# bcgsc/goldpolish

Hardware: NVIDIA B200
Metric: polished_mbp_per_s (higher is better)
Workload: dtype u8/u64 integer

## Files before the change

### goldpolish_b200/api.py

```python
from __future__ import annotations

import ctypes as C
import os

import numpy as np

BF_BYTES = 524288
CBF_BYTES = 10485760
DEFAULT_KS = (32, 28, 24, 20)
GP_MAX_K = 8

_HERE = os.path.dirname(os.path.abspath(__file__))


def lib_path() -> str:
    return os.environ.get("GP_LIB_PATH") or os.path.join(_HERE, "libgoldpolish_b200.so")


class GpError(RuntimeError):
    def __init__(self, code: int, msg: str):
        super().__init__(f"goldpolish_b200 error {code}: {msg}")
        self.code = code


class _Config(C.Structure):
    _fields_ = [("struct_size", C.c_uint32), ("device", C.c_int32), ("nk", C.c_uint32),
                ("k", C.c_uint32 * GP_MAX_K), ("max_insertions", C.c_uint32), ("max_deletions", C.c_uint32),
                ("mode", C.c_int32), ("mask", C.c_int32), ("missing_ratio", C.c_float),
                ("edit_ratio", C.c_float), ("jump", C.c_uint32), ("min_contig_len", C.c_uint32),
                ("max_resident_batches", C.c_uint32), ("use_ratio", C.c_int32),
                ("missing_threshold", C.c_float), ("edit_threshold", C.c_float), ("keep_counters", C.c_int32),
                ("prep_mode", C.c_int32), ("prep_k", C.c_uint32), ("to_upper", C.c_int32),
                ("max_resident_filters", C.c_uint32)]


class _Stats(C.Structure):
    _fields_ = [("kmer_ops", C.c_uint64), ("serial_kmers", C.c_uint64), ("triggers", C.c_uint64),
                ("edits", C.c_uint64), ("masked", C.c_uint64), ("rollbacks", C.c_uint64),
                ("build_ms", C.c_float), ("polish_ms", C.c_float), ("pack_ms", C.c_float),
                ("build_kernel_ms", C.c_float), ("edit_kernel_ms", C.c_float),
                ("build_launches", C.c_uint32), ("polish_launches", C.c_uint32), ("pack_launches", C.c_uint32),
                ("build_kernel", C.c_uint32), ("build_slots", C.c_uint32), ("polish_reruns", C.c_uint32),
                ("edit_sms", C.c_uint32)]


READ_ENTRY_DTYPE = np.dtype([("read_id", np.uint32), ("kmer_threshold", np.uint32)])

_lib = None

EXPORTS = ["gp_default_config", "gp_ctx_create", "gp_ctx_destroy", "gp_last_error", "gp_ctx_set_stream",
           "gp_ctx_synchronize", "gp_get_stats", "gp_reads_upload", "gp_build_filters", "gp_build_stage",
           "gp_build_run", "gp_build_fetch", "gp_build_fetch_cbf", "gp_filters_load", "gp_polish",
           "gp_polish_stage", "gp_polish_run", "gp_polish_fetch", "gp_kmer_threshold", "gp_mappings_cap",
           "gp_guard_rejects", "gp_roof_microbench", "gp_build_round_times", "gp_pipeline_run", "gp_prep", "gp_build_output_host", "gp_host_alloc", "gp_host_free",
           "gp_build_cta_times", "gp_flagged_bed", "gp_debug_nthash", "gp_reads_begin", "gp_reads_append", "gp_reads_end"]


def load_library():
    global _lib
    if _lib is not None:
        return _lib
    p = lib_path()
    if not os.path.exists(p):
        raise ImportError(f"{p} is missing: build it with `python -c 'import __graft_entry__ as g; g.build()'` "
                          "or `make -C goldpolish_b200/csrc`; goldpolish_b200 has no CPU fallback")
    l = C.CDLL(p)
    vp, u32, u64 = C.c_void_p, C.c_uint32, C.c_uint64
    l.gp_default_config.argtypes = [C.POINTER(_Config)]
    l.gp_default_config.restype = None
    l.gp_ctx_create.argtypes = [C.POINTER(_Config), C.POINTER(vp)]
    l.gp_ctx_destroy.argtypes = [vp]
    l.gp_ctx_destroy.restype = None
    l.gp_last_error.argtypes = [vp]
    l.gp_last_error.restype = C.c_char_p
    l.gp_ctx_set_stream.argtypes = [vp, vp]
    l.gp_ctx_synchronize.argtypes = [vp]
    l.gp_get_stats.argtypes = [vp, C.POINTER(_Stats)]
    l.gp_reads_upload.argtypes = [vp, vp, vp, u64]
    l.gp_build_filters.argtypes = [vp, u32, vp, vp, vp]
    l.gp_build_stage.argtypes = [vp, u32, vp, vp]
    l.gp_build_run.argtypes = [vp]
    l.gp_build_fetch.argtypes = [vp, vp]
    l.gp_build_fetch_cbf.argtypes = [vp, u32, u32, vp]
    l.gp_filters_load.argtypes = [vp, u32, vp]
    l.gp_polish.argtypes = [vp, u32, vp, vp, vp, vp, u64, vp, vp]
    l.gp_polish_stage.argtypes = [vp, u32, vp, vp, vp]
    l.gp_polish_run.argtypes = [vp]
    l.gp_polish_fetch.argtypes = [vp, vp, u64, vp, vp]
    l.gp_kmer_threshold.argtypes = [u64]
    l.gp_kmer_threshold.restype = C.c_int
    l.gp_mappings_cap.argtypes = [u64, C.c_double]
    l.gp_mappings_cap.restype = u64
    l.gp_guard_rejects.argtypes = [u64, u64]
    l.gp_guard_rejects.restype = C.c_int
    l.gp_roof_microbench.argtypes = [vp, u32, u32, u64, C.POINTER(C.c_double), C.POINTER(C.c_float)]
    l.gp_build_round_times.argtypes = [vp, C.POINTER(u64)]
    l.gp_pipeline_run.argtypes = [vp]
    l.gp_reads_begin.argtypes = [vp, u64, vp]
    l.gp_reads_append.argtypes = [vp, vp, u64]
    l.gp_reads_end.argtypes = [vp]
    l.gp_debug_nthash.argtypes = [vp, u64, u32, vp, vp, u64, C.POINTER(u64)]
    l.gp_flagged_bed.argtypes = [vp, vp, u32, vp, vp, vp, u64]
    l.gp_flagged_bed.restype = u64
    l.gp_build_cta_times.argtypes = [vp, vp, u32, C.POINTER(u32)]
    l.gp_build_output_host.argtypes = [vp, vp]
    l.gp_host_alloc.argtypes = [u64]
    l.gp_host_alloc.restype = vp
    l.gp_host_free.argtypes = [vp]
    l.gp_host_free.restype = None
    l.gp_prep.argtypes = [vp, u32, vp, vp, C.c_int32, u32, C.c_int32, vp, u64, vp]
    _lib = l
    return l


def kmer_threshold(mappings_bases: int) -> int:
    return load_library().gp_kmer_threshold(int(mappings_bases))


def mappings_cap(target_len: int, subsample_max_per_10kbp: float) -> int:
    return int(load_library().gp_mappings_cap(int(target_len), float(subsample_max_per_10kbp)))


def guard_rejects(input_bytes: int, output_bytes: int) -> bool:
    return bool(load_library().gp_guard_rejects(int(input_bytes), int(output_bytes)))


def flagged_bed(seqs, offsets, names=None):
    l = load_library()
    off = np.ascontiguousarray(offsets, dtype=np.uint64)
    n = len(off) - 1
    cap = 1024
    while True:
        rec = np.zeros(cap, dtype=np.uint32)
        st = np.zeros(cap, dtype=np.uint64)
        en = np.zeros(cap, dtype=np.uint64)
        got = int(l.gp_flagged_bed(_ptr(seqs), _ptr(off), n, _ptr(rec), _ptr(st), _ptr(en), cap))
        if got <= cap:
            break
        cap = got
    return [((names[int(rec[i])] if names is not None else int(rec[i])), int(st[i]), int(en[i])) for i in range(got)]


def _ptr(a):
    if a is None:
        return None
    if isinstance(a, np.ndarray):
        if not a.flags["C_CONTIGUOUS"]:
            raise ValueError("array must be C-contiguous")
        return a.ctypes.data
    if hasattr(a, "data_ptr"):
        if a.is_cuda or not a.is_contiguous():
            raise ValueError("tensor must be a contiguous host tensor")
        return a.data_ptr()
    raise TypeError(type(a))


class Context:

    def __init__(self, device: int = 0, ks=DEFAULT_KS, max_insertions=5, max_deletions=5, mode=1, mask=1,
                 missing_ratio=0.5, edit_ratio=0.5, jump=3, min_contig_len=100, max_resident_batches=0,
                 keep_counters=0, prep_mode=0, prep_k=0, to_upper=0, max_resident_filters=0):
        self._l = load_library()
        cfg = _Config()
        self._l.gp_default_config(C.byref(cfg))
        cfg.device = device
        cfg.nk = len(ks)
        for i, k in enumerate(ks):
            cfg.k[i] = k
        cfg.max_insertions, cfg.max_deletions, cfg.mode, cfg.mask = max_insertions, max_deletions, mode, mask
        cfg.missing_ratio, cfg.edit_ratio, cfg.jump, cfg.min_contig_len = missing_ratio, edit_ratio, jump, min_contig_len
        cfg.max_resident_batches = max_resident_batches
        cfg.keep_counters = keep_counters
        cfg.prep_mode, cfg.prep_k, cfg.to_upper = prep_mode, prep_k, to_upper
        cfg.max_resident_filters = max_resident_filters
        h = C.c_void_p()
        rc = self._l.gp_ctx_create(C.byref(cfg), C.byref(h))
        if rc != 0:
            raise GpError(rc, self._l.gp_last_error(None).decode())
        self._h = h
        self.ks = tuple(ks)
        self.nk = len(ks)
        self.n_batches = 0

    def close(self):
        if getattr(self, "_h", None):
            self._l.gp_ctx_destroy(self._h)
            self._h = None

    def __del__(self):
        try:
            self.close()
        except Exception:
            pass

    def __enter__(self):
        return self

    def __exit__(self, *a):
        self.close()

    def _ck(self, rc):
        if rc != 0:
            raise GpError(rc, self._l.gp_last_error(self._h).decode())

    def set_stream(self, cuda_stream: int | None):
        self._ck(self._l.gp_ctx_set_stream(self._h, C.c_void_p(cuda_stream or 0)))

    def synchronize(self):
        self._ck(self._l.gp_ctx_synchronize(self._h))

    def stats(self) -> dict:
        s = _Stats()
        self._ck(self._l.gp_get_stats(self._h, C.byref(s)))
        return {n: getattr(s, n) for n, _ in _Stats._fields_}

    def upload_reads(self, seqs, offsets):
        offsets = np.ascontiguousarray(offsets, dtype=np.uint64)
        self._keep = (seqs, offsets)
        self._ck(self._l.gp_reads_upload(self._h, _ptr(seqs), _ptr(offsets), len(offsets) - 1))

    def upload_reads_piecewise(self, lens, pieces):
        lens = np.ascontiguousarray(lens, dtype=np.uint32)
        self._ck(self._l.gp_reads_begin(self._h, len(lens), _ptr(lens)))
        for seqs, n in pieces:
            seqs = np.ascontiguousarray(seqs, dtype=np.uint8)
            self._ck(self._l.gp_reads_append(self._h, _ptr(seqs) if seqs.size else None, int(n)))
        self._ck(self._l.gp_reads_end(self._h))

    def build_stage(self, batch_entry_off, entries):
        off = np.ascontiguousarray(batch_entry_off, dtype=np.uint64)
        ent = np.ascontiguousarray(entries, dtype=READ_ENTRY_DTYPE)
        self.n_batches = len(off) - 1
        self._ck(self._l.gp_build_stage(self._h, self.n_batches, _ptr(off), _ptr(ent)))

    def build_run(self):
        self._ck(self._l.gp_build_run(self._h))

    def build_output(self, pinned):
        self._bf_pinned = pinned
        self._ck(self._l.gp_build_output_host(self._h, _ptr(pinned) if pinned is not None else None))

    def build_fetch(self, out=None, want=True):
        if want and out is None:
            out = np.empty((self.n_batches, self.nk, BF_BYTES), dtype=np.uint8)
        self._ck(self._l.gp_build_fetch(self._h, _ptr(out) if want else None))
        return out if want else None

    def build_filters(self, batch_entry_off, entries, fetch=True, out=None):
        self.build_stage(batch_entry_off, entries)
        self.build_run()
        return self.build_fetch(out=out, want=fetch)

    def fetch_cbf(self, batch: int, k_index: int) -> np.ndarray:
        out = np.empty(CBF_BYTES, dtype=np.uint8)
        self._ck(self._l.gp_build_fetch_cbf(self._h, batch, k_index, _ptr(out)))
        return out

    def load_filters(self, payloads):
        payloads = np.ascontiguousarray(payloads, dtype=np.uint8)
        n = payloads.size // (self.nk * BF_BYTES)
        if n * self.nk * BF_BYTES != payloads.size:
            raise ValueError("payloads must be n_batches * nk * 524288 bytes")
        self.n_batches = n
        self._ck(self._l.gp_filters_load(self._h, n, _ptr(payloads)))

    def polish_stage(self, seqs, offsets, contig_batch):
        off = np.ascontiguousarray(offsets, dtype=np.uint64)
        cb = np.ascontiguousarray(contig_batch, dtype=np.uint32)
        self._n_contigs = len(off) - 1
        self._in_bases = int(off[-1])
        self._ck(self._l.gp_polish_stage(self._h, self._n_contigs, _ptr(seqs), _ptr(off), _ptr(cb)))

    def polish_run(self):
        self._ck(self._l.gp_polish_run(self._h))

    def pipeline_run(self):
        self._ck(self._l.gp_pipeline_run(self._h))

    def polish_fetch(self, out=None):
        n = self._n_contigs
        out_off = np.zeros(n + 1, dtype=np.uint64)
        dropped = np.zeros(max(n, 1), dtype=np.uint8)
        if out is None:
            out = np.empty(self._in_bases + self._in_bases // 4 + 65536, dtype=np.uint8)
        rc = self._l.gp_polish_fetch(self._h, _ptr(out), out.nbytes if isinstance(out, np.ndarray) else out.numel(),
                                     _ptr(out_off), _ptr(dropped))
        if rc == -1 and int(out_off[n]) > (out.nbytes if isinstance(out, np.ndarray) else out.numel()):
            out = np.empty(int(out_off[n]), dtype=np.uint8)
            rc = self._l.gp_polish_fetch(self._h, _ptr(out), out.nbytes, _ptr(out_off), _ptr(dropped))
        self._ck(rc)
        return out, out_off, dropped[:n]

    def polish(self, seqs, offsets, contig_batch, out=None):
        self.polish_stage(seqs, offsets, contig_batch)
        self.polish_run()
        return self.polish_fetch(out=out)

    def prep(self, seqs, offsets, mode: int, k: int = 0, to_upper: int = 0):
        off = np.ascontiguousarray(offsets, dtype=np.uint64)
        n = len(off) - 1
        out = np.empty(int(off[-1]) + n + 16, dtype=np.uint8)
        out_off = np.zeros(n + 1, dtype=np.uint64)
        self._ck(self._l.gp_prep(self._h, n, _ptr(seqs), _ptr(off), mode, k, to_upper, _ptr(out), out.nbytes, _ptr(out_off)))
        return out, out_off

    def build_round_times(self):
        out = (C.c_uint64 * 32)()
        self._ck(self._l.gp_build_round_times(self._h, out))
        r = {n: (out[3 * i] / 1e6, out[3 * i + 1] / 1e6, int(out[3 * i + 2])) for i, n in enumerate(self.INTERVAL_KINDS)}
        r["list_entries"] = int(out[31])
        return r

    INTERVAL_KINDS = ("clear", "round0", "level1", "late", "round0+late", "level1+late")

    def debug_nthash(self, read_id: int, k: int):
        n = C.c_uint64()
        cap = 1 << 16
        while True:
            hs = np.zeros((cap, 4), dtype=np.uint64)
            valid = np.zeros(cap, dtype=np.uint8)
            rc = self._l.gp_debug_nthash(self._h, read_id, k, _ptr(hs), _ptr(valid), cap, C.byref(n))
            if rc == -1 and n.value > cap:
                cap = n.value
                continue
            self._ck(rc)
            break
        pos = np.nonzero(valid[:n.value])[0]
        return pos, hs[pos]

    def build_cta_times(self) -> np.ndarray:
        out = np.zeros((1024, 32), dtype=np.uint64)
        n = C.c_uint32()
        self._ck(self._l.gp_build_cta_times(self._h, _ptr(out), 1024, C.byref(n)))
        return out[:n.value, :18].reshape(n.value, 6, 3)

    def roof_microbench(self, warps: int, iters: int, region_bytes: int = CBF_BYTES):
        sps, ms = C.c_double(), C.c_float()
        self._ck(self._l.gp_roof_microbench(self._h, warps, iters, region_bytes, C.byref(sps), C.byref(ms)))
        return sps.value, ms.value
```

### goldpolish_b200/csrc/gp_abi.cu

```cuda
#include "gp_kernels.cuh"

#include <algorithm>
#include <cstdio>
#include <cstdlib>
#include <cstring>
#include <numeric>
#include <string>
#include <vector>

namespace {

thread_local std::string g_create_error;

struct DevBuf {
  void* p = nullptr;
  size_t cap = 0;
  cudaError_t ensure(size_t need)
  {
    if (need <= cap) return cudaSuccess;
    if (p) cudaFree(p);
    p = nullptr; cap = 0;
    size_t want = need + need / 8 + 256;
    cudaError_t e = cudaMalloc(&p, want);
    if (e != cudaSuccess) { cudaGetLastError(); e = cudaMalloc(&p, need); want = need; }
    if (e == cudaSuccess) cap = want;
    return e;
  }
  void release() { if (p) cudaFree(p); p = nullptr; cap = 0; }
  template<typename T> T* as() const { return static_cast<T*>(p); }
};

}

struct gp_ctx {
  gp_config cfg;
  int sm_count = 0;
  cudaStream_t own_stream = nullptr, stream = nullptr;
  uint8_t* bf_host_user = nullptr;
  uint32_t* bf_host_dev = nullptr;
  bool bf_streamed = false;
  std::vector<uint32_t> h_pre, h_maxthr;
  std::vector<uint64_t> h_batch_entry_off;
  std::vector<uint4> h_stream_tab;
  DevBuf d_stream_tab;
  std::vector<uint32_t> h_empty_streams;
  bool edit_ev_valid = false;
  int l2_persist_max = 0, l2_window_max = 0;
  bool l2_window_set = false, l2_roof_window = false;
  int overlap_state = 0;
  bool pipelined = false;
  cudaEvent_t ev[6] = { nullptr, nullptr, nullptr, nullptr, nullptr, nullptr };
  std::vector<cudaEvent_t> wave_ev;
  cudaEvent_t edit_ev[2] = { nullptr, nullptr };
  std::string err;
  gp_stats stats;
  bool build_timed = false, polish_timed = false, pack_timed = false;

  uint64_t n_reads = 0;
  uint64_t reads_total = 0, reads_next = 0, read_slab = 0;
  std::vector<uint32_t> h_read_len;
  std::vector<uint64_t> h_read_boff;
  DevBuf d_ascii, d_ascii_off, d_pk, d_nm, d_read_boff, d_read_len;

  uint32_t n_batches = 0;
  bool filters_ready = false;
  bool build_done = false;
  bool build_staged = false;
  uint32_t wave_batches = 0;
  bool bf_all_resident = true;
  std::vector<uint32_t> h_bf_slot;
  DevBuf d_bf_slot;
  std::vector<uint32_t> wave_first, wave_count, wave_order_off;
  DevBuf d_batch_entry_off, d_entries, d_bf_pool, d_cbf_pool, d_stream_order, d_next, d_counters;
  DevBuf d_step_pre, d_batch_max_thr, d_V, d_alive, d_anchor, d_entry_rel, d_cta_times, d_sm_table;
  uint32_t edit_sms = 0;
  uint32_t edit_ctas_per_sm = 0;
  int sm_split_state = 0;
  uint32_t level_grid = 0;
  uint64_t anchor_stride = 0;
  uint32_t alive_words = 0, n_entries = 0, surv_cap = 0, level_slots = 1, level_time_bits = 26, level_arrays = 2;
  bool levels_ok = false;
  int build_algo = 0;
  int build_algo_resolved = 1;

  uint32_t n_contigs = 0;
  bool polish_staged = false, polish_done = false;
  uint32_t grow = 0;
  std::vector<uint64_t> h_in_off, h_cap_off, h_node_off;
  std::vector<uint32_t> h_len, h_order, h_batch;
  std::vector<uint32_t> h_batch_order, h_order_pipe;
  std::vector<uint32_t> h_wave_contig_off;
  DevBuf d_batch_order, d_batch_done, d_order_pipe;
  DevBuf d_input, d_in_off, d_buf0, d_buf1, d_cap_off, d_cur_len, d_which, d_dropped, d_nodes, d_node_off,
    d_contig_batch, d_order, d_pnext, d_pcounters, d_error, d_out, d_out_off;
};

#define GP_FAIL(ctx, code, msg)                                                                              \
  do {                                                                                                       \
    (ctx)->err = (msg);                                                                                      \
    return (code);                                                                                           \
  } while (0)

#define GP_CUDA(ctx, call)                                                                                   \
  do {                                                                                                       \
    cudaError_t e_ = (call);                                                                                 \
    if (e_ != cudaSuccess) {                                                                                 \
      (ctx)->err = std::string(#call) + ": " + cudaGetErrorString(e_);                                       \
      cudaGetLastError();                                                                                    \
      return e_ == cudaErrorMemoryAllocation ? GP_ERR_OOM : GP_ERR_CUDA;                                     \
    }                                                                                                        \
  } while (0)

namespace {

__global__ void scatter_contigs_kernel(const char* __restrict__ in, const uint64_t* __restrict__ in_off,
                                       char* __restrict__ buf0, const uint64_t* __restrict__ cap_off,
                                       uint32_t* __restrict__ cur_len, uint32_t n)
{
  for (uint32_t c = blockIdx.x; c < n; c += gridDim.x) {
    const uint64_t a = in_off[c];
    const uint32_t len = uint32_t(in_off[c + 1] - a);
    char* dst = buf0 + cap_off[c];
    for (uint32_t i = threadIdx.x; i < len; i += blockDim.x) dst[i] = in[a + i];
    if (threadIdx.x == 0) cur_len[c] = len;
  }
}

__global__ void gather_contigs_kernel(const char* __restrict__ buf0, const char* __restrict__ buf1,
                                      const uint64_t* __restrict__ cap_off, const uint8_t* __restrict__ which,
                                      const uint64_t* __restrict__ out_off, char* __restrict__ out, uint32_t n)
{
  for (uint32_t c = blockIdx.x; c < n; c += gridDim.x) {
    const uint64_t o = out_off[c];
    const uint32_t len = uint32_t(out_off[c + 1] - o);
    const char* src = (which[c] ? buf1 : buf0) + cap_off[c];
    for (uint32_t i = threadIdx.x; i < len; i += blockDim.x) out[o + i] = src[i];
  }
}

int validate_config(const gp_config& c, std::string& why)
{
  if (c.nk == 0 || c.nk > GP_MAX_K_VALUES) { why = "nk must be 1..8"; return GP_ERR_ARG; }
  for (uint32_t i = 0; i < c.nk; i++)
    if (c.k[i] < 4 || c.k[i] > 32) { why = "k must be within 4..32"; return GP_ERR_ARG; }
  if (c.max_insertions > 5) { why = "max_insertions must be <= 5"; return GP_ERR_ARG; }
  if (c.max_deletions > 10) { why = "max_deletions must be <= 10"; return GP_ERR_ARG; }
  if (c.mode < 0 || c.mode > 2) { why = "mode must be 0..2"; return GP_ERR_ARG; }
  if (c.jump == 0) { why = "jump must be >= 1"; return GP_ERR_ARG; }
  if (c.prep_mode < 0 || c.prep_mode > 2) { why = "prep_mode must be 0..2"; return GP_ERR_ARG; }
  if (c.prep_mode && (c.prep_k == 0 || c.prep_k > 64)) { why = "prep_k must be within 1..64"; return GP_ERR_ARG; }
  if (!c.use_ratio && (!(c.missing_threshold > 0) || !(c.edit_threshold > 0))) { why = "x / y thresholds must be > 0"; return GP_ERR_ARG; }
  return GP_OK;
}

}

extern "C" {

void gp_default_config(gp_config* cfg)
{
  std::memset(cfg, 0, sizeof(*cfg));
  cfg->struct_size = sizeof(gp_config);
  cfg->device = 0;
  cfg->nk = 4;
  cfg->k[0] = 32; cfg->k[1] = 28; cfg->k[2] = 24; cfg->k[3] = 20;
  cfg->max_insertions = 5; cfg->max_deletions = 5; cfg->mode = 1; cfg->mask = 1;
  cfg->missing_ratio = 0.5f; cfg->edit_ratio = 0.5f;
  cfg->use_ratio = 1;
  cfg->missing_threshold = 5.0f; cfg->edit_threshold = 9.0f;
  cfg->jump = 3; cfg->min_contig_len = 100;
  cfg->max_resident_batches = 0;
}

const char* gp_last_error(const gp_ctx* ctx) { return ctx ? ctx->err.c_str() : g_create_error.c_str(); }

int gp_ctx_create(const gp_config* cfg, gp_ctx** out)
{
  if (!cfg || !out) { g_create_error = "null argument"; return GP_ERR_ARG; }
  *out = nullptr;
  gp_config c;
  gp_default_config(&c);
  std::memcpy(&c, cfg, std::min<size_t>(cfg->struct_size ? cfg->struct_size : sizeof(gp_config), sizeof(gp_config)));
  c.struct_size = sizeof(gp_config);
  std::string why;
  if (int rc = validate_config(c, why)) { g_create_error = why; return rc; }
  int ndev = 0;
  cudaError_t e = cudaGetDeviceCount(&ndev);
  if (e != cudaSuccess || ndev == 0) {
    cudaGetLastError();
    g_create_error = std::string("no CUDA device available (") + cudaGetErrorString(e) +
                     "); goldpolish_b200 has no CPU path";
    return GP_ERR_NO_DEVICE;
  }
  if (c.device < 0 || c.device >= ndev) { g_create_error = "device ordinal out of range"; return GP_ERR_ARG; }
  if ((e = cudaSetDevice(c.device)) != cudaSuccess) { g_create_error = cudaGetErrorString(e); return GP_ERR_CUDA; }
  gp_ctx* ctx = new gp_ctx();
  ctx->cfg = c;
  std::memset(&ctx->stats, 0, sizeof(ctx->stats));
  cudaDeviceGetAttribute(&ctx->sm_count, cudaDevAttrMultiProcessorCount, c.device);
  cudaDeviceGetAttribute(&ctx->l2_persist_max, cudaDevAttrMaxPersistingL2CacheSize, c.device);
  cudaDeviceGetAttribute(&ctx->l2_window_max, cudaDevAttrMaxAccessPolicyWindowSize, c.device);

  if ((e = cudaStreamCreateWithFlags(&ctx->own_stream, cudaStreamNonBlocking)) != cudaSuccess) {
    g_create_error = cudaGetErrorString(e);
    delete ctx;
    return GP_ERR_CUDA;
  }
  ctx->stream = ctx->own_stream;
  gp::preload_levels();
  gp::preload_edit();
  for (auto& ev : ctx->ev) cudaEventCreate(&ev);
  for (auto& ev : ctx->edit_ev) cudaEventCreate(&ev);
  *out = ctx;
  return GP_OK;
}

void gp_ctx_destroy(gp_ctx* ctx)
{
  if (!ctx) return;
  cudaSetDevice(ctx->cfg.device);
  cudaStreamSynchronize(ctx->stream);
  DevBuf* bufs[] = { &ctx->d_ascii, &ctx->d_ascii_off, &ctx->d_pk, &ctx->d_nm, &ctx->d_read_boff, &ctx->d_read_len,
                     &ctx->d_batch_entry_off, &ctx->d_entries, &ctx->d_bf_pool, &ctx->d_cbf_pool, &ctx->d_stream_order,
                     &ctx->d_next, &ctx->d_counters, &ctx->d_step_pre, &ctx->d_batch_max_thr, &ctx->d_V, &ctx->d_alive, &ctx->d_anchor, &ctx->d_entry_rel, &ctx->d_input, &ctx->d_in_off, &ctx->d_buf0, &ctx->d_buf1,
                     &ctx->d_cap_off, &ctx->d_cur_len, &ctx->d_which, &ctx->d_dropped, &ctx->d_nodes, &ctx->d_node_off,
                     &ctx->d_contig_batch, &ctx->d_order, &ctx->d_pnext, &ctx->d_pcounters, &ctx->d_error, &ctx->d_out,
                     &ctx->d_out_off, &ctx->d_batch_order, &ctx->d_batch_done, &ctx->d_order_pipe, &ctx->d_stream_tab, &ctx->d_cta_times, &ctx->d_bf_slot };
  for (auto* b : bufs) b->release();
  if (ctx->l2_window_set) { cudaCtxResetPersistingL2Cache(); cudaDeviceSetLimit(cudaLimitPersistingL2CacheSize, 0); }
  for (auto& ev : ctx->ev) if (ev) cudaEventDestroy(ev);
  for (auto& ev : ctx->edit_ev) if (ev) cudaEventDestroy(ev);
  for (auto& ev : ctx->wave_ev) if (ev) cudaEventDestroy(ev);
  if (ctx->own_stream) cudaStreamDestroy(ctx->own_stream);
  delete ctx;
}

int gp_ctx_set_stream(gp_ctx* ctx, void* cuda_stream)
{
  if (!ctx) return GP_ERR_ARG;
  cudaSetDevice(ctx->cfg.device);
  GP_CUDA(ctx, cudaStreamSynchronize(ctx->stream));
  ctx->stream = cuda_stream ? static_cast<cudaStream_t>(cuda_stream) : ctx->own_stream;
  return GP_OK;
}

int gp_ctx_synchronize(gp_ctx* ctx)
{
  if (!ctx) return GP_ERR_ARG;
  cudaSetDevice(ctx->cfg.device);
  GP_CUDA(ctx, cudaStreamSynchronize(ctx->stream));
  return GP_OK;
}

static uint32_t sm_split_check(gp_ctx* ctx)
{
  if (!ctx->edit_sms || !ctx->d_sm_table.p) return 0;
  std::vector<uint32_t> t(1 + 2 * 2048);
  if (cudaMemcpy(t.data(), ctx->d_sm_table.p, t.size() * 4, cudaMemcpyDeviceToHost) != cudaSuccess) { cudaGetLastError(); return 0; }
  uint32_t full = 0, other = 0, given_back = 0;
  const uint32_t keep = uint32_t(ctx->sm_count) - ctx->edit_sms;
  for (size_t i = 0; i < 2048; i++) {
    const uint32_t arrived = t[1 + 2 * i], rank_p1 = t[2 + 2 * i];
    if (arrived == ctx->edit_ctas_per_sm) { full++; if (rank_p1 > keep) given_back++; }
    else if (arrived) other++;
  }
  const bool ok = !other && full == uint32_t(ctx->sm_count) && given_back == ctx->edit_sms;
  if (ctx->sm_split_state == 0 || !ok) ctx->sm_split_state = ok ? 1 : -1;
  return ok ? given_back : 0;
}

int gp_get_stats(const gp_ctx* cctx, gp_stats* out)
{
  if (!cctx || !out) return GP_ERR_ARG;
  gp_ctx* ctx = const_cast<gp_ctx*>(cctx);
  cudaSetDevice(ctx->cfg.device);
  GP_CUDA(ctx, cudaStreamSynchronize(ctx->stream));
  if (ctx->pack_timed) cudaEventElapsedTime(&ctx->stats.pack_ms, ctx->ev[0], ctx->ev[1]);
  if (ctx->build_timed && ctx->pipelined) {
    cudaEventElapsedTime(&ctx->stats.build_ms, ctx->ev[2], ctx->ev[3]);
    unsigned long long c[gp::kBuildCounters], pc[8];
    GP_CUDA(ctx, cudaMemcpy(c, ctx->d_counters.p, sizeof c, cudaMemcpyDeviceToHost));
    GP_CUDA(ctx, cudaMemcpy(pc, ctx->d_pcounters.p, sizeof pc, cudaMemcpyDeviceToHost));
    ctx->stats.kmer_ops = c[0];
    ctx->stats.serial_kmers = c[1];
    ctx->stats.build_kernel_ms = float(double(c[21] - c[20]) * 1e-6);
    ctx->stats.edit_kernel_ms = float(double(pc[5] - pc[4]) * 1e-6);
    ctx->stats.polish_ms = ctx->stats.edit_kernel_ms;
    ctx->stats.triggers = pc[0]; ctx->stats.edits = pc[1]; ctx->stats.masked = pc[2]; ctx->stats.rollbacks = pc[3];
    ctx->stats.edit_sms = sm_split_check(ctx);
    *out = ctx->stats;
    return GP_OK;
  }
  if (ctx->build_timed) {
    cudaEventElapsedTime(&ctx->stats.build_ms, ctx->ev[2], ctx->ev[3]);
    ctx->stats.build_kernel_ms = 0;
    for (size_t wv = 0; wv < ctx->wave_first.size() && 2 * wv + 1 < ctx->wave_ev.size(); wv++) {
      float t = 0;
      if (cudaEventElapsedTime(&t, ctx->wave_ev[2 * wv], ctx->wave_ev[2 * wv + 1]) == cudaSuccess) ctx->stats.build_kernel_ms += t;
    }
    unsigned long long c[2] = { 0, 0 };
    GP_CUDA(ctx, cudaMemcpy(c, ctx->d_counters.p, sizeof c, cudaMemcpyDeviceToHost));
    ctx->stats.kmer_ops = c[0];
    ctx->stats.serial_kmers = c[1];
  }
  if (ctx->polish_timed && ctx->edit_ev_valid) {
    cudaEventElapsedTime(&ctx->stats.polish_ms, ctx->ev[4], ctx->ev[5]);
    ctx->stats.edit_kernel_ms = 0;
    if (ctx->n_contigs) cudaEventElapsedTime(&ctx->stats.edit_kernel_ms, ctx->edit_ev[0], ctx->edit_ev[1]);
    unsigned long long c[4] = { 0, 0, 0, 0 };
    GP_CUDA(ctx, cudaMemcpy(c, ctx->d_pcounters.p, sizeof c, cudaMemcpyDeviceToHost));
    ctx->stats.triggers = c[0]; ctx->stats.edits = c[1]; ctx->stats.masked = c[2]; ctx->stats.rollbacks = c[3];
  }
  *out = ctx->stats;
  return GP_OK;
}

static const uint64_t kReadSlabBytes = 256ull << 20;

int gp_reads_begin(gp_ctx* ctx, uint64_t n_reads, const uint32_t* lens)
{
  if (!ctx || (!lens && n_reads)) return GP_ERR_ARG;
  if (n_reads > 0xFFFFFFF0ull) GP_FAIL(ctx, GP_ERR_ARG, "too many reads");
  cudaSetDevice(ctx->cfg.device);
  ctx->n_reads = 0;
  ctx->reads_next = 0;
  ctx->h_read_len.assign(lens, lens + n_reads);
  ctx->h_read_boff.resize(n_reads + 1);
  uint64_t b = 0, longest = 0;
  for (uint64_t r = 0; r < n_reads; r++) {
    if (lens[r] >= (1u << 31)) GP_FAIL(ctx, GP_ERR_ARG, "read longer than 2^31 bases");
    ctx->h_read_boff[r] = b;
    b += (uint64_t(lens[r]) + 31) & ~31ull;
    longest = std::max<uint64_t>(longest, lens[r]);
  }
  ctx->h_read_boff[n_reads] = b;
  const uint64_t words = b / 32 + 2;
  ctx->read_slab = std::max(kReadSlabBytes, longest);
  if (const char* e = std::getenv("GP_READ_SLAB_BYTES")) ctx->read_slab = std::max<uint64_t>(uint64_t(std::atoll(e)), std::max<uint64_t>(longest, 1));
  GP_CUDA(ctx, ctx->d_read_boff.ensure((n_reads + 1) * 8));
  GP_CUDA(ctx, ctx->d_read_len.ensure((n_reads + 1) * 4));
  GP_CUDA(ctx, ctx->d_pk.ensure(words * 8));
  GP_CUDA(ctx, ctx->d_nm.ensure(words * 4));
  cudaStream_t s = ctx->stream;
  GP_CUDA(ctx, cudaMemcpyAsync(ctx->d_read_boff.p, ctx->h_read_boff.data(), (n_reads + 1) * 8, cudaMemcpyHostToDevice, s));
  if (n_reads) GP_CUDA(ctx, cudaMemcpyAsync(ctx->d_read_len.p, ctx->h_read_len.data(), n_reads * 4, cudaMemcpyHostToDevice, s));
  GP_CUDA(ctx, cudaMemsetAsync(ctx->d_nm.as<uint32_t>() + (words - 2), 0xFF, 8, s));
  GP_CUDA(ctx, cudaMemsetAsync(ctx->d_pk.as<uint64_t>() + (words - 2), 0, 16, s));
  GP_CUDA(ctx, cudaEventRecord(ctx->ev[0], s));
  GP_CUDA(ctx, cudaStreamSynchronize(s));
  ctx->reads_total = n_reads;
  ctx->stats.pack_launches = 0;
  return GP_OK;
}

int gp_reads_append(gp_ctx* ctx, const char* seqs, uint64_t n)
{
  if (!ctx || (!seqs && n)) return GP_ERR_ARG;
  if (ctx->reads_next + n > ctx->reads_total) GP_FAIL(ctx, GP_ERR_STATE, "gp_reads_append: more reads than gp_reads_begin announced");
  cudaSetDevice(ctx->cfg.device);
  cudaStream_t s = ctx->stream;
  uint64_t r = ctx->reads_next, done = 0;
  const uint64_t r_end = r + n;
  std::vector<uint64_t> aoff;
  while (r < r_end) {
    uint64_t r1 = r, bytes = 0;
    while (r1 < r_end && (r1 == r || bytes + ctx->h_read_len[r1] <= ctx->read_slab)) bytes += ctx->h_read_len[r1++];
    const uint64_t cnt = r1 - r;
    aoff.resize(cnt + 1);
    aoff[0] = 0;
    for (uint64_t i = 0; i < cnt; i++) aoff[i + 1] = aoff[i] + ctx->h_read_len[r + i];
    GP_CUDA(ctx, ctx->d_ascii.ensure(bytes + 16));
    GP_CUDA(ctx, ctx->d_ascii_off.ensure((cnt + 1) * 8));
    if (bytes) GP_CUDA(ctx, cudaMemcpyAsync(ctx->d_ascii.p, seqs + done, bytes, cudaMemcpyHostToDevice, s));
    GP_CUDA(ctx, cudaMemcpyAsync(ctx->d_ascii_off.p, aoff.data(), (cnt + 1) * 8, cudaMemcpyHostToDevice, s));
    gp::launch_pack_reads(ctx->d_ascii.as<char>(), ctx->d_ascii_off.as<uint64_t>(), ctx->d_read_boff.as<uint64_t>() + r,
                          ctx->d_pk.as<uint64_t>(), ctx->d_nm.as<uint32_t>(), uint32_t(cnt), s);
    GP_CUDA(ctx, cudaGetLastError());
    ctx->stats.pack_launches++;
    GP_CUDA(ctx, cudaStreamSynchronize(s));
    done += bytes;
    r = r1;
  }
  ctx->reads_next = r_end;
  return GP_OK;
}

int gp_reads_end(gp_ctx* ctx)
{
  if (!ctx) return GP_ERR_ARG;
  if (ctx->reads_next != ctx->reads_total) GP_FAIL(ctx, GP_ERR_STATE, "gp_reads_end: fewer reads appended than gp_reads_begin announced");
  cudaSetDevice(ctx->cfg.device);
  GP_CUDA(ctx, cudaEventRecord(ctx->ev[1], ctx->stream));
  GP_CUDA(ctx, cudaStreamSynchronize(ctx->stream));
  ctx->pack_timed = true;
  if (ctx->d_ascii.cap > 2 * kReadSlabBytes) ctx->d_ascii.release();
  ctx->n_reads = ctx->reads_total;
  return GP_OK;
}

int gp_reads_upload(gp_ctx* ctx, const char* seqs, const uint64_t* offsets, uint64_t n_reads)
{
  if (!ctx || (!seqs && n_reads) || !offsets) return GP_ERR_ARG;
  std::vector<uint32_t> lens(n_reads);
  for (uint64_t r = 0; r < n_reads; r++) {
    const uint64_t len = offsets[r + 1] - offsets[r];
    if (len >= (1ull << 31)) GP_FAIL(ctx, GP_ERR_ARG, "read longer than 2^31 bases");
    lens[r] = uint32_t(len);
  }
  if (int rc = gp_reads_begin(ctx, n_reads, lens.data())) return rc;
  if (n_reads)
    if (int rc = gp_reads_append(ctx, seqs + offsets[0], n_reads)) return rc;
  return gp_reads_end(ctx);
}

int gp_build_stage(gp_ctx* ctx, uint32_t n_batches, const uint64_t* batch_entry_off, const gp_read_entry* entries)
{
  if (!ctx || !batch_entry_off || (!entries && n_batches && batch_entry_off[n_batches])) return GP_ERR_ARG;
  cudaSetDevice(ctx->cfg.device);
  const gp_config& c = ctx->cfg;
  const uint64_t n_entries = batch_entry_off[n_batches];
  std::vector<uint64_t> work(n_batches, 0);
  for (uint32_t b = 0; b < n_batches; b++) {
    for (uint64_t e = batch_entry_off[b]; e < batch_entry_off[b + 1]; e++) {
      if (entries[e].read_id >= ctx->n_reads) GP_FAIL(ctx, GP_ERR_ARG, "read_id out of range (upload reads first)");
      if (entries[e].kmer_threshold < 4)
        GP_FAIL(ctx, GP_ERR_ARG, "kmer_threshold must be greater than or equal to 4");
      work[b] += ctx->h_read_len[entries[e].read_id];
    }
  }
  {
    std::vector<uint32_t> pre(size_t(c.nk) * (n_entries + 1), 0u), maxthr(std::max<uint32_t>(n_batches, 1), 0u);
    bool ok = true;
    uint64_t max_steps = 0;
    for (uint32_t ki = 0; ki < c.nk; ki++) {
      uint32_t* pk = pre.data() + size_t(ki) * (n_entries + 1);
      uint64_t acc = 0;
      for (uint64_t e = 0; e < n_entries; e++) {
        pk[e] = uint32_t(acc);
        const uint32_t len = ctx->h_read_len[entries[e].read_id];
        if (len >= c.k[ki]) acc += (uint64_t(len) - c.k[ki] + 1 + 31) / 32;
      }
      pk[n_entries] = uint32_t(acc);
      if (acc >= 0xFFFFFFFFull) ok = false;
      for (uint32_t b = 0; b < n_batches && ok; b++) {
        const uint64_t st = uint64_t(pk[batch_entry_off[b + 1]]) - pk[batch_entry_off[b]];
        max_steps = std::max(max_steps, st);
        if (st * 32 >= (1ull << 26)) ok = false;
      }
    }
    std::vector<uint16_t> entry_rel(std::max<uint64_t>(n_entries, 1), 0);
    for (uint32_t b = 0; b < n_batches; b++) {
      if (batch_entry_off[b + 1] - batch_entry_off[b] > 0xFFFFull) ok = false;
      for (uint64_t e = batch_entry_off[b]; e < batch_entry_off[b + 1]; e++) {
        maxthr[b] = std::max(maxthr[b], entries[e].kmer_threshold);
        if (entries[e].kmer_threshold > 24) ok = false;
        entry_rel[e] = uint16_t(e - batch_entry_off[b]);
      }
    }
    ctx->h_empty_streams.clear();
    for (uint32_t ki = 0; ki < c.nk; ki++) {
      const uint32_t* pk = pre.data() + size_t(ki) * (n_entries + 1);
      for (uint32_t b = 0; b < n_batches; b++)
        if (pk[batch_entry_off[b + 1]] == pk[batch_entry_off[b]]) ctx->h_empty_streams.push_back(b * c.nk + ki);
    }
    ctx->anchor_stride = 1;
    for (uint32_t ki = 0; ki < c.nk; ki++)
      ctx->anchor_stride = std::max<uint64_t>(ctx->anchor_stride, uint64_t(pre[size_t(ki) * (n_entries + 1) + n_entries]) + 1);
    ctx->levels_ok = ok;
    ctx->h_pre = pre;
    ctx->h_maxthr = maxthr;
    ctx->h_batch_entry_off.assign(batch_entry_off, batch_entry_off + n_batches + 1);
    ctx->n_entries = uint32_t(n_entries);
    ctx->alive_words = uint32_t(max_steps + 1);
    ctx->level_time_bits = 16;
    while (ctx->level_time_bits < 26 && (max_steps * 32) >> ctx->level_time_bits) ctx->level_time_bits++;
    GP_CUDA(ctx, ctx->d_step_pre.ensure(pre.size() * 4));
    GP_CUDA(ctx, ctx->d_batch_max_thr.ensure(maxthr.size() * 4));
    ctx->level_slots = 2;
    if (const char* f = std::getenv("GP_LEVEL_OVERLAP")) ctx->level_slots = f[0] == '0' ? 1u : 2u;
    ctx->level_arrays = 2;
    if (const char* f = std::getenv("GP_LEVEL_ARRAYS")) ctx->level_arrays = f[0] == '3' ? 3u : 2u;
    GP_CUDA(ctx, ctx->d_V.ensure(gp::kCbfCounters * 4 * ctx->level_arrays));
    ctx->surv_cap = uint32_t(size_t(ctx->alive_words) * 32 + size_t(8192) * 9 * 32);
    GP_CUDA(ctx, ctx->d_alive.ensure(size_t(ctx->surv_cap) * gp::kLevelSurvWords * gp::kLevelListBufs * 4 + 64 + 8192));
    GP_CUDA(ctx, cudaMemcpyAsync(ctx->d_step_pre.p, pre.data(), pre.size() * 4, cudaMemcpyHostToDevice, ctx->stream));
    GP_CUDA(ctx, cudaMemcpyAsync(ctx->d_batch_max_thr.p, maxthr.data(), maxthr.size() * 4, cudaMemcpyHostToDevice, ctx->stream));
    if (ok) {
      GP_CUDA(ctx, ctx->d_entry_rel.ensure(entry_rel.size() * 2));
      GP_CUDA(ctx, ctx->d_anchor.ensure(ctx->anchor_stride * c.nk * 2));
      GP_CUDA(ctx, cudaMemcpyAsync(ctx->d_entry_rel.p, entry_rel.data(), entry_rel.size() * 2, cudaMemcpyHostToDevice, ctx->stream));
      gp::launch_fill_anchor(ctx->d_step_pre.as<uint32_t>(), ctx->d_entry_rel.as<uint16_t>(), ctx->d_anchor.as<uint16_t>(),
                             uint32_t(n_entries), c.nk, ctx->anchor_stride, ctx->stream);
      GP_CUDA(ctx, cudaGetLastError());
    }
    GP_CUDA(ctx, cudaStreamSynchronize(ctx->stream));
  }
  {
    int algo = ctx->build_algo;
    if (const char* f = std::getenv("GP_BUILD_KERNEL")) algo = f[0] == 'l' ? 2 : (f[0] == 's' || f[0] == 'p') ? 1 : algo;
    if (algo == 0) algo = 2;
    if (!ctx->levels_ok) algo = 1;
    ctx->build_algo_resolved = algo;
  }
  const bool uses_cbf = ctx->build_algo_resolved == 1 || c.keep_counters;
  const uint64_t per_batch = uint64_t(c.nk) * gp::kCbfCounters, per_batch_bf = uint64_t(c.nk) * gp::kBfBytes;
  uint32_t wave = n_batches;
  if (c.max_resident_batches) wave = std::min(wave, c.max_resident_batches);
  {
    size_t free_b = 0, total_b = 0;
    GP_CUDA(ctx, cudaMemGetInfo(&free_b, &total_b));
    const uint64_t usable = uint64_t(free_b) + ctx->d_cbf_pool.cap + ctx->d_bf_pool.cap;
    const uint64_t headroom = 3ull << 30;
    uint64_t bf_limit = n_batches;
    if (c.max_resident_filters) bf_limit = std::min<uint64_t>(bf_limit, c.max_resident_filters);
    const uint64_t fit_bf = usable > headroom ? (usable - headroom) / 2 / per_batch_bf : 0;
    if (fit_bf == 0 && n_batches) GP_FAIL(ctx, GP_ERR_OOM, "not enough device memory for one batch of filters");
    bf_limit = std::min(bf_limit, fit_bf);
    ctx->bf_all_resident = bf_limit >= n_batches;
    if (!ctx->bf_all_resident) wave = uint32_t(std::min<uint64_t>(wave, bf_limit));
    if (uses_cbf) {
      const uint64_t left = usable > headroom ? usable - headroom - (ctx->bf_all_resident ? uint64_t(n_batches) * per_batch_bf : 0) : 0;
      const uint64_t fit = left / (per_batch + (ctx->bf_all_resident ? 0 : per_batch_bf));
      if (fit == 0 && n_batches) GP_FAIL(ctx, GP_ERR_OOM, "not enough device memory for one batch of counting filters");
      wave = uint32_t(std::min<uint64_t>(wave, fit));
    }
  }
  GP_CUDA(ctx, ctx->d_bf_pool.ensure(std::max<uint64_t>(uint64_t(ctx->bf_all_resident ? n_batches : wave) * per_batch_bf, 4)));
  if (n_batches && uses_cbf) {
    cudaError_t e = ctx->d_cbf_pool.ensure(uint64_t(wave) * per_batch);
    while (e != cudaSuccess && wave > 1) { cudaGetLastError(); wave = (wave + 1) / 2; e = ctx->d_cbf_pool.ensure(uint64_t(wave) * per_batch); }
    GP_CUDA(ctx, e);
  }
  ctx->wave_batches = wave;
  ctx->wave_first.clear(); ctx->wave_count.clear(); ctx->wave_order_off.clear();
  std::vector<uint32_t> order_all;
  order_all.reserve(size_t(n_batches) * c.nk);
  for (uint32_t first = 0; first < n_batches; first += wave) {
    const uint32_t cnt = std::min(wave, n_batches - first);
    ctx->wave_first.push_back(first);
    ctx->wave_count.push_back(cnt);
    ctx->wave_order_off.push_back(uint32_t(order_all.size()));
    std::vector<uint32_t> idx(size_t(cnt) * c.nk);
    std::iota(idx.begin(), idx.end(), 0u);
    std::stable_sort(idx.begin(), idx.end(), [&](uint32_t a, uint32_t b2) {
      return work[first + a / c.nk] > work[first + b2 / c.nk];
    });
    order_all.insert(order_all.end(), idx.begin(), idx.end());
  }
  const size_t n_waves = ctx->wave_first.size();
  GP_CUDA(ctx, ctx->d_batch_entry_off.ensure((size_t(n_batches) + 1) * 8));
  GP_CUDA(ctx, ctx->d_entries.ensure(std::max<size_t>(n_entries, 1) * sizeof(gp_read_entry)));
  GP_CUDA(ctx, ctx->d_stream_order.ensure(std::max<size_t>(order_all.size(), 1) * 4));
  GP_CUDA(ctx, ctx->d_next.ensure(std::max<size_t>(n_waves, 1) * 4));
  GP_CUDA(ctx, ctx->d_counters.ensure(gp::kBuildCounters * 8));
  cudaStream_t s = ctx->stream;
  GP_CUDA(ctx, cudaMemcpyAsync(ctx->d_batch_entry_off.p, batch_entry_off, (size_t(n_batches) + 1) * 8, cudaMemcpyHostToDevice, s));
  if (n_entries)
    GP_CUDA(ctx, cudaMemcpyAsync(ctx->d_entries.p, entries, n_entries * sizeof(gp_read_entry), cudaMemcpyHostToDevice, s));
  if (!order_all.empty())
    GP_CUDA(ctx, cudaMemcpyAsync(ctx->d_stream_order.p, order_all.data(), order_all.size() * 4, cudaMemcpyHostToDevice, s));
  GP_CUDA(ctx, cudaStreamSynchronize(s));
  ctx->n_batches = n_batches;
  ctx->build_staged = true;
  ctx->filters_ready = false;
  ctx->build_done = false;
  return GP_OK;
}

static int build_stream_tab(gp_ctx* ctx, cudaStream_t s, bool build_order)
{
  const gp_config& c = ctx->cfg;
  const size_t total = size_t(ctx->n_batches) * c.nk;
  ctx->h_stream_tab.resize(std::max<size_t>(total, 1));
  const size_t ne1 = size_t(ctx->n_entries) + 1;
  size_t w = 0;
  for (size_t wv = 0; wv < ctx->wave_first.size(); wv++)
    for (uint32_t st = 0; st < ctx->wave_count[wv] * c.nk; st++, w++) {
      const uint32_t lb = st / c.nk, ki = st - lb * c.nk;
      const uint32_t b = build_order ? ctx->h_batch_order[ctx->wave_first[wv] + lb] : ctx->wave_first[wv] + lb;
      const uint32_t* pk = ctx->h_pre.data() + size_t(ki) * ne1;
      const uint32_t steps = pk[ctx->h_batch_entry_off[b + 1]] - pk[ctx->h_batch_entry_off[b]];
      ctx->h_stream_tab[w] = make_uint4(steps, ctx->h_maxthr[b] - 2u + ki, b, 0u);
    }
  GP_CUDA(ctx, ctx->d_stream_tab.ensure(ctx->h_stream_tab.size() * sizeof(uint4)));
  GP_CUDA(ctx, cudaMemcpyAsync(ctx->d_stream_tab.p, ctx->h_stream_tab.data(), ctx->h_stream_tab.size() * sizeof(uint4), cudaMemcpyHostToDevice, s));
  return GP_OK;
}

static int upload_bf_slots(gp_ctx* ctx, cudaStream_t s, bool build_order)
{
  if (ctx->bf_all_resident) return GP_OK;
  const uint32_t nb = ctx->n_batches, wave = std::max(ctx->wave_batches, 1u);
  ctx->h_bf_slot.resize(nb);
  for (uint32_t pos = 0; pos < nb; pos++) ctx->h_bf_slot[build_order ? ctx->h_batch_order[pos] : pos] = pos % wave;
  GP_CUDA(ctx, ctx->d_bf_slot.ensure(std::max<size_t>(nb, 1) * 4));
  GP_CUDA(ctx, cudaMemcpyAsync(ctx->d_bf_slot.p, ctx->h_bf_slot.data(), size_t(nb) * 4, cudaMemcpyHostToDevice, s));
  return GP_OK;
}

static int build_launch_levels_wave(gp_ctx* ctx, cudaStream_t s, size_t wv, uint32_t* batch_done, int ctas_per_sm, uint32_t reserve_sms = 0)
{
  const gp_config& c = ctx->cfg;
  {
    size_t tab_off = 0;
    for (size_t i = 0; i < wv; i++) tab_off += size_t(ctx->wave_count[i]) * c.nk;
    gp::LevelParams p;
    std::memset(&p, 0, sizeof p);
    p.pk = ctx->d_pk.as<uint64_t>();
    p.nm = ctx->d_nm.as<uint32_t>();
    p.read_boff = ctx->d_read_boff.as<uint64_t>();
    p.read_len = ctx->d_read_len.as<uint32_t>();
    p.batch_entry_off = ctx->d_batch_entry_off.as<uint64_t>();
    p.entries = ctx->d_entries.as<gp_read_entry>();
    p.step_pre = ctx->d_step_pre.as<uint32_t>();
    p.batch_max_thr = ctx->d_batch_max_thr.as<uint32_t>();
    p.anchor = ctx->d_anchor.as<uint16_t>();
    p.anchor_stride = ctx->anchor_stride;
    p.V = ctx->d_V.as<uint32_t>();
    p.surv = ctx->d_alive.as<uint32_t>();
    p.bars = reinterpret_cast<unsigned long long*>(ctx->d_alive.as<uint32_t>() + size_t(gp::kLevelSurvWords) * gp::kLevelListBufs * ctx->surv_cap);
    p.overlap = ctx->level_slots > 1 ? 1u : 0u;
    p.arrays = ctx->level_arrays;
    p.time_bits = ctx->level_time_bits;
    if (const char* f = std::getenv("GP_LEVEL_REPORT_CTA")) p.report_cta = uint32_t(std::atoi(f));
    p.cbf_pool = c.keep_counters ? ctx->d_cbf_pool.as<uint8_t>() : nullptr;
    p.bf_pool = ctx->d_bf_pool.as<uint32_t>();
    p.bf_slot = ctx->bf_all_resident ? nullptr : ctx->d_bf_slot.as<uint32_t>();
    p.counters = ctx->d_counters.as<unsigned long long>();
    p.surv_cap = ctx->surv_cap;
    p.n_entries = ctx->n_entries;
    p.n_streams = ctx->wave_count[wv] * c.nk;
    p.first_batch = ctx->wave_first[wv];
    p.stream_tab = ctx->d_stream_tab.as<uint4>() + tab_off;
    p.nk = c.nk;
    for (uint32_t i = 0; i < gp::kMaxK; i++) p.k[i] = i < c.nk ? c.k[i] : 0;
    if (c.keep_counters) GP_CUDA(ctx, cudaMemsetAsync(ctx->d_cbf_pool.p, 0, uint64_t(p.n_streams) * gp::kCbfCounters, s));
    GP_CUDA(ctx, cudaMemsetAsync(ctx->d_V.p, 0xFF, gp::kCbfCounters * 4 * ctx->level_arrays, s));
    GP_CUDA(ctx, cudaMemsetAsync(p.bars, 0, 64 + 8192, s));
    p.speed = reinterpret_cast<uint32_t*>(p.bars + 8);
    {
      const char* e = std::getenv("GP_LEVEL_WEIGHTED");
      p.weighted = !(e && e[0] == '0') ? 1u : 0u;
    }
    while (ctx->wave_ev.size() < 2 * (wv + 1)) { cudaEvent_t e2 = nullptr; cudaEventCreate(&e2); ctx->wave_ev.push_back(e2); }
    if (!batch_done) GP_CUDA(ctx, cudaEventRecord(ctx->wave_ev[2 * wv], s));
    p.batch_done = batch_done;
    p.n_batches_total = ctx->n_batches;
    p.bf_host = ctx->bf_host_dev;
    {
      const size_t vbytes = gp::kCbfCounters * 4 * p.arrays;
      const char* e = std::getenv("GP_L2_PERSIST");
      const bool want = !(e && e[0] == '0') && ctx->l2_persist_max > 0 && vbytes <= size_t(ctx->l2_window_max);
      cudaStreamAttrValue av;
      std::memset(&av, 0, sizeof av);
      if (want) {
        const char* wsel = std::getenv("GP_L2_WINDOW");
        const bool only_c = wsel && wsel[0] == 'c' && p.arrays == 3u;
        const size_t wbytes = only_c ? gp::kCbfCounters * 4 : vbytes;
        av.accessPolicyWindow.base_ptr = only_c ? static_cast<void*>(ctx->d_V.as<uint32_t>() + 2 * gp::kCbfCounters) : ctx->d_V.p;
        av.accessPolicyWindow.num_bytes = wbytes;
        av.accessPolicyWindow.hitRatio = std::min(1.0f, float(ctx->l2_persist_max) / float(wbytes));
        av.accessPolicyWindow.hitProp = cudaAccessPropertyPersisting;
        av.accessPolicyWindow.missProp = cudaAccessPropertyStreaming;
      }
      if (want != ctx->l2_window_set) {
        if (cudaDeviceSetLimit(cudaLimitPersistingL2CacheSize, want ? size_t(ctx->l2_persist_max) : 0) != cudaSuccess) cudaGetLastError();
        if (!want) cudaCtxResetPersistingL2Cache();
      }
      if (want || ctx->l2_window_set) {
        GP_CUDA(ctx, cudaStreamSetAttribute(s, cudaStreamAttributeAccessPolicyWindow, &av));
        ctx->l2_window_set = want;
      }
    }
    if (std::getenv("GP_LEVEL_CTA_TIMES")) {
      GP_CUDA(ctx, ctx->d_cta_times.ensure(size_t(ctx->sm_count) * 4 * 32 * 8));
      GP_CUDA(ctx, cudaMemsetAsync(ctx->d_cta_times.p, 0, size_t(ctx->sm_count) * 4 * 32 * 8, s));
      p.cta_times = ctx->d_cta_times.as<unsigned long long>();
    }
    if (reserve_sms) {
      const size_t bytes = (1 + 2 * 2048) * 4;
      GP_CUDA(ctx, ctx->d_sm_table.ensure(bytes));
      GP_CUDA(ctx, cudaMemsetAsync(ctx->d_sm_table.p, 0, bytes, s));
      p.keep_sms = uint32_t(ctx->sm_count) - reserve_sms;
      p.sm_table = ctx->d_sm_table.as<uint32_t>();
    }
    ctx->level_grid = uint32_t((ctx->sm_count - int(reserve_sms)) * gp::levels_ctas_per_sm(ctas_per_sm));
    GP_CUDA(ctx, gp::launch_build_filters_levels(p, ctx->sm_count, s, ctas_per_sm));
    if (!batch_done) GP_CUDA(ctx, cudaEventRecord(ctx->wave_ev[2 * wv + 1], s));
  }
  return GP_OK;
}

static int build_launch_inorder_wave(gp_ctx* ctx, cudaStream_t s, size_t wv)
{
  const gp_config& c = ctx->cfg;
  gp::BuildParams p;
  std::memset(&p, 0, sizeof p);
  p.pk = ctx->d_pk.as<uint64_t>();
  p.nm = ctx->d_nm.as<uint32_t>();
  p.read_boff = ctx->d_read_boff.as<uint64_t>();
  p.read_len = ctx->d_read_len.as<uint32_t>();
  p.batch_entry_off = ctx->d_batch_entry_off.as<uint64_t>();
  p.entries = ctx->d_entries.as<gp_read_entry>();
  p.cbf_pool = ctx->d_cbf_pool.as<uint8_t>();
  p.bf_pool = ctx->d_bf_pool.as<uint32_t>();
  p.bf_slot = ctx->bf_all_resident ? nullptr : ctx->d_bf_slot.as<uint32_t>();
  p.stream_order = ctx->d_stream_order.as<uint32_t>() + ctx->wave_order_off[wv];
  p.next_stream = ctx->d_next.as<uint32_t>() + wv;
  p.counters = ctx->d_counters.as<unsigned long long>();
  p.n_streams = ctx->wave_count[wv] * c.nk;
  p.first_batch = ctx->wave_first[wv];
  p.nk = c.nk;
  for (uint32_t i = 0; i < gp::kMaxK; i++) p.k[i] = i < c.nk ? c.k[i] : 0;
  GP_CUDA(ctx, cudaMemsetAsync(ctx->d_cbf_pool.p, 0, uint64_t(p.n_streams) * gp::kCbfCounters, s));
  while (ctx->wave_ev.size() < 2 * (wv + 1)) { cudaEvent_t e2 = nullptr; cudaEventCreate(&e2); ctx->wave_ev.push_back(e2); }
  GP_CUDA(ctx, cudaEventRecord(ctx->wave_ev[2 * wv], s));
  gp::launch_build_filters(p, ctx->sm_count, s);
  GP_CUDA(ctx, cudaGetLastError());
  GP_CUDA(ctx, cudaEventRecord(ctx->wave_ev[2 * wv + 1], s));
  return GP_OK;
}

static int wave_payloads_out(gp_ctx* ctx, cudaStream_t s, size_t wv, bool kernel_streams)
{
  if (ctx->bf_all_resident || kernel_streams || !ctx->bf_host_user) return GP_OK;
  const uint64_t per = uint64_t(ctx->cfg.nk) * gp::kBfBytes;
  GP_CUDA(ctx, cudaMemcpyAsync(ctx->bf_host_user + uint64_t(ctx->wave_first[wv]) * per, ctx->d_bf_pool.p,
                               uint64_t(ctx->wave_count[wv]) * per, cudaMemcpyDeviceToHost, s));
  return GP_OK;
}

int gp_build_run(gp_ctx* ctx)
{
  if (!ctx) return GP_ERR_ARG;
  if (!ctx->build_staged) GP_FAIL(ctx, GP_ERR_STATE, "gp_build_run before gp_build_stage");
  cudaSetDevice(ctx->cfg.device);
  const gp_config& c = ctx->cfg;
  cudaStream_t s = ctx->stream;
  if (!ctx->bf_all_resident && !ctx->bf_host_user)
    GP_FAIL(ctx, GP_ERR_STATE, "the filters of this call are not all resident at once (max_resident_filters / device memory): "
                               "name a page-locked destination with gp_build_output_host, or use gp_pipeline_run");
  GP_CUDA(ctx, cudaEventRecord(ctx->ev[2], s));
  ctx->pipelined = false;
  uint32_t launches = 0;
  GP_CUDA(ctx, cudaMemsetAsync(ctx->d_counters.p, 0, gp::kBuildCounters * 8, s));
  GP_CUDA(ctx, cudaMemsetAsync(ctx->d_counters.as<unsigned long long>() + 20, 0xFF, 8, s));
  const uint64_t per_bf = uint64_t(c.nk) * gp::kBfBytes;
  if (ctx->n_batches) {
    GP_CUDA(ctx, cudaMemsetAsync(ctx->d_next.p, 0, ctx->wave_first.size() * 4, s));
    if (ctx->bf_all_resident) GP_CUDA(ctx, cudaMemsetAsync(ctx->d_bf_pool.p, 0, uint64_t(ctx->n_batches) * per_bf, s));
  }
  const int algo = ctx->build_algo_resolved;
  if (int rc = upload_bf_slots(ctx, s, false)) return rc;
  if (algo == 2)
    if (int rc = build_stream_tab(ctx, s, false)) return rc;
  for (size_t wv = 0; wv < ctx->wave_first.size(); wv++) {
    if (!ctx->bf_all_resident) GP_CUDA(ctx, cudaMemsetAsync(ctx->d_bf_pool.p, 0, uint64_t(ctx->wave_count[wv]) * per_bf, s));
    if (algo == 2) { if (int rc = build_launch_levels_wave(ctx, s, wv, nullptr, 0)) return rc; }
    else if (int rc = build_launch_inorder_wave(ctx, s, wv)) return rc;
    if (int rc = wave_payloads_out(ctx, s, wv, algo == 2 && ctx->bf_host_dev)) return rc;
    launches += 1;
  }
  ctx->bf_streamed = ctx->bf_host_user && ((algo == 2 && ctx->bf_host_dev) || !ctx->bf_all_resident);
  GP_CUDA(ctx, cudaEventRecord(ctx->ev[3], s));
  ctx->build_timed = true;
  ctx->stats.build_launches = launches;
  ctx->stats.build_kernel = uint32_t(algo);
  ctx->stats.build_slots = algo == 2 ? ctx->level_slots : 0;
  ctx->filters_ready = ctx->bf_all_resident;
  ctx->build_done = true;
  return GP_OK;
}

int gp_build_round_times(gp_ctx* ctx, uint64_t out[32])
{
  if (!ctx || !out) return GP_ERR_ARG;
  if (!ctx->build_done) GP_FAIL(ctx, GP_ERR_STATE, "no filters have been built");
  cudaSetDevice(ctx->cfg.device);
  GP_CUDA(ctx, cudaStreamSynchronize(ctx->stream));
  unsigned long long c[gp::kBuildCounters];
  GP_CUDA(ctx, cudaMemcpy(c, ctx->d_counters.p, sizeof c, cudaMemcpyDeviceToHost));
  std::memset(out, 0, 32 * 8);
  for (uint32_t i = 0; i < gp::kLevelDiag; i++) out[i] = c[gp::kLevelDiagAt + i];
  out[31] = c[17];
  return GP_OK;
}

int gp_debug_nthash(gp_ctx* ctx, uint64_t read_id, uint32_t k, uint64_t* hashes, uint8_t* valid, uint64_t cap_positions,
                    uint64_t* n_positions)
{
  if (!ctx || !hashes || !valid || !n_positions) return GP_ERR_ARG;
  if (read_id >= ctx->n_reads) GP_FAIL(ctx, GP_ERR_ARG, "read_id out of range (upload reads first)");
  if (k < 4 || k > 32) GP_FAIL(ctx, GP_ERR_ARG, "k must be within 4..32");
  cudaSetDevice(ctx->cfg.device);
  const uint32_t len = ctx->h_read_len[read_id];
  const uint64_t npos = len >= k ? uint64_t(len) - k + 1 : 0;
  *n_positions = npos;
  if (npos == 0) return GP_OK;
  if (npos > cap_positions) GP_FAIL(ctx, GP_ERR_ARG, "gp_debug_nthash: output too small (needed positions are in n_positions)");
  uint64_t boff = 0;
  GP_CUDA(ctx, cudaMemcpy(&boff, ctx->d_read_boff.as<uint64_t>() + read_id, 8, cudaMemcpyDeviceToHost));
  DevBuf dh, dv;
  GP_CUDA(ctx, dh.ensure(npos * 32));
  cudaError_t e = dv.ensure(npos);
  if (e != cudaSuccess) { dh.release(); GP_CUDA(ctx, e); }
  gp::launch_debug_nthash(ctx->d_pk.as<uint64_t>(), ctx->d_nm.as<uint32_t>(), boff >> 5, len, k, dh.as<uint64_t>(), dv.as<uint8_t>(), ctx->stream);
  e = cudaGetLastError();
  if (e == cudaSuccess) e = cudaMemcpyAsync(hashes, dh.p, npos * 32, cudaMemcpyDeviceToHost, ctx->stream);
  if (e == cudaSuccess) e = cudaMemcpyAsync(valid, dv.p, npos, cudaMemcpyDeviceToHost, ctx->stream);
  if (e == cudaSuccess) e = cudaStreamSynchronize(ctx->stream);
  dh.release(); dv.release();
  GP_CUDA(ctx, e);
  return GP_OK;
}

int gp_build_cta_times(gp_ctx* ctx, uint64_t* out, uint32_t cap_ctas, uint32_t* n_ctas)
{
  if (!ctx || !out || !n_ctas) return GP_ERR_ARG;
  if (!ctx->build_done || !ctx->d_cta_times.p) GP_FAIL(ctx, GP_ERR_STATE, "no per-CTA times were recorded (set GP_LEVEL_CTA_TIMES=1 before the build)");
  cudaSetDevice(ctx->cfg.device);
  GP_CUDA(ctx, cudaStreamSynchronize(ctx->stream));
  *n_ctas = std::min(cap_ctas, ctx->level_grid);
  GP_CUDA(ctx, cudaMemcpy(out, ctx->d_cta_times.p, size_t(*n_ctas) * 32 * 8, cudaMemcpyDeviceToHost));
  return GP_OK;
}

void* gp_host_alloc(uint64_t bytes)
{
  void* p = nullptr;
  if (cudaHostAlloc(&p, size_t(bytes), cudaHostAllocDefault) != cudaSuccess) { cudaGetLastError(); return nullptr; }
  return p;
}

void gp_host_free(void* p)
{
  if (p) cudaFreeHost(p);
}

int gp_build_output_host(gp_ctx* ctx, uint8_t* bf_out_pinned)
{
  if (!ctx) return GP_ERR_ARG;
  cudaSetDevice(ctx->cfg.device);
  ctx->bf_host_user = nullptr;
  ctx->bf_host_dev = nullptr;
  ctx->bf_streamed = false;
  if (!bf_out_pinned) return GP_OK;
  cudaPointerAttributes at;
  if (cudaPointerGetAttributes(&at, bf_out_pinned) != cudaSuccess || at.type != cudaMemoryTypeHost || !at.devicePointer) {
    cudaGetLastError();
    GP_FAIL(ctx, GP_ERR_ARG, "gp_build_output_host needs page-locked host memory (cudaHostAlloc / cudaHostRegister)");
  }
  ctx->bf_host_user = bf_out_pinned;
  ctx->bf_host_dev = static_cast<uint32_t*>(at.devicePointer);
  return GP_OK;
}

int gp_build_fetch(gp_ctx* ctx, uint8_t* bf_out)
{
  if (!ctx) return GP_ERR_ARG;
  if (!ctx->build_done && !ctx->filters_ready) GP_FAIL(ctx, GP_ERR_STATE, "no filters have been built");
  cudaSetDevice(ctx->cfg.device);
  if (bf_out && bf_out == ctx->bf_host_user && ctx->bf_streamed) {
    GP_CUDA(ctx, cudaStreamSynchronize(ctx->stream));
    for (uint32_t sidx : ctx->h_empty_streams) std::memset(bf_out + uint64_t(sidx) * gp::kBfBytes, 0, gp::kBfBytes);
    return GP_OK;
  }
  if (bf_out && !ctx->bf_all_resident)
    GP_FAIL(ctx, GP_ERR_STATE, "the filters of earlier waves are no longer resident: their payloads went to the buffer named with "
                               "gp_build_output_host (pass that pointer)");
  if (bf_out && ctx->n_batches)
    GP_CUDA(ctx, cudaMemcpyAsync(bf_out, ctx->d_bf_pool.p, uint64_t(ctx->n_batches) * ctx->cfg.nk * gp::kBfBytes,
                                 cudaMemcpyDeviceToHost, ctx->stream));
  GP_CUDA(ctx, cudaStreamSynchronize(ctx->stream));
  return GP_OK;
}

int gp_build_fetch_cbf(gp_ctx* ctx, uint32_t batch, uint32_t k_index, uint8_t* cbf_out)
{
  if (!ctx || !cbf_out) return GP_ERR_ARG;
  if (!ctx->build_done) GP_FAIL(ctx, GP_ERR_STATE, "no filters have been built");
  if (batch >= ctx->n_batches || k_index >= ctx->cfg.nk) GP_FAIL(ctx, GP_ERR_ARG, "batch / k index out of range");
  if (ctx->build_algo_resolved == 2 && !ctx->cfg.keep_counters)
    GP_FAIL(ctx, GP_ERR_STATE, "counting-filter bytes were not materialised: create the context with keep_counters = 1");
  const size_t last = ctx->wave_first.size() - 1;
  if (batch < ctx->wave_first[last]) GP_FAIL(ctx, GP_ERR_STATE, "counting filter of an earlier wave is no longer resident");
  cudaSetDevice(ctx->cfg.device);
  const uint64_t sid = uint64_t(batch - ctx->wave_first[last]) * ctx->cfg.nk + k_index;
  GP_CUDA(ctx, cudaMemcpyAsync(cbf_out, ctx->d_cbf_pool.as<uint8_t>() + sid * gp::kCbfCounters, gp::kCbfCounters,
                               cudaMemcpyDeviceToHost, ctx->stream));
  GP_CUDA(ctx, cudaStreamSynchronize(ctx->stream));
  return GP_OK;
}

int gp_build_filters(gp_ctx* ctx, uint32_t n_batches, const uint64_t* batch_entry_off, const gp_read_entry* entries,
                     uint8_t* bf_out)
{
  int rc = gp_build_stage(ctx, n_batches, batch_entry_off, entries);
  if (rc) return rc;
  if ((rc = gp_build_run(ctx))) return rc;
  return gp_build_fetch(ctx, bf_out);
}

int gp_filters_load(gp_ctx* ctx, uint32_t n_batches, const uint8_t* bf_payloads)
{
  if (!ctx || (!bf_payloads && n_batches)) return GP_ERR_ARG;
  cudaSetDevice(ctx->cfg.device);
  const uint64_t bytes = uint64_t(n_batches) * ctx->cfg.nk * gp::kBfBytes;
  GP_CUDA(ctx, ctx->d_bf_pool.ensure(std::max<uint64_t>(bytes, 4)));
  if (bytes) GP_CUDA(ctx, cudaMemcpyAsync(ctx->d_bf_pool.p, bf_payloads, bytes, cudaMemcpyHostToDevice, ctx->stream));
  GP_CUDA(ctx, cudaStreamSynchronize(ctx->stream));
  ctx->n_batches = n_batches;
  ctx->filters_ready = true;
  ctx->bf_all_resident = true;
  ctx->build_staged = false;
  ctx->build_done = false;
  return GP_OK;
}

static int polish_layout(gp_ctx* ctx)
{
  const uint32_t n = ctx->n_contigs;
  const uint32_t g = ctx->grow;
  ctx->h_cap_off.assign(n + 1, 0);
  ctx->h_node_off.assign(n + 1, 0);
  for (uint32_t i = 0; i < n; i++) {
    const uint64_t len = ctx->h_len[i];
    uint64_t cap = len + (len >> 1) + 4096;
    uint64_t nodes = (len >> 2) + 2048;
    cap <<= g; nodes <<= g;
    cap = (cap + 15) & ~15ull;
    if (cap >= (1ull << 32)) { ctx->err = "contig too long for 32-bit positions"; return GP_ERR_ARG; }
    ctx->h_cap_off[i + 1] = ctx->h_cap_off[i] + cap;
    ctx->h_node_off[i + 1] = ctx->h_node_off[i] + nodes;
  }
  GP_CUDA(ctx, ctx->d_buf0.ensure(std::max<uint64_t>(ctx->h_cap_off[n], 16)));
  GP_CUDA(ctx, ctx->d_buf1.ensure(std::max<uint64_t>(ctx->h_cap_off[n], 16)));
  GP_CUDA(ctx, ctx->d_nodes.ensure(std::max<uint64_t>(ctx->h_node_off[n], 1) * sizeof(gp::EdNode)));
  GP_CUDA(ctx, ctx->d_cap_off.ensure((size_t(n) + 1) * 8));
  GP_CUDA(ctx, ctx->d_node_off.ensure((size_t(n) + 1) * 8));
  GP_CUDA(ctx, cudaMemcpyAsync(ctx->d_cap_off.p, ctx->h_cap_off.data(), (size_t(n) + 1) * 8, cudaMemcpyHostToDevice, ctx->stream));
  GP_CUDA(ctx, cudaMemcpyAsync(ctx->d_node_off.p, ctx->h_node_off.data(), (size_t(n) + 1) * 8, cudaMemcpyHostToDevice, ctx->stream));
  GP_CUDA(ctx, cudaStreamSynchronize(ctx->stream));
  return GP_OK;
}

int gp_polish_stage(gp_ctx* ctx, uint32_t n_contigs, const char* seqs, const uint64_t* offsets, const uint32_t* contig_batch)
{
  if (!ctx || !offsets || (!seqs && n_contigs && offsets[n_contigs]) || (!contig_batch && n_contigs)) return GP_ERR_ARG;
  if (!ctx->filters_ready && !ctx->build_staged)
    GP_FAIL(ctx, GP_ERR_STATE, "gp_polish needs filters (gp_build_filters, gp_build_stage or gp_filters_load)");
  cudaSetDevice(ctx->cfg.device);
  const uint32_t n = n_contigs;
  ctx->n_contigs = n;
  ctx->h_len.resize(n);
  ctx->h_in_off.assign(offsets, offsets + n + 1);
  ctx->h_batch.assign(contig_batch, contig_batch + n);
  for (uint32_t i = 0; i < n; i++) {
    const uint64_t len = offsets[i + 1] - offsets[i];
    if (len >= (1ull << 31)) GP_FAIL(ctx, GP_ERR_ARG, "contig longer than 2^31 bases");
    if (contig_batch[i] >= ctx->n_batches) GP_FAIL(ctx, GP_ERR_ARG, "contig_batch out of range of the current filter set");
    ctx->h_len[i] = uint32_t(len);
  }
  ctx->h_order.resize(n);
  std::iota(ctx->h_order.begin(), ctx->h_order.end(), 0u);
  std::stable_sort(ctx->h_order.begin(), ctx->h_order.end(), [&](uint32_t a, uint32_t b) { return ctx->h_len[a] > ctx->h_len[b]; });
  const uint64_t total = offsets[n];
  GP_CUDA(ctx, ctx->d_input.ensure(std::max<uint64_t>(total, 16)));
  GP_CUDA(ctx, ctx->d_in_off.ensure((size_t(n) + 1) * 8));
  GP_CUDA(ctx, ctx->d_cur_len.ensure(std::max<size_t>(n, 1) * 4));
  GP_CUDA(ctx, ctx->d_which.ensure(std::max<size_t>(n, 1)));
  GP_CUDA(ctx, ctx->d_dropped.ensure(std::max<size_t>(n, 1)));
  GP_CUDA(ctx, ctx->d_contig_batch.ensure(std::max<size_t>(n, 1) * 4));
  GP_CUDA(ctx, ctx->d_order.ensure(std::max<size_t>(n, 1) * 4));
  GP_CUDA(ctx, ctx->d_pnext.ensure(4));
  GP_CUDA(ctx, ctx->d_pcounters.ensure(64));
  GP_CUDA(ctx, ctx->d_error.ensure(4));
  cudaStream_t s = ctx->stream;
  if (total) GP_CUDA(ctx, cudaMemcpyAsync(ctx->d_input.p, seqs, total, cudaMemcpyHostToDevice, s));
  GP_CUDA(ctx, cudaMemcpyAsync(ctx->d_in_off.p, offsets, (size_t(n) + 1) * 8, cudaMemcpyHostToDevice, s));
  if (n) {
    GP_CUDA(ctx, cudaMemcpyAsync(ctx->d_contig_batch.p, contig_batch, size_t(n) * 4, cudaMemcpyHostToDevice, s));
    GP_CUDA(ctx, cudaMemcpyAsync(ctx->d_order.p, ctx->h_order.data(), size_t(n) * 4, cudaMemcpyHostToDevice, s));
  }
  ctx->grow = 0;
  if (int rc = polish_layout(ctx)) return rc;
  ctx->polish_staged = true;
  ctx->polish_done = false;
  return GP_OK;
}

static int polish_prepare(gp_ctx* ctx)
{
  cudaStream_t s = ctx->stream;
  const uint32_t n = ctx->n_contigs;
  GP_CUDA(ctx, cudaMemsetAsync(ctx->d_pnext.p, 0, 4, s));
  GP_CUDA(ctx, cudaMemsetAsync(ctx->d_pcounters.p, 0, 64, s));
  GP_CUDA(ctx, cudaMemsetAsync(ctx->d_pcounters.as<unsigned long long>() + 4, 0xFF, 8, s));
  GP_CUDA(ctx, cudaMemsetAsync(ctx->d_error.p, 0, 4, s));
  if (n == 0) return GP_OK;
  const uint32_t grid = std::min<uint32_t>(n, uint32_t(ctx->sm_count) * 8u);
  scatter_contigs_kernel<<<grid, 256, 0, s>>>(ctx->d_input.as<char>(), ctx->d_in_off.as<uint64_t>(), ctx->d_buf0.as<char>(),
                                              ctx->d_cap_off.as<uint64_t>(), ctx->d_cur_len.as<uint32_t>(), n);
  GP_CUDA(ctx, cudaGetLastError());
  return GP_OK;
}

static int polish_edit(gp_ctx* ctx, cudaStream_t es, const uint32_t* order, uint32_t n_order, const uint32_t* batch_done, int alongside)
{
  const gp_config& c = ctx->cfg;
  const uint32_t n = order ? n_order : ctx->n_contigs;
  if (n == 0) return GP_OK;
  gp::EditParams p;
  std::memset(&p, 0, sizeof p);
  p.n_contigs = n;
  p.buf[0] = ctx->d_buf0.as<char>();
  p.buf[1] = ctx->d_buf1.as<char>();
  p.cap_off = ctx->d_cap_off.as<uint64_t>();
  p.cur_len = ctx->d_cur_len.as<uint32_t>();
  p.which = ctx->d_which.as<uint8_t>();
  p.dropped = ctx->d_dropped.as<uint8_t>();
  p.nodes = ctx->d_nodes.as<gp::EdNode>();
  p.node_off = ctx->d_node_off.as<uint64_t>();
  p.contig_batch = ctx->d_contig_batch.as<uint32_t>();
  p.bf_pool = ctx->d_bf_pool.as<uint32_t>();
  p.bf_slot = ctx->bf_all_resident ? nullptr : ctx->d_bf_slot.as<uint32_t>();
  p.order = order ? order : ctx->d_order.as<uint32_t>();
  p.batch_done = batch_done;
  p.n_batches = ctx->n_batches;
  p.next_contig = ctx->d_pnext.as<uint32_t>();
  p.counters = ctx->d_pcounters.as<unsigned long long>();
  p.error = ctx->d_error.as<int>();
  p.nk = c.nk;
  for (uint32_t i = 0; i < c.nk; i++) {
    p.k[i] = c.k[i];
    const float kf = static_cast<float>(c.k[i]);
    const float jf = static_cast<float>(c.jump);
    if (c.use_ratio) {
      p.thr_missing[i] = (kf / jf) * c.missing_ratio;
      p.thr_edit[i] = (kf / jf) * c.edit_ratio;
      p.thr_del[i] = (1 + (kf / jf)) * c.edit_ratio;
    } else {
      p.thr_missing[i] = kf / c.missing_threshold;
      p.thr_edit[i] = kf / c.edit_threshold;
      p.thr_del[i] = kf / c.edit_threshold;
    }
    p.insertion_cap[i] = static_cast<unsigned>(kf * 1.5f);
  }
  p.max_insertions = c.max_insertions; p.max_deletions = c.max_deletions; p.jump = c.jump;
  p.min_contig_len = c.min_contig_len; p.mode = c.mode; p.mask = c.mask;
  if (!alongside) GP_CUDA(ctx, cudaEventRecord(ctx->edit_ev[0], es));
  GP_CUDA(ctx, gp::launch_edit(p, ctx->sm_count, es, alongside));
  if (!alongside) GP_CUDA(ctx, cudaEventRecord(ctx->edit_ev[1], es));
  ctx->edit_ev_valid = !alongside;
  return GP_OK;
}

static int prep_launch(gp_ctx* ctx, int32_t mode, uint32_t k, int32_t to_upper)
{
  if (ctx->n_contigs == 0 || (!mode && !to_upper)) return GP_OK;
  gp::PrepParams q;
  std::memset(&q, 0, sizeof q);
  q.n_contigs = ctx->n_contigs;
  q.buf[0] = ctx->d_buf0.as<char>();
  q.buf[1] = ctx->d_buf1.as<char>();
  q.cap_off = ctx->d_cap_off.as<uint64_t>();
  q.cur_len = ctx->d_cur_len.as<uint32_t>();
  q.which = ctx->d_which.as<uint8_t>();
  q.dropped = ctx->d_dropped.as<uint8_t>();
  q.k = k; q.mode = mode; q.to_upper = to_upper;
  GP_CUDA(ctx, gp::launch_prep(q, ctx->sm_count, ctx->stream));
  return GP_OK;
}

static int polish_launch(gp_ctx* ctx)
{
  if (int rc = polish_prepare(ctx)) return rc;
  if (int rc = polish_edit(ctx, ctx->stream, nullptr, 0, nullptr, false)) return rc;
  return prep_launch(ctx, ctx->cfg.prep_mode, ctx->cfg.prep_k, ctx->cfg.to_upper);
}

int gp_polish_run(gp_ctx* ctx)
{
  if (!ctx) return GP_ERR_ARG;
  if (!ctx->polish_staged) GP_FAIL(ctx, GP_ERR_STATE, "gp_polish_run before gp_polish_stage");
  if (!ctx->filters_ready)
    GP_FAIL(ctx, GP_ERR_STATE, "gp_polish_run needs the whole filter set resident (build it first; when the filters do not all fit, "
                               "gp_pipeline_run polishes wave by wave)");
  cudaSetDevice(ctx->cfg.device);
  GP_CUDA(ctx, cudaEventRecord(ctx->ev[4], ctx->stream));
  if (int rc = polish_launch(ctx)) return rc;
  GP_CUDA(ctx, cudaEventRecord(ctx->ev[5], ctx->stream));
  ctx->polish_timed = true;
  ctx->stats.polish_launches = ctx->n_contigs ? 2 + ((ctx->cfg.prep_mode || ctx->cfg.to_upper) ? 1 : 0) : 0;
  ctx->polish_done = true;
  return GP_OK;
}

int gp_prep(gp_ctx* ctx, uint32_t n_records, const char* seqs, const uint64_t* offsets, int32_t mode, uint32_t k,
            int32_t to_upper, char* out_seqs, uint64_t out_cap, uint64_t* out_offsets)
{
  if (!ctx || !offsets || !out_offsets || (!seqs && n_records && offsets[n_records])) return GP_ERR_ARG;
  if (mode < 0 || mode > 2 || (mode && (k == 0 || k > 64))) GP_FAIL(ctx, GP_ERR_ARG, "gp_prep: mode 0..2, k 1..64");
  cudaSetDevice(ctx->cfg.device);
  const uint32_t n = n_records;
  ctx->n_contigs = n;
  ctx->h_len.resize(n);
  ctx->h_in_off.assign(offsets, offsets + n + 1);
  ctx->h_batch.assign(n, 0u);
  for (uint32_t i = 0; i < n; i++) {
    const uint64_t len = offsets[i + 1] - offsets[i];
    if (len >= (1ull << 31)) GP_FAIL(ctx, GP_ERR_ARG, "record longer than 2^31 bases");
    ctx->h_len[i] = uint32_t(len);
  }
  const uint64_t total = offsets[n];
  GP_CUDA(ctx, ctx->d_input.ensure(std::max<uint64_t>(total, 16)));
  GP_CUDA(ctx, ctx->d_in_off.ensure((size_t(n) + 1) * 8));
  GP_CUDA(ctx, ctx->d_cur_len.ensure(std::max<size_t>(n, 1) * 4));
  GP_CUDA(ctx, ctx->d_which.ensure(std::max<size_t>(n, 1)));
  GP_CUDA(ctx, ctx->d_dropped.ensure(std::max<size_t>(n, 1)));
  GP_CUDA(ctx, ctx->d_pnext.ensure(4));
  GP_CUDA(ctx, ctx->d_pcounters.ensure(64));
  GP_CUDA(ctx, ctx->d_error.ensure(4));
  cudaStream_t s = ctx->stream;
  if (total) GP_CUDA(ctx, cudaMemcpyAsync(ctx->d_input.p, seqs, total, cudaMemcpyHostToDevice, s));
  GP_CUDA(ctx, cudaMemcpyAsync(ctx->d_in_off.p, offsets, (size_t(n) + 1) * 8, cudaMemcpyHostToDevice, s));
  ctx->grow = 0;
  if (int rc = polish_layout(ctx)) return rc;
  if (int rc = polish_prepare(ctx)) return rc;
  GP_CUDA(ctx, cudaMemsetAsync(ctx->d_which.p, 0, std::max<size_t>(n, 1), s));
  GP_CUDA(ctx, cudaMemsetAsync(ctx->d_dropped.p, 0, std::max<size_t>(n, 1), s));
  if (int rc = prep_launch(ctx, mode, k, to_upper)) return rc;
  ctx->polish_staged = false;
  ctx->polish_done = true;
  return gp_polish_fetch(ctx, out_seqs, out_cap, out_offsets, nullptr);
}

int gp_pipeline_run(gp_ctx* ctx)
{
  if (!ctx) return GP_ERR_ARG;
  if (!ctx->build_staged) GP_FAIL(ctx, GP_ERR_STATE, "gp_pipeline_run before gp_build_stage");
  if (!ctx->polish_staged) GP_FAIL(ctx, GP_ERR_STATE, "gp_pipeline_run before gp_polish_stage");
  cudaSetDevice(ctx->cfg.device);
  const gp_config& c = ctx->cfg;
  const uint32_t n = ctx->n_contigs, nb = ctx->n_batches;
  if (ctx->overlap_state == 0 && ctx->pipelined) {
    int err = 0;
    GP_CUDA(ctx, cudaMemcpyAsync(&err, ctx->d_error.p, 4, cudaMemcpyDeviceToHost, ctx->stream));
    GP_CUDA(ctx, cudaStreamSynchronize(ctx->stream));
    if (ctx->overlap_state == 0) ctx->overlap_state = err == 2 ? -1 : 1;
    if (ctx->sm_split_state == 0) sm_split_check(ctx);
  }
  const int algo = ctx->build_algo_resolved;
  const bool overlap = algo == 2 && n && nb && !c.keep_counters && ctx->overlap_state >= 0 && !std::getenv("GP_NO_OVERLAP");
  if (!overlap && ctx->bf_all_resident) {
    if (int rc = gp_build_run(ctx)) return rc;
    return gp_polish_run(ctx);
  }
  {
    std::vector<uint32_t> maxlen(nb, 0), pos(nb, 0);
    for (uint32_t i = 0; i < n; i++) maxlen[ctx->h_batch[i]] = std::max(maxlen[ctx->h_batch[i]], ctx->h_len[i]);
    ctx->h_batch_order.resize(nb);
    std::iota(ctx->h_batch_order.begin(), ctx->h_batch_order.end(), 0u);
    if (overlap)
      std::stable_sort(ctx->h_batch_order.begin(), ctx->h_batch_order.end(), [&](uint32_t a, uint32_t b) { return maxlen[a] > maxlen[b]; });
    for (uint32_t i = 0; i < nb; i++) pos[ctx->h_batch_order[i]] = i;
    ctx->h_order_pipe.resize(n);
    std::iota(ctx->h_order_pipe.begin(), ctx->h_order_pipe.end(), 0u);
    std::stable_sort(ctx->h_order_pipe.begin(), ctx->h_order_pipe.end(), [&](uint32_t a, uint32_t b) {
      const uint32_t pa = pos[ctx->h_batch[a]], pb = pos[ctx->h_batch[b]];
      return pa != pb ? pa < pb : ctx->h_len[a] > ctx->h_len[b];
    });
    ctx->h_wave_contig_off.assign(ctx->wave_first.size() + 1, 0);
    for (uint32_t i = 0; i < n; i++) {
      const uint32_t p = pos[ctx->h_batch[i]];
      size_t wv = ctx->wave_batches ? p / ctx->wave_batches : 0;
      if (wv >= ctx->wave_first.size()) wv = ctx->wave_first.size() - 1;
      ctx->h_wave_contig_off[wv + 1]++;
    }
    for (size_t wv = 0; wv < ctx->wave_first.size(); wv++) ctx->h_wave_contig_off[wv + 1] += ctx->h_wave_contig_off[wv];
  }
  cudaStream_t s = ctx->stream;
  GP_CUDA(ctx, ctx->d_batch_order.ensure(std::max<size_t>(nb, 1) * 4));
  GP_CUDA(ctx, ctx->d_batch_done.ensure((size_t(nb) + 1) * 4));
  GP_CUDA(ctx, ctx->d_order_pipe.ensure(std::max<size_t>(n, 1) * 4));
  GP_CUDA(ctx, cudaEventRecord(ctx->ev[2], s));
  GP_CUDA(ctx, cudaMemcpyAsync(ctx->d_batch_order.p, ctx->h_batch_order.data(), size_t(nb) * 4, cudaMemcpyHostToDevice, s));
  GP_CUDA(ctx, cudaMemcpyAsync(ctx->d_order_pipe.p, ctx->h_order_pipe.data(), size_t(n) * 4, cudaMemcpyHostToDevice, s));
  GP_CUDA(ctx, cudaMemsetAsync(ctx->d_batch_done.p, 0, (size_t(nb) + 1) * 4, s));
  GP_CUDA(ctx, cudaMemsetAsync(ctx->d_counters.p, 0, gp::kBuildCounters * 8, s));
  GP_CUDA(ctx, cudaMemsetAsync(ctx->d_counters.as<unsigned long long>() + 20, 0xFF, 8, s));
  GP_CUDA(ctx, cudaMemsetAsync(ctx->d_next.p, 0, ctx->wave_first.size() * 4, s));
  const uint64_t per_bf = uint64_t(c.nk) * gp::kBfBytes;
  if (ctx->bf_all_resident) GP_CUDA(ctx, cudaMemsetAsync(ctx->d_bf_pool.p, 0, uint64_t(nb) * per_bf, s));
  if (int rc = upload_bf_slots(ctx, s, true)) return rc;
  if (algo == 2)
    if (int rc = build_stream_tab(ctx, s, true)) return rc;
  if (int rc = polish_prepare(ctx)) return rc;
  uint32_t edit_sms = 0;
  if (overlap) {
    uint64_t draft = 0, steps = 0;
    for (uint32_t i = 0; i < n; i++) draft += ctx->h_len[i];
    for (uint32_t ki = 0; ki < c.nk; ki++) steps += ctx->h_pre[size_t(ki) * (ctx->n_entries + 1) + ctx->n_entries];
    const double edit_s = double(draft) * 0.8e-6, build_s = std::max(1e-6, double(steps) * 32.0 / 9.6e9);
    edit_sms = uint32_t(std::ceil(4.5 * edit_s / build_s / 12.0));
    edit_sms = std::min(std::max(edit_sms, 2u), 24u);
    if (const char* e = std::getenv("GP_EDIT_SMS")) edit_sms = uint32_t(std::max(0, std::atoi(e)));
    if (std::getenv("GP_LEVEL_CTAS") || int(edit_sms) * 2 > ctx->sm_count) edit_sms = 0;
    if (ctx->sm_split_state < 0) edit_sms = 0;
  }
  ctx->edit_sms = edit_sms;
  ctx->edit_ctas_per_sm = uint32_t(gp::levels_ctas_per_sm(0));
  ctx->stats.edit_sms = edit_sms;
  int shared_ctas = 2;
  if (const char* e = std::getenv("GP_EXP_PIPE_CTAS")) shared_ctas = std::max(1, std::atoi(e));
  uint32_t launches = 0, edit_launches = 0;
  uint32_t* bd = overlap ? ctx->d_batch_done.as<uint32_t>() : nullptr;
  for (size_t wv = 0; wv < ctx->wave_first.size(); wv++) {
    if (!ctx->bf_all_resident) GP_CUDA(ctx, cudaMemsetAsync(ctx->d_bf_pool.p, 0, uint64_t(ctx->wave_count[wv]) * per_bf, s));
    if (algo == 2) { if (int rc = build_launch_levels_wave(ctx, s, wv, bd, overlap && !edit_sms ? shared_ctas : 0, edit_sms)) return rc; }
    else if (int rc = build_launch_inorder_wave(ctx, s, wv)) return rc;
    launches++;
    const uint32_t c0 = ctx->h_wave_contig_off[wv], c1 = ctx->h_wave_contig_off[wv + 1];
    if (c1 > c0) {
      if (wv) GP_CUDA(ctx, cudaMemsetAsync(ctx->d_pnext.p, 0, 4, s));
      if (int rc = polish_edit(ctx, s, ctx->d_order_pipe.as<uint32_t>() + c0, c1 - c0, bd, overlap ? (edit_sms ? 2 : 1) : 0)) return rc;
      edit_launches++;
    }
    if (int rc = wave_payloads_out(ctx, s, wv, algo == 2 && ctx->bf_host_dev)) return rc;
  }
  ctx->bf_streamed = ctx->bf_host_user && ((algo == 2 && ctx->bf_host_dev) || !ctx->bf_all_resident);
  if (int rc = prep_launch(ctx, c.prep_mode, c.prep_k, c.to_upper)) return rc;
  GP_CUDA(ctx, cudaEventRecord(ctx->ev[3], s));
  ctx->pipelined = true;
  ctx->build_timed = true;
  ctx->polish_timed = true;
  ctx->stats.build_launches = launches;
  ctx->stats.build_kernel = uint32_t(algo);
  ctx->stats.build_slots = algo == 2 ? ctx->level_slots : 0;
  ctx->stats.polish_launches = 1 + edit_launches + ((c.prep_mode || c.to_upper) ? 1 : 0);
  ctx->filters_ready = ctx->bf_all_resident;
  ctx->build_done = true;
  ctx->polish_done = true;
  return GP_OK;
}

int gp_polish_fetch(gp_ctx* ctx, char* out_seqs, uint64_t out_cap, uint64_t* out_offsets, uint8_t* out_dropped)
{
  if (!ctx || !out_offsets) return GP_ERR_ARG;
  if (!ctx->polish_done) GP_FAIL(ctx, GP_ERR_STATE, "gp_polish_fetch before gp_polish_run");
  cudaSetDevice(ctx->cfg.device);
  cudaStream_t s = ctx->stream;
  const uint32_t n = ctx->n_contigs;
  std::vector<uint32_t> len(n);
  std::vector<uint8_t> dropped(n);
  for (;;) {
    int err = 0;
    GP_CUDA(ctx, cudaMemcpyAsync(&err, ctx->d_error.p, 4, cudaMemcpyDeviceToHost, s));
    if (n) {
      GP_CUDA(ctx, cudaMemcpyAsync(len.data(), ctx->d_cur_len.p, size_t(n) * 4, cudaMemcpyDeviceToHost, s));
      GP_CUDA(ctx, cudaMemcpyAsync(dropped.data(), ctx->d_dropped.p, n, cudaMemcpyDeviceToHost, s));
    }
    GP_CUDA(ctx, cudaStreamSynchronize(s));
    if (!err) break;
    ctx->stats.polish_reruns++;
    auto rerun = [&]() { return ctx->filters_ready ? polish_launch(ctx) : gp_pipeline_run(ctx); };
    if (err == 2) {
      ctx->overlap_state = -1;
      if (int rc = rerun()) return rc;
      continue;
    }
    if (ctx->grow >= 4) GP_FAIL(ctx, GP_ERR_OVERFLOW, "edited contig outgrew its device buffers");
    ctx->grow++;
    if (int rc = polish_layout(ctx)) return rc;
    if (int rc = rerun()) return rc;
  }
  uint64_t o = 0;
  for (uint32_t i = 0; i < n; i++) {
    out_offsets[i] = o;
    if (!dropped[i]) o += len[i];
    if (out_dropped) out_dropped[i] = dropped[i];
  }
  out_offsets[n] = o;
  if (o > out_cap || (o && !out_seqs)) GP_FAIL(ctx, GP_ERR_ARG, "output buffer too small (needed size is in out_offsets[n])");
  if (o) {
    GP_CUDA(ctx, ctx->d_out.ensure(o));
    GP_CUDA(ctx, ctx->d_out_off.ensure((size_t(n) + 1) * 8));
    GP_CUDA(ctx, cudaMemcpyAsync(ctx->d_out_off.p, out_offsets, (size_t(n) + 1) * 8, cudaMemcpyHostToDevice, s));
    const uint32_t grid = std::min<uint32_t>(n, uint32_t(ctx->sm_count) * 8u);
    gather_contigs_kernel<<<grid, 256, 0, s>>>(ctx->d_buf0.as<char>(), ctx->d_buf1.as<char>(), ctx->d_cap_off.as<uint64_t>(),
                                               ctx->d_which.as<uint8_t>(), ctx->d_out_off.as<uint64_t>(), ctx->d_out.as<char>(), n);
    GP_CUDA(ctx, cudaGetLastError());
    GP_CUDA(ctx, cudaMemcpyAsync(out_seqs, ctx->d_out.p, o, cudaMemcpyDeviceToHost, s));
    GP_CUDA(ctx, cudaStreamSynchronize(s));
  }
  return GP_OK;
}

int gp_polish(gp_ctx* ctx, uint32_t n_contigs, const char* seqs, const uint64_t* offsets, const uint32_t* contig_batch,
              char* out_seqs, uint64_t out_cap, uint64_t* out_offsets, uint8_t* out_dropped)
{
  int rc = gp_polish_stage(ctx, n_contigs, seqs, offsets, contig_batch);
  if (rc) return rc;
  if ((rc = gp_polish_run(ctx))) return rc;
  return gp_polish_fetch(ctx, out_seqs, out_cap, out_offsets, out_dropped);
}

uint64_t gp_flagged_bed(const char* seqs, const uint64_t* offsets, uint32_t n_records, uint32_t* run_record,
                        uint64_t* run_start, uint64_t* run_end, uint64_t cap)
{
  if (!offsets || (!seqs && n_records && offsets[n_records])) return 0;
  uint64_t n = 0;
  for (uint32_t r = 0; r < n_records; r++) {
    const char* s = seqs + offsets[r];
    const uint64_t len = offsets[r + 1] - offsets[r];
    for (uint64_t i = 0; i < len;) {
      if (s[i] < 'a' || s[i] > 'z') { i++; continue; }
      uint64_t j = i + 1;
      while (j < len && s[j] >= 'a' && s[j] <= 'z') j++;
      if (n < cap) {
        if (run_record) run_record[n] = r;
        if (run_start) run_start[n] = i;
        if (run_end) run_end[n] = j;
      }
      n++;
      i = j;
    }
  }
  return n;
}

int gp_kmer_threshold(uint64_t mappings_bases)
{
  const double a = 4.66943, b = 2.11391e-07;
  const int t = int(std::round(a + double(mappings_bases) * b));
  return std::min(t, 13);
}

uint64_t gp_mappings_cap(uint64_t target_len, double subsample_max_per_10kbp)
{
  return uint64_t(double(target_len) * subsample_max_per_10kbp / 10000.0);
}

int gp_guard_rejects(uint64_t input_bytes, uint64_t output_bytes)
{
  if (input_bytes == 0) return 0;
  return (output_bytes * 10000ull) / input_bytes < 7500ull ? 1 : 0;
}

int gp_roof_microbench(gp_ctx* ctx, uint32_t warps, uint32_t iters, uint64_t region_bytes, double* sectors_per_s, float* ms)
{
  if (!ctx || !sectors_per_s || warps == 0 || iters == 0 || region_bytes < 4096) return GP_ERR_ARG;
  cudaSetDevice(ctx->cfg.device);
  DevBuf cbf, bf;
  GP_CUDA(ctx, cbf.ensure(std::max<uint64_t>(uint64_t(warps) * region_bytes, gp::kCbfCounters * 4)));
  cudaError_t e = bf.ensure(uint64_t(warps) * gp::kBfBytes);
  if (e != cudaSuccess) { cbf.release(); GP_CUDA(ctx, e); }
  cudaStream_t s = ctx->stream;
  int mode = 0;
  if (const char* m = std::getenv("GP_ROOF_MODE")) mode = std::atoi(m);
  {
    cudaStreamSynchronize(s);
    const bool want = mode >= 3 && ctx->l2_persist_max > 0 && !(std::getenv("GP_L2_PERSIST") && std::getenv("GP_L2_PERSIST")[0] == '0');
    cudaStreamAttrValue av;
    std::memset(&av, 0, sizeof av);
    if (want) {
      av.accessPolicyWindow.base_ptr = cbf.p;
      av.accessPolicyWindow.num_bytes = gp::kCbfCounters * 4;
      av.accessPolicyWindow.hitRatio = 1.0f;
      av.accessPolicyWindow.hitProp = cudaAccessPropertyPersisting;
      av.accessPolicyWindow.missProp = cudaAccessPropertyStreaming;
    }
    if (cudaDeviceSetLimit(cudaLimitPersistingL2CacheSize, want ? size_t(ctx->l2_persist_max) : 0) != cudaSuccess) cudaGetLastError();
    cudaCtxResetPersistingL2Cache();
    cudaStreamSetAttribute(s, cudaStreamAttributeAccessPolicyWindow, &av);
    ctx->l2_window_set = false;
    ctx->l2_roof_window = want;
  }
  cudaMemsetAsync(cbf.p, 0, uint64_t(warps) * region_bytes, s);
  cudaMemsetAsync(bf.p, 0, uint64_t(warps) * gp::kBfBytes, s);
  cudaEvent_t a, b;
  cudaEventCreate(&a); cudaEventCreate(&b);
  gp::launch_roof(cbf.as<uint8_t>(), bf.as<uint32_t>(), region_bytes, std::min(iters, 64u), warps, s);
  cudaEventRecord(a, s);
  gp::launch_roof(cbf.as<uint8_t>(), bf.as<uint32_t>(), region_bytes, iters, warps, s);
  cudaEventRecord(b, s);
  e = cudaStreamSynchronize(s);
  float t = 0;
  cudaEventElapsedTime(&t, a, b);
  cudaEventDestroy(a); cudaEventDestroy(b);
  if (ctx->l2_roof_window) {
    cudaStreamAttrValue av;
    std::memset(&av, 0, sizeof av);
    cudaStreamSetAttribute(s, cudaStreamAttributeAccessPolicyWindow, &av);
    cudaCtxResetPersistingL2Cache();
    cudaDeviceSetLimit(cudaLimitPersistingL2CacheSize, 0);
    ctx->l2_roof_window = false;
  }
  cbf.release(); bf.release();
  GP_CUDA(ctx, e);
  if (ms) *ms = t;
  const int touches = mode >= 3 ? 4 : 8;
  *sectors_per_s = double(warps) * iters * 32.0 * touches / (double(t) * 1e-3);
  return GP_OK;
}

}
```

### goldpolish_b200/csrc/gp_build_levels.cu

```cuda
#include "gp_hashing.cuh"

#include <algorithm>
#include <cstdlib>

namespace gp {

constexpr uint32_t kTimeBits = 26;
constexpr uint32_t kTimeMask = (1u << kTimeBits) - 1u;
constexpr int kLevelWarps = 8;

constexpr uint32_t kRuns = 8;

struct LevelCtx {
  const uint64_t* tf;
  const uint64_t* tr;
  uint32_t lane, gwarp;
};

__device__ __forceinline__ uint64_t warp_list_base(uint32_t n_steps, const uint64_t* cum, uint32_t gwarp)
{
  return ((uint64_t(n_steps) * cum[0]) >> 32) + uint64_t(gwarp) * (kRuns + 1u);
}
__device__ __forceinline__ void run_of_row(uint32_t r, uint32_t n_steps, const uint64_t* cum, uint32_t& s0, uint32_t& len)
{
  const uint32_t r0 = uint32_t(uint64_t(n_steps) * r / kRuns), r1 = uint32_t(uint64_t(n_steps) * (r + 1u) / kRuns);
  const uint64_t rowlen = r1 - r0, phase = (uint64_t(r) << 32) / kRuns;
  const uint32_t a = uint32_t((rowlen * cum[0] + phase) >> 32), b = uint32_t((rowlen * cum[1] + phase) >> 32);
  s0 = r0 + a;
  len = r < kRuns ? b - a : 0u;
}

__device__ __forceinline__ uint32_t pack_index(uint64_t h) { return cbf_index(h) | ((uint32_t(h >> 21) & 1u) << 24); }
__device__ __forceinline__ void unpack_index(uint32_t w, uint32_t& ci, uint32_t& bi)
{
  ci = w & 0xFFFFFFu;
  bi = (w & 0x1FFFFFu) | ((w >> 24) << 21);
}
__device__ __forceinline__ void derive_rest(uint64_t h0, const StreamConsts& sc, uint32_t (&pw)[4])
{
  uint64_t h1 = h0 * sc.mul1, h2 = h0 * sc.mul2, h3 = h0 * sc.mul3;
  h1 ^= h1 >> kMultiShift; h2 ^= h2 >> kMultiShift; h3 ^= h3 >> kMultiShift;
  pw[1] = pack_index(h1); pw[2] = pack_index(h2); pw[3] = pack_index(h3);
}

template<bool PARTIAL, typename F>
__device__ __forceinline__ void for_runs(const LevelParams& p, const LevelCtx& c, const uint64_t* cum, uint32_t batch, uint32_t ki,
                                         const StreamConsts& sc, uint32_t n_steps, uint32_t row0, uint32_t row1, F&& f)
{
  const uint32_t* pre = p.step_pre + uint64_t(ki) * (p.n_entries + 1);
  const uint64_t e0 = p.batch_entry_off[batch], e1 = p.batch_entry_off[batch + 1];
  const uint32_t base = __ldg(pre + e0);
  const uint16_t* anchor = p.anchor + uint64_t(ki) * p.anchor_stride + base;
  uint32_t h_e = 0, h_first = 0, h_last = 0, h_thr = 0, h_len = 0, h_wlo = 0, h_whi = 0;
  {
    uint32_t s0 = 0, len = 0;
    if (c.lane >= row0 && c.lane < row1) run_of_row(c.lane, n_steps, cum, s0, len);
    if (len) {
      h_e = __ldg(anchor + s0);
      const uint64_t e = e0 + h_e;
      h_first = __ldg(pre + e) - base; h_last = __ldg(pre + e + 1) - base;
      const gp_read_entry ent = p.entries[e];
      h_thr = ent.kmer_threshold;
      h_len = p.read_len[ent.read_id];
      const uint64_t wb = p.read_boff[ent.read_id] >> 5;
      h_wlo = uint32_t(wb); h_whi = uint32_t(wb >> 32);
    }
  }
#pragma unroll 1
  for (uint32_t r = row0; r < row1; r++) {
    uint32_t s0, len;
    run_of_row(r, n_steps, cum, s0, len);
    if (len == 0) continue;
    const uint32_t s_end = s0 + len;
    const uint64_t e_head = e0 + __shfl_sync(0xffffffffu, h_e, r);
    uint32_t first = __shfl_sync(0xffffffffu, h_first, r), last = __shfl_sync(0xffffffffu, h_last, r);
    uint32_t kthr = __shfl_sync(0xffffffffu, h_thr, r), len_r = __shfl_sync(0xffffffffu, h_len, r);
    uint64_t wbase = uint64_t(__shfl_sync(0xffffffffu, h_wlo, r)) | (uint64_t(__shfl_sync(0xffffffffu, h_whi, r)) << 32);
    uint32_t s = s0;
    for (uint64_t e = e_head; e < e1 && s < s_end; e++) {
      if (e != e_head) {
        first = __ldg(pre + e) - base; last = __ldg(pre + e + 1) - base;
        if (last <= s) continue;
        const gp_read_entry ent = p.entries[e];
        kthr = ent.kmer_threshold;
        len_r = p.read_len[ent.read_id];
        wbase = p.read_boff[ent.read_id] >> 5;
      }
      const uint32_t thr = kthr - 2u + ki;
      const uint32_t npos = len_r - sc.k + 1;
      uint32_t rs = s - first;
      uint64_t w0 = __ldg(p.pk + wbase + rs), w1 = __ldg(p.pk + wbase + rs + 1);
      uint32_t m0 = __ldg(p.nm + wbase + rs), m1 = __ldg(p.nm + wbase + rs + 1);
      for (; s < last && s < s_end; s++) {
        rs = s - first;
        const uint64_t cw0 = w0, cw1 = w1;
        const uint32_t cm0 = m0, cm1 = m1;
        if (s + 1 < last && s + 1 < s_end) {
          w0 = cw1; m0 = cm1;
          w1 = __ldg(p.pk + wbase + rs + 2);
          m1 = __ldg(p.nm + wbase + rs + 2);
        }
        uint64_t h0 = 0;
        const bool valid = hash_h0<PARTIAL>(c.tf, c.tr, cw0, cw1, cm0, cm1, rs * 32u, npos, c.lane, sc, h0);
        uint32_t pw[4] = { 0xFFFFF0u, 0xFFFFF1u, 0xFFFFF2u, 0xFFFFF3u };
        if (valid) { pw[0] = pack_index(h0); derive_rest(h0, sc, pw); }
        f(s, thr, valid, h0, pw);
      }
    }
  }
}

__global__ void fill_anchor_kernel(const uint32_t* __restrict__ step_pre, const uint16_t* __restrict__ entry_rel,
                                   uint16_t* __restrict__ anchor, uint32_t n_entries, uint32_t nk, uint64_t anchor_stride)
{
  const uint64_t w = (uint64_t(blockIdx.x) * blockDim.x + threadIdx.x) >> 5;
  const uint32_t lane = threadIdx.x & 31u;
  if (w >= uint64_t(n_entries) * nk) return;
  const uint32_t ki = uint32_t(w / n_entries), e = uint32_t(w - uint64_t(ki) * n_entries);
  const uint32_t* pre = step_pre + uint64_t(ki) * (n_entries + 1);
  const uint32_t a = pre[e], b = pre[e + 1];
  const uint16_t v = entry_rel[e];
  for (uint32_t s = a + lane; s < b; s += 32) anchor[uint64_t(ki) * anchor_stride + s] = v;
}

void launch_fill_anchor(const uint32_t* step_pre, const uint16_t* entry_rel, uint16_t* anchor, uint32_t n_entries,
                        uint32_t nk, uint64_t anchor_stride, cudaStream_t s)
{
  const uint64_t warps = uint64_t(n_entries) * nk;
  if (warps == 0) return;
  fill_anchor_kernel<<<uint32_t((warps + 7) / 8), 256, 0, s>>>(step_pre, entry_rel, anchor, n_entries, nk, anchor_stride);
}

struct SurvList {
  uint32_t *lo, *hi, *meta;
};
__device__ __forceinline__ SurvList list_of(const LevelParams& p, uint32_t buf, uint32_t n_steps, const uint64_t* cum, uint32_t gwarp)
{
  SurvList l;
  l.lo = p.surv + uint64_t(buf) * kLevelSurvWords * p.surv_cap + warp_list_base(n_steps, cum, gwarp) * 32u;
  l.hi = l.lo + p.surv_cap;
  l.meta = l.hi + p.surv_cap;
  return l;
}
__device__ __forceinline__ void surv_append(const SurvList& l, uint32_t& cnt, bool q, uint64_t h0, uint32_t meta, uint32_t lane)
{
  const uint32_t m = __ballot_sync(0xffffffffu, q);
  if (q) {
    const uint32_t i = cnt + __popc(m & ((1u << lane) - 1u));
    l.lo[i] = uint32_t(h0);
    l.hi[i] = uint32_t(h0 >> 32);
    l.meta[i] = meta;
  }
  cnt += __popc(m);
}
template<int E>
__device__ __forceinline__ void fetch_entries(const SurvList& l, uint32_t cnt, uint32_t r, uint32_t lane, uint32_t (&lo)[E],
                                              uint32_t (&hi)[E], uint32_t (&meta)[E])
{
#pragma unroll
  for (int e = 0; e < E; e++) {
    const uint32_t i = r + 32u * e + lane;
    lo[e] = 0; hi[e] = 0; meta[e] = 0;
    if (i < cnt) {
      lo[e] = __ldcg(l.lo + i);
      hi[e] = __ldcg(l.hi + i);
      meta[e] = __ldcg(l.meta + i);
    }
  }
}
__device__ __forceinline__ void red_min(uint32_t* p, uint32_t v)
{
  asm volatile("red.relaxed.gpu.global.min.u32 [%0], %1;" ::"l"(p), "r"(v) : "memory");
}
__device__ __forceinline__ void red_or(uint32_t* p, uint32_t v)
{
  asm volatile("red.relaxed.gpu.global.or.b32 [%0], %1;" ::"l"(p), "r"(v) : "memory");
}

__device__ __forceinline__ void bf_load(const uint32_t* __restrict__ bf, const uint32_t (&pw)[4], uint32_t (&w)[4])
{
#pragma unroll
  for (int j = 0; j < 4; j++) { uint32_t ci, bi; unpack_index(pw[j], ci, bi); w[j] = __ldcg(bf + (bi >> 5)); }
}
__device__ __forceinline__ void bf_set(uint32_t* __restrict__ bf, const uint32_t (&pw)[4], const uint32_t (&w)[4])
{
#pragma unroll
  for (int j = 0; j < 4; j++) {
    uint32_t ci, bi;
    unpack_index(pw[j], ci, bi);
    if (!(w[j] & (1u << (bi & 31u)))) red_or(bf + (bi >> 5), 1u << (bi & 31u));
  }
}
__device__ __forceinline__ void bf_insert(uint32_t* __restrict__ bf, const uint32_t (&pw)[4])
{
  uint32_t w[4];
  bf_load(bf, pw, w);
  bf_set(bf, pw, w);
}

struct ListJob {
  SurvList lst;
  uint32_t cnt;
  const uint32_t* V;
  uint32_t* Vn;
  uint32_t* bf;
  uint8_t* cbf;
  uint32_t L, lread, tag, tag_next, vmask;
};

__device__ __forceinline__ uint32_t list_round_all(const ListJob& J, const StreamConsts& sc, uint32_t lane, uint32_t (&nlo)[2],
                                                   uint32_t (&nhi)[2], uint32_t (&nmeta)[2])
{
  uint32_t kept = 0;
  for (uint32_t r = 0; r < J.cnt; r += 64u) {
    uint64_t h0[2];
    uint32_t pw[2][4], meta[2], v[2][4], fw[2][4];
    bool live[2], q[2], ins[2];
#pragma unroll
    for (int e = 0; e < 2; e++) {
      live[e] = r + 32u * e + lane < J.cnt;
      meta[e] = nmeta[e];
      h0[e] = uint64_t(nlo[e]) | (uint64_t(nhi[e]) << 32);
      ins[e] = live[e] && (meta[e] >> kTimeBits) == J.L + 1u;
      pw[e][0] = pack_index(h0[e]);
      derive_rest(h0[e], sc, pw[e]);
#pragma unroll
      for (int j = 0; j < 4; j++) v[e][j] = live[e] ? __ldcg(J.V + (pw[e][j] & 0xFFFFFFu)) : 0u;
#pragma unroll
      for (int j = 0; j < 4; j++) fw[e][j] = 0u;
      if (ins[e]) bf_load(J.bf, pw[e], fw[e]);
    }
    if (r + 64u < J.cnt) fetch_entries<2>(J.lst, J.cnt, r + 64u, lane, nlo, nhi, nmeta);
#pragma unroll
    for (int e = 0; e < 2; e++) {
      const uint32_t t = meta[e] & kTimeMask, thr = meta[e] >> kTimeBits;
      bool reached = live[e];
      uint32_t mx = 0;
#pragma unroll
      for (int j = 0; j < 4; j++) {
        reached &= (v[e][j] & ~J.vmask) == J.tag;
        mx = max(mx, v[e][j] & J.vmask);
        if (J.cbf && live[e] && v[e][j] == (J.tag | t)) J.cbf[pw[e][j] & 0xFFFFFFu] = (uint8_t)J.L;
      }
      q[e] = reached && t > mx && thr > J.L;
      if (q[e] && ins[e]) bf_set(J.bf, pw[e], fw[e]);
      if (q[e] && J.L < J.lread) {
#pragma unroll
        for (int j = 0; j < 4; j++) red_min(J.Vn + (pw[e][j] & 0xFFFFFFu), J.tag_next | t);
      }
    }
    surv_append(J.lst, kept, q[0], h0[0], meta[0], lane);
    surv_append(J.lst, kept, q[1], h0[1], meta[1], lane);
  }
  return kept;
}

__device__ __forceinline__ uint32_t list_round_first(const ListJob& J, const StreamConsts& sc, uint32_t lane, uint32_t (&nlo)[2],
                                                     uint32_t (&nhi)[2], uint32_t (&nmeta)[2])
{
  uint32_t kept = 0;
  for (uint32_t r = 0; r < J.cnt; r += 64u) {
    uint64_t h0[2];
    uint32_t pw[2][4], meta[2], v0[2], v[2][3];
    bool live[2], q[2];
#pragma unroll
    for (int e = 0; e < 2; e++) {
      live[e] = r + 32u * e + lane < J.cnt;
      meta[e] = nmeta[e];
      h0[e] = uint64_t(nlo[e]) | (uint64_t(nhi[e]) << 32);
      pw[e][0] = pack_index(h0[e]);
      v0[e] = live[e] ? __ldcg(J.V + (pw[e][0] & 0xFFFFFFu)) : 0u;
    }
    if (r + 64u < J.cnt) fetch_entries<2>(J.lst, J.cnt, r + 64u, lane, nlo, nhi, nmeta);
#pragma unroll
    for (int e = 0; e < 2; e++) {
      const uint32_t t = meta[e] & kTimeMask;
      q[e] = live[e] && (v0[e] & ~J.vmask) == J.tag && (v0[e] & J.vmask) < t;
      if (q[e]) derive_rest(h0[e], sc, pw[e]);
#pragma unroll
      for (int j = 0; j < 3; j++) v[e][j] = q[e] ? __ldcg(J.V + (pw[e][j + 1] & 0xFFFFFFu)) : 0u;
    }
#pragma unroll
    for (int e = 0; e < 2; e++) {
      const uint32_t t = meta[e] & kTimeMask, thr = meta[e] >> kTimeBits;
#pragma unroll
      for (int j = 0; j < 3; j++) q[e] = q[e] && (v[e][j] & ~J.vmask) == J.tag && (v[e][j] & J.vmask) < t;
      q[e] = q[e] && thr > J.L;
      if (q[e] && thr == J.L + 1u) bf_insert(J.bf, pw[e]);
      if (q[e] && J.L < J.lread) {
#pragma unroll
        for (int j = 0; j < 4; j++) red_min(J.Vn + (pw[e][j] & 0xFFFFFFu), J.tag_next | t);
      }
    }
    surv_append(J.lst, kept, q[0], h0[0], meta[0], lane);
    surv_append(J.lst, kept, q[1], h0[1], meta[1], lane);
  }
  return kept;
}

__device__ __forceinline__ unsigned long long ld_relaxed_u64(const unsigned long long* p)
{
  unsigned long long v;
  asm volatile("ld.relaxed.gpu.global.u64 %0, [%1];" : "=l"(v) : "l"(p) : "memory");
  return v;
}

__device__ __forceinline__ unsigned long long globaltimer_ns()
{
  unsigned long long t;
  asm volatile("mov.u64 %0, %%globaltimer;" : "=l"(t));
  return t;
}

__device__ __forceinline__ void filter_final(const LevelParams& p, uint32_t batch, uint32_t ki, uint32_t slot, uint32_t gtid, uint32_t gthreads)
{
  if (p.bf_host) {
    const uint4* __restrict__ src = reinterpret_cast<const uint4*>(p.bf_pool + (uint64_t(slot) * p.nk + ki) * kBfWords);
    uint4* __restrict__ dst = reinterpret_cast<uint4*>(p.bf_host + (uint64_t(batch) * p.nk + ki) * kBfWords);
    for (uint32_t i = gtid; i < kBfWords / 4u; i += gthreads) dst[i] = __ldcg(src + i);
  }
  if (p.batch_done && gtid == 0) {
    atomicAdd(p.batch_done + batch, 1u);
    atomicAdd(p.batch_done + p.n_batches_total, 1u);
  }
}

__device__ __forceinline__ unsigned long long block_sum(unsigned long long v, unsigned long long* scratch)
{
#pragma unroll
  for (int o = 16; o > 0; o >>= 1) v += __shfl_xor_sync(0xffffffffu, v, o);
  __syncthreads();
  if ((threadIdx.x & 31u) == 0u) scratch[threadIdx.x >> 5] = v;
  __syncthreads();
  unsigned long long t = 0;
  for (uint32_t w = 0; w < (blockDim.x >> 5); w++) t += scratch[w];
  return t;
}

enum : uint32_t { MK_NONE = 0, MK_CLEAR = 1, MK_R0 = 2, MK_R1 = 3 };

struct StreamSt {
  uint32_t valid;
  uint32_t sid, batch, ki, n_steps, lread;
  uint32_t slot;
  uint32_t buf;
  uint32_t cum;
  uint32_t pb;
  uint32_t L;
  uint32_t tag;
  uint32_t tag_next;
};

struct Sched {
  StreamSt cur;
  StreamSt tail;
  uint32_t next_sid, epoch, ord;
  uint32_t need_clear, parts, part, r0_done, publish, recal;
  uint4 nx_info;
};

struct Plan {
  uint32_t finished, main_kind, tail_on;
  uint32_t row0, row1, part, last_part, publish, recal;
  StreamSt cur, tail;
  uint32_t done_n, done_b[2], done_ki[2], done_slot[2];
};

__global__ void __launch_bounds__(kLevelWarps * 32, 3) build_filters_levels_kernel(LevelParams p)
{
  __shared__ uint64_t tf[8 * 256];
  __shared__ uint64_t tr[8 * 256];
  __shared__ Sched sch;
  __shared__ Plan plans[2];
  __shared__ uint32_t warp_cnt[2][kLevelWarps];
  __shared__ uint64_t cum_sh[2][kLevelWarps + 1];
  __shared__ unsigned long long cal_ns, cal_steps;
  __shared__ unsigned long long red_sh[3][kLevelWarps];
  __shared__ unsigned long long diag[kLevelDiag];
  __shared__ uint32_t dense_sh;
  if (p.batch_done) asm volatile("griddepcontrol.launch_dependents;" ::: "memory");
  if (threadIdx.x == 0) {
    uint32_t dense = blockIdx.x;
    if (p.keep_sms < p.sms) {
      const uint32_t per_sm = gridDim.x / p.sms;
      uint32_t smid;
      asm volatile("mov.u32 %0, %%smid;" : "=r"(smid));
      uint32_t* arrivals = p.sm_table + 1u + 2u * (smid & 2047u);
      uint32_t* rank_p1 = arrivals + 1;
      const uint32_t slot = atomicAdd(arrivals, 1u);
      uint32_t rank;
      if (slot == 0u) {
        rank = atomicAdd(p.sm_table, 1u);
        atomicExch(rank_p1, rank + 1u);
      } else {
        while ((rank = *reinterpret_cast<volatile uint32_t*>(rank_p1)) == 0u) { }
        rank -= 1u;
      }
      dense = rank < p.keep_sms && slot < per_sm ? slot * p.keep_sms + rank : 0xFFFFFFFFu;
    }
    dense_sh = dense;
  }
  __syncthreads();
  if (dense_sh == 0xFFFFFFFFu) return;
#define nb (p.n_ctas)
#define bid dense_sh
#define gtid (dense_sh * blockDim.x + threadIdx.x)
#define gthreads (nb * blockDim.x)
  LevelCtx c;
  c.lane = threadIdx.x & 31u;
  c.gwarp = 0;
  if (bid == 0 && threadIdx.x == 0) atomicMin(p.counters + 20, globaltimer_ns());
  fill_hash_tables(tf, tr);
  c.tf = tf; c.tr = tr;
#define gwarp_now (dense_sh * uint32_t(kLevelWarps) + wib)
  const uint32_t nwarps = (nb * blockDim.x) >> 5;
  const uint32_t wib = threadIdx.x >> 5;
  const uint32_t tb = p.time_bits, vmask = (1u << tb) - 1u, maxtag = (1u << (32u - tb)) - 1u;
  const bool planner = threadIdx.x == 32u;
  unsigned long long ops = 0, list_seen = 0;
  if (threadIdx.x == 0) { cal_ns = 0; cal_steps = 0; }
  if (threadIdx.x < kLevelDiag) diag[threadIdx.x] = 0;
  if (threadIdx.x <= uint32_t(kLevelWarps))
    cum_sh[0][threadIdx.x] = cum_sh[1][threadIdx.x] = (uint64_t(bid * kLevelWarps + threadIdx.x) << 32) / nwarps;

  auto new_tag = [&]() { sch.epoch++; return (maxtag - sch.epoch) << tb; };
  auto begin_stream = [&]() {
    StreamSt& S = sch.cur;
    const uint32_t prev_cum = S.cum;
    S.valid = 0;
    for (;;) {
      const uint32_t sid = sch.next_sid;
      if (sid >= p.n_streams) return;
      sch.next_sid = sid + 1u;
      const uint4 info = sch.nx_info;
      if (sid + 1u < p.n_streams) sch.nx_info = __ldg(p.stream_tab + sid + 1u);
      const uint32_t ki = sid % p.nk, batch = info.z;
      if (info.x == 0) {
        if (p.batch_done && bid == 0) { atomicAdd(p.batch_done + batch, 1u); atomicAdd(p.batch_done + p.n_batches_total, 1u); }
        continue;
      }
      const uint32_t lmax = info.y;
      S.valid = 1; S.sid = sid; S.batch = batch; S.ki = ki; S.n_steps = info.x;
      S.slot = p.bf_slot ? __ldg(p.bf_slot + batch) : batch;
      S.lread = p.cbf_pool ? lmax : lmax - 1u;
      S.buf = sch.ord & 1u;
      sch.ord++;
      sch.publish = p.weighted && (sch.ord & 63u) == 4u;
      sch.recal = p.weighted && (sch.ord & 63u) == 5u;
      S.cum = sch.recal ? prev_cum ^ 1u : prev_cum;
      sch.part = 0; sch.r0_done = 0;
      const uint32_t pending = sch.tail.valid ? sch.tail.lread + 2u - sch.tail.L : 0u;
      sch.need_clear = sch.epoch + lmax + 2u + pending > maxtag - 1u;
      const uint32_t z = (sch.tail.lread + sch.tail.pb) & 1u;
      S.pb = sch.tail.valid ? (p.arrays == 3u ? z ^ 1u : z) : 0u;
      sch.parts = 1;
      if (p.overlap && p.arrays == 3u && sch.tail.valid && !sch.need_clear) {
        const uint32_t left = sch.tail.lread + 1u - sch.tail.L;
        sch.parts = left > 2u ? min(left - 1u, kRuns) : 1u;
      }
      return;
    }
  };
  auto make_plan = [&](const Plan* prev, Plan& P) {
    P.done_n = 0;
    auto push_done = [&](const StreamSt& S) { P.done_b[P.done_n] = S.batch; P.done_ki[P.done_n] = S.ki; P.done_slot[P.done_n] = S.slot; P.done_n++; };
    if (prev) {
      if (prev->tail_on) {
        if (sch.tail.L >= sch.tail.lread) { push_done(sch.tail); sch.tail.valid = 0; }
        else { sch.tail.L++; sch.tail.tag = sch.tail.tag_next; }
      }
      switch (prev->main_kind) {
      case MK_CLEAR:
        sch.epoch = 0; sch.need_clear = 0;
        break;
      case MK_R0:
        if (++sch.part == sch.parts) {
          sch.r0_done = 1;
          if (sch.cur.lread == 0u) { push_done(sch.cur); sch.cur.valid = 0; }
        }
        break;
      case MK_R1:
        if (sch.cur.lread <= 1u) push_done(sch.cur);
        else { sch.tail = sch.cur; sch.tail.L = 2; sch.tail.tag = sch.cur.tag_next; }
        sch.cur.valid = 0;
        break;
      default: break;
      }
    }
    if (!sch.cur.valid) begin_stream();
    P.tail_on = sch.tail.valid;
    P.main_kind = MK_NONE;
    if (sch.cur.valid) {
      if (sch.need_clear) {
        if (!sch.tail.valid) P.main_kind = MK_CLEAR;
      } else if (!sch.r0_done) {
        if (!sch.tail.valid || (p.overlap && (p.arrays == 3u || sch.tail.L == sch.tail.lread))) {
          P.main_kind = MK_R0;
          if (sch.part == 0u) sch.cur.tag = new_tag();
          P.part = sch.part;
          P.last_part = sch.part + 1u == sch.parts;
          P.row0 = kRuns * sch.part / sch.parts;
          P.row1 = kRuns * (sch.part + 1u) / sch.parts;
          P.publish = sch.publish; P.recal = sch.recal;
        }
      } else {
        if (!sch.tail.valid || (p.overlap && p.arrays == 3u && sch.tail.L == sch.tail.lread)) {
          P.main_kind = MK_R1;
          sch.cur.L = 1;
          sch.cur.tag_next = new_tag();
        }
      }
    }
    if (P.tail_on) sch.tail.tag_next = new_tag();
    P.cur = sch.cur; P.tail = sch.tail;
    P.finished = P.main_kind == MK_NONE && !P.tail_on;
  };
  if (planner) {
    sch.next_sid = 0; sch.epoch = 0; sch.ord = 0;
    sch.cur.valid = 0; sch.cur.cum = 0; sch.tail.valid = 0;
    sch.need_clear = 0; sch.parts = 1; sch.part = 0; sch.r0_done = 0; sch.publish = 0; sch.recal = 0;
    sch.nx_info = p.n_streams ? __ldg(p.stream_tab) : make_uint4(0u, 0u, 0u, 0u);
    make_plan(nullptr, plans[0]);
  }
  __syncthreads();

  auto t1_array = [&](const StreamSt& S) { return p.V + (p.arrays == 3u ? 2u : ((1u + S.pb) & 1u)) * kCbfCounters; };
  unsigned long long target = 0;
  for (uint32_t it = 0;; it++) {
    const Plan& P = plans[it & 1u];
    const uint32_t main_kind = P.main_kind, tail_on = P.tail_on;
    const bool tail_first = tail_on && ((wib & 1u) == 0u || main_kind == MK_NONE);
    uint32_t nx_lo[2], nx_hi[2], nx_meta[2];
    uint32_t pre_for = 0;
    if (!P.finished && (tail_first || main_kind == MK_R1)) {
      const StreamSt* S = tail_first ? &P.tail : &P.cur;
      const SurvList l = list_of(p, S->buf, S->n_steps, cum_sh[S->cum] + wib, gwarp_now);
      fetch_entries<2>(l, warp_cnt[S->buf][wib], 0, c.lane, nx_lo, nx_hi, nx_meta);
      pre_for = tail_first ? 1u : 2u;
    }
    unsigned long long t_a = 0, t_b = 0;
    if (threadIdx.x == 0) {
      t_a = globaltimer_ns();
      while (ld_relaxed_u64(p.bars) < target) {
        if (globaltimer_ns() - t_a > 10000000000ull) asm volatile("trap;");
      }
      __threadfence();
      t_b = globaltimer_ns();
      target += nb;
    }
    __syncthreads();
    for (uint32_t i = 0; i < P.done_n; i++) filter_final(p, P.done_b[i], P.done_ki[i], P.done_slot[i], gtid, gthreads);
    if (P.finished) break;
    if (planner) make_plan(&P, plans[(it + 1u) & 1u]);
    if (main_kind == MK_R0 && P.part == 0u && P.recal) {
      unsigned long long tot = 0;
      for (uint32_t i = threadIdx.x; i < gridDim.x; i += blockDim.x) tot += __ldcg(p.speed + i);
      tot = block_sum(tot, red_sh[0]);
      const unsigned long long mean = max(1ull, tot / nb), lo = max(1ull, mean * 7ull / 10ull), hi = mean * 14ull / 10ull + 1ull;
      unsigned long long all = 0, before = 0, mine = 0;
      for (uint32_t i = threadIdx.x; i < nb; i += blockDim.x) {
        const unsigned long long v = min(max((unsigned long long)__ldcg(p.speed + i), lo), hi);
        all += v;
        if (i < bid) before += v;
        if (i == bid) mine = v;
      }
      all = block_sum(all, red_sh[0]); before = block_sum(before, red_sh[1]); mine = block_sum(mine, red_sh[2]);
      if (threadIdx.x <= uint32_t(kLevelWarps))
        cum_sh[P.cur.cum][threadIdx.x] = ((before * kLevelWarps + mine * threadIdx.x) << 32) / (all * kLevelWarps);
      __syncthreads();
    }

    for (uint32_t ph = 0; ph < 2u; ph++) {
      const bool tail_now = tail_on ? (tail_first ? ph == 0u : ph == 1u) : false;
      const bool main_now = tail_on ? !tail_now : ph == 0u;
      if (!tail_now && !(main_now && main_kind != MK_NONE)) continue;
      if (main_now && main_kind == MK_CLEAR) {
        for (uint64_t i = gtid; i < kCbfCounters * p.arrays; i += gthreads) p.V[i] = 0xFFFFFFFFu;
        continue;
      }
      if (main_now && main_kind == MK_R0) {
        const uint32_t ki = P.cur.ki, batch = P.cur.batch, cb = P.cur.buf, n_steps = P.cur.n_steps;
        const uint64_t* cum = cum_sh[P.cur.cum] + wib;
        const StreamConsts sc = stream_consts(p.k[ki]);
        uint32_t* __restrict__ bf = p.bf_pool + (uint64_t(P.cur.slot) * p.nk + ki) * kBfWords;
        const SurvList lst = list_of(p, cb, n_steps, cum, gwarp_now);
        uint32_t cnt = P.part ? warp_cnt[cb][wib] : 0u;
        const uint32_t tag = P.cur.tag;
        uint32_t* __restrict__ VC = t1_array(P.cur);
        unsigned long long w_t0 = 0;
        uint32_t w_steps = 0;
        if (threadIdx.x == 0) w_t0 = globaltimer_ns();
        with_kmer_shape(sc, [&](auto shape) {
          for_runs<decltype(shape)::value>(p, c, cum, batch, ki, sc, n_steps, P.row0, P.row1,
                   [&](uint32_t s, uint32_t thr, bool valid, uint64_t h0, const uint32_t (&pw)[4]) {
                     const uint32_t t = s * 32u + c.lane;
                     const bool q = valid && thr > 0u;
                     if (q) {
#pragma unroll
                       for (int j = 0; j < 4; j++) red_min(VC + (pw[j] & 0xFFFFFFu), tag | t);
                       if (thr == 1u) bf_insert(bf, pw);
                     }
                     if (valid) ops++;
                     w_steps++;
                     surv_append(lst, cnt, q && thr > 1u, h0, t | (thr << kTimeBits), c.lane);
                   });
        });
        if (c.lane == 0) warp_cnt[cb][wib] = cnt;
        if (threadIdx.x == 0 && p.weighted) { cal_ns += globaltimer_ns() - w_t0; cal_steps += w_steps; }
        continue;
      }
      const StreamSt* S = tail_now ? &P.tail : &P.cur;
      const uint32_t sbuf = S->buf;
      const StreamConsts sc = stream_consts(p.k[S->ki]);
      ListJob J;
      J.L = S->L; J.lread = S->lread; J.tag = S->tag; J.tag_next = S->tag_next; J.vmask = vmask;
      J.lst = list_of(p, sbuf, S->n_steps, cum_sh[S->cum] + wib, gwarp_now);
      J.V = J.L == 1u ? t1_array(*S) : p.V + ((J.L + S->pb) & 1u) * kCbfCounters;
      J.Vn = p.V + ((J.L + 1u + S->pb) & 1u) * kCbfCounters;
      J.bf = p.bf_pool + (uint64_t(S->slot) * p.nk + S->ki) * kBfWords;
      J.cbf = p.cbf_pool ? p.cbf_pool + uint64_t(S->sid) * kCbfCounters : nullptr;
      J.cnt = warp_cnt[sbuf][wib];
      if (c.lane == 0) list_seen += J.cnt;
      if (pre_for != (tail_now ? 1u : 2u)) fetch_entries<2>(J.lst, J.cnt, 0, c.lane, nx_lo, nx_hi, nx_meta);
      pre_for = 0;
      const uint32_t kept = (J.cbf || J.L > 1u) ? list_round_all(J, sc, c.lane, nx_lo, nx_hi, nx_meta)
                                                 : list_round_first(J, sc, c.lane, nx_lo, nx_hi, nx_meta);
      __syncwarp();
      if (c.lane == 0) warp_cnt[sbuf][wib] = kept;
    }

    __syncthreads();
    if (threadIdx.x == 0) {
      const unsigned long long t_c = globaltimer_ns();
      if (main_kind == MK_R0 && P.publish && P.last_part && p.weighted) {
        p.speed[bid] = uint32_t(min(max(cal_steps * 4000000ull / max(cal_ns, 1ull), 1ull), 262143ull));
        cal_ns = 0; cal_steps = 0;
      }
      __threadfence();
      atomicAdd(p.bars, 1ull);
      const uint32_t kind = main_kind == MK_CLEAR ? 0u : main_kind == MK_R0 ? (tail_on ? 4u : 1u) : main_kind == MK_R1 ? (tail_on ? 5u : 2u) : 3u;
      diag[kind * 3 + 0] += t_b - t_a;
      diag[kind * 3 + 1] += t_c - t_b;
      diag[kind * 3 + 2] += 1;
    }
  }
#pragma unroll
  for (int o = 16; o > 0; o >>= 1) ops += __shfl_xor_sync(0xffffffffu, ops, o);
  if (c.lane == 0 && ops) atomicAdd(p.counters + 0, ops);
  if (c.lane == 0 && list_seen) atomicAdd(p.counters + 17, list_seen);
  if (bid == 0 && threadIdx.x == 0) atomicMax(p.counters + 21, globaltimer_ns());
  if (bid == p.report_cta && threadIdx.x == 0)
    for (uint32_t i = 0; i < kLevelDiag; i++) p.counters[kLevelDiagAt + i] += diag[i];
  if (p.cta_times && threadIdx.x < kLevelDiag) p.cta_times[bid * 32u + threadIdx.x] = diag[threadIdx.x];
#undef bid
#undef nb
#undef gtid
#undef gthreads
#undef gwarp_now
}

__global__ void __launch_bounds__(kLevelWarps * 32) debug_nthash_kernel(const uint64_t* __restrict__ pk, const uint32_t* __restrict__ nm,
                                                                        uint64_t wbase, uint32_t len, uint32_t k,
                                                                        uint64_t* __restrict__ h, uint8_t* __restrict__ valid)
{
  __shared__ uint64_t tf[8 * 256];
  __shared__ uint64_t tr[8 * 256];
  fill_hash_tables(tf, tr);
  __syncthreads();
  if (len < k) return;
  const StreamConsts sc = stream_consts(k);
  const uint32_t npos = len - k + 1, lane = threadIdx.x & 31u;
  const uint32_t warp = (blockIdx.x * blockDim.x + threadIdx.x) >> 5, nwarps = (gridDim.x * blockDim.x) >> 5;
  with_kmer_shape(sc, [&](auto shape) {
    for (uint32_t s = warp; s * 32u < npos; s += nwarps) {
      const uint64_t w0 = __ldg(pk + wbase + s), w1 = __ldg(pk + wbase + s + 1);
      const uint32_t m0 = __ldg(nm + wbase + s), m1 = __ldg(nm + wbase + s + 1);
      uint64_t h0 = 0;
      const bool ok = hash_h0<decltype(shape)::value>(tf, tr, w0, w1, m0, m1, s * 32u, npos, lane, sc, h0);
      const uint32_t pos = s * 32u + lane;
      if (pos < npos) {
        valid[pos] = ok ? 1 : 0;
        uint64_t h1 = h0 * sc.mul1, h2 = h0 * sc.mul2, h3 = h0 * sc.mul3;
        h1 ^= h1 >> kMultiShift; h2 ^= h2 >> kMultiShift; h3 ^= h3 >> kMultiShift;
        h[4 * uint64_t(pos) + 0] = ok ? h0 : 0; h[4 * uint64_t(pos) + 1] = ok ? h1 : 0;
        h[4 * uint64_t(pos) + 2] = ok ? h2 : 0; h[4 * uint64_t(pos) + 3] = ok ? h3 : 0;
      }
    }
  });
}

void launch_debug_nthash(const uint64_t* pk, const uint32_t* nm, uint64_t wbase, uint32_t len, uint32_t k, uint64_t* h,
                         uint8_t* valid, cudaStream_t s)
{
  debug_nthash_kernel<<<8, kLevelWarps * 32, 0, s>>>(pk, nm, wbase, len, k, h, valid);
}

int levels_ctas_per_sm(int ctas_per_sm)
{
  int per_sm = 0;
  cudaOccupancyMaxActiveBlocksPerMultiprocessor(&per_sm, build_filters_levels_kernel, kLevelWarps * 32, 0);
  if (per_sm < 1) per_sm = 1;
  if (per_sm > 4) per_sm = 4;
  if (ctas_per_sm > 0) per_sm = std::min(per_sm, ctas_per_sm);
  if (const char* e = std::getenv("GP_LEVEL_CTAS")) per_sm = std::max(1, std::min(per_sm, std::atoi(e)));
  return per_sm;
}

int levels_max_grid(int sm_count, int ctas_per_sm) { return sm_count * levels_ctas_per_sm(ctas_per_sm); }

void preload_levels()
{
  cudaFuncAttributes a;
  if (cudaFuncGetAttributes(&a, (const void*)build_filters_levels_kernel) != cudaSuccess) cudaGetLastError();
  if (cudaFuncGetAttributes(&a, (const void*)fill_anchor_kernel) != cudaSuccess) cudaGetLastError();
}

cudaError_t launch_build_filters_levels(const LevelParams& p, int sm_count, cudaStream_t s, int ctas_per_sm)
{
  if (p.n_streams == 0) return cudaSuccess;
  cudaFuncSetAttribute((const void*)build_filters_levels_kernel, cudaFuncAttributePreferredSharedMemoryCarveout, 58);
  LevelParams lp = p;
  lp.sms = uint32_t(sm_count);
  if (lp.keep_sms == 0 || lp.keep_sms > lp.sms || !lp.sm_table) lp.keep_sms = lp.sms;
  lp.n_ctas = lp.keep_sms * uint32_t(levels_ctas_per_sm(ctas_per_sm));
  void* args[] = { &lp };
  return cudaLaunchCooperativeKernel((const void*)build_filters_levels_kernel, dim3(sm_count * levels_ctas_per_sm(ctas_per_sm)),
                                     dim3(kLevelWarps * 32), args, 0, s);
}

}
```

### goldpolish_b200/csrc/gp_kernels.cuh

```cuda
#pragma once

#include "../../include/goldpolish_b200.h"
#include "gp_common.cuh"

namespace gp {

constexpr int kBuildCounters = 64;
constexpr uint32_t kLevelDiag = 18, kLevelDiagAt = 32;

struct BuildParams {
  const uint64_t* pk;
  const uint32_t* nm;
  const uint64_t* read_boff;
  const uint32_t* read_len;
  const uint64_t* batch_entry_off;
  const gp_read_entry* entries;
  uint8_t* cbf_pool;
  uint32_t* bf_pool;
  const uint32_t* bf_slot;
  const uint32_t* stream_order;
  uint32_t* next_stream;
  unsigned long long* counters;
  uint32_t n_streams;
  uint32_t first_batch;
  uint32_t nk;
  uint32_t k[kMaxK];
};

constexpr uint32_t kLevelSurvWords = 3;
constexpr uint32_t kLevelListBufs = 2;

struct LevelParams {
  const uint64_t* pk;
  const uint32_t* nm;
  const uint64_t* read_boff;
  const uint32_t* read_len;
  const uint64_t* batch_entry_off;
  const gp_read_entry* entries;
  const uint32_t* step_pre;
  const uint32_t* batch_max_thr;
  const uint4* stream_tab;
  uint32_t* batch_done;
  uint32_t n_batches_total;
  const uint16_t* anchor;
  uint64_t anchor_stride;
  uint32_t* V;
  uint32_t* surv;
  unsigned long long* bars;
  uint32_t* speed;
  uint32_t weighted;
  uint32_t sms;
  uint32_t n_ctas;
  uint32_t keep_sms;
  uint32_t* sm_table;
  uint32_t overlap;
  uint32_t arrays;
  uint8_t* cbf_pool;
  uint32_t* bf_pool;
  const uint32_t* bf_slot;
  uint32_t* bf_host;
  unsigned long long* counters;
  unsigned long long* cta_times;
  uint32_t surv_cap;
  uint32_t time_bits;
  uint32_t report_cta;
  uint32_t n_entries;
  uint32_t n_streams;
  uint32_t first_batch;
  uint32_t nk;
  uint32_t k[kMaxK];
};

struct EdNode {
  int32_t type;
  uint32_t s, e, c;
};

struct EditParams {
  uint32_t n_contigs;
  char* buf[2];
  const uint64_t* cap_off;
  uint32_t* cur_len;
  uint8_t* which;
  uint8_t* dropped;
  EdNode* nodes;
  const uint64_t* node_off;
  const uint32_t* contig_batch;
  const uint32_t* bf_pool;
  const uint32_t* bf_slot;
  const uint32_t* batch_done;
  uint32_t n_batches;
  const uint32_t* order;
  uint32_t* next_contig;
  unsigned long long* counters;
  int* error;
  uint32_t nk;
  uint32_t k[kMaxK];
  float thr_missing[kMaxK], thr_edit[kMaxK], thr_del[kMaxK];
  uint32_t insertion_cap[kMaxK];
  uint32_t max_insertions, max_deletions, jump, min_contig_len;
  int32_t mode, mask;
};

struct PrepParams {
  uint32_t n_contigs;
  char* buf[2];
  const uint64_t* cap_off;
  uint32_t* cur_len;
  uint8_t* which;
  const uint8_t* dropped;
  uint32_t k;
  int32_t mode;
  int32_t to_upper;
};

void launch_pack_reads(const char* ascii, const uint64_t* ascii_off, const uint64_t* base_off, uint64_t* pk,
                       uint32_t* nm, uint32_t n_reads, cudaStream_t s);
void launch_build_filters(const BuildParams& p, int sm_count, cudaStream_t s);
cudaError_t launch_build_filters_levels(const LevelParams& p, int sm_count, cudaStream_t s, int ctas_per_sm = 0);
int levels_ctas_per_sm(int ctas_per_sm);
void preload_levels();
void launch_debug_nthash(const uint64_t* pk, const uint32_t* nm, uint64_t wbase, uint32_t len, uint32_t k, uint64_t* h,
                         uint8_t* valid, cudaStream_t s);
int levels_max_grid(int sm_count, int ctas_per_sm);
void preload_edit();
void launch_fill_anchor(const uint32_t* step_pre, const uint16_t* entry_rel, uint16_t* anchor, uint32_t n_entries,
                        uint32_t nk, uint64_t anchor_stride, cudaStream_t s);
void launch_roof(uint8_t* cbf_pool, uint32_t* bf_pool, uint64_t region, uint32_t iters, uint32_t warps, cudaStream_t s);
cudaError_t launch_prep(const PrepParams& p, int sm_count, cudaStream_t s);
cudaError_t launch_edit(const EditParams& p, int sm_count, cudaStream_t s, int alongside_build = 0);

}
```

Baseline: 31.71.

## Group level-build survivors into hash buckets and dedupe warp peers before atomics

Restructures the level-based filter build so survivor entries are binned into per-CTA hash buckets, with an overflow list, and regrouped through a shared-memory counting sort before each round. Within a warp, lanes holding identical k-mer hashes are matched so that only one leader issues the Bloom-filter insert and the red.min updates, carrying the minimum time. The goal is fewer redundant global atomics and better locality on the counter array. In exchange it adds a grouping phase, extra bucket memory, match and ballot overhead per element, and it drops the three-array split-round mode.

```diff
diff --git a/goldpolish_b200/api.py b/goldpolish_b200/api.py
--- a/goldpolish_b200/api.py
+++ b/goldpolish_b200/api.py
@@ -311,7 +311,13 @@
         r["list_entries"] = int(out[31])
         return r
 
-    INTERVAL_KINDS = ("clear", "round0", "level1", "late", "round0+late", "level1+late")
+    INTERVAL_KINDS = ("clear", "hash", "level1", "late", "hash+late", "group")
+
+    def build_touch_counts(self):
+        out = (C.c_uint64 * 32)()
+        self._ck(self._l.gp_build_round_times(self._h, out))
+        n = len(self.INTERVAL_KINDS) * 3
+        return {"group_visits": int(out[n]), "red_min": int(out[n + 1]), "overflow_entries": int(out[n + 2])}
 
     def debug_nthash(self, read_id: int, k: int):
         n = C.c_uint64()
diff --git a/goldpolish_b200/csrc/gp_abi.cu b/goldpolish_b200/csrc/gp_abi.cu
--- a/goldpolish_b200/csrc/gp_abi.cu
+++ b/goldpolish_b200/csrc/gp_abi.cu
@@ -72,13 +72,13 @@
   DevBuf d_bf_slot;
   std::vector<uint32_t> wave_first, wave_count, wave_order_off;
   DevBuf d_batch_entry_off, d_entries, d_bf_pool, d_cbf_pool, d_stream_order, d_next, d_counters;
-  DevBuf d_step_pre, d_batch_max_thr, d_V, d_alive, d_anchor, d_entry_rel, d_cta_times, d_sm_table;
+  DevBuf d_step_pre, d_batch_max_thr, d_V, d_alive, d_groups, d_anchor, d_entry_rel, d_cta_times, d_sm_table;
   uint32_t edit_sms = 0;
   uint32_t edit_ctas_per_sm = 0;
   int sm_split_state = 0;
   uint32_t level_grid = 0;
   uint64_t anchor_stride = 0;
-  uint32_t alive_words = 0, n_entries = 0, surv_cap = 0, level_slots = 1, level_time_bits = 26, level_arrays = 2;
+  uint32_t alive_words = 0, n_entries = 0, surv_cap = 0, level_slots = 1, level_time_bits = 26;
   bool levels_ok = false;
   int build_algo = 0;
   int build_algo_resolved = 1;
@@ -222,7 +222,7 @@
   cudaStreamSynchronize(ctx->stream);
   DevBuf* bufs[] = { &ctx->d_ascii, &ctx->d_ascii_off, &ctx->d_pk, &ctx->d_nm, &ctx->d_read_boff, &ctx->d_read_len,
                      &ctx->d_batch_entry_off, &ctx->d_entries, &ctx->d_bf_pool, &ctx->d_cbf_pool, &ctx->d_stream_order,
-                     &ctx->d_next, &ctx->d_counters, &ctx->d_step_pre, &ctx->d_batch_max_thr, &ctx->d_V, &ctx->d_alive, &ctx->d_anchor, &ctx->d_entry_rel, &ctx->d_input, &ctx->d_in_off, &ctx->d_buf0, &ctx->d_buf1,
+                     &ctx->d_next, &ctx->d_counters, &ctx->d_step_pre, &ctx->d_batch_max_thr, &ctx->d_V, &ctx->d_alive, &ctx->d_groups, &ctx->d_anchor, &ctx->d_entry_rel, &ctx->d_input, &ctx->d_in_off, &ctx->d_buf0, &ctx->d_buf1,
                      &ctx->d_cap_off, &ctx->d_cur_len, &ctx->d_which, &ctx->d_dropped, &ctx->d_nodes, &ctx->d_node_off,
                      &ctx->d_contig_batch, &ctx->d_order, &ctx->d_pnext, &ctx->d_pcounters, &ctx->d_error, &ctx->d_out,
                      &ctx->d_out_off, &ctx->d_batch_order, &ctx->d_batch_done, &ctx->d_order_pipe, &ctx->d_stream_tab, &ctx->d_cta_times, &ctx->d_bf_slot };
@@ -478,11 +478,7 @@
     GP_CUDA(ctx, ctx->d_batch_max_thr.ensure(maxthr.size() * 4));
     ctx->level_slots = 2;
     if (const char* f = std::getenv("GP_LEVEL_OVERLAP")) ctx->level_slots = f[0] == '0' ? 1u : 2u;
-    ctx->level_arrays = 2;
-    if (const char* f = std::getenv("GP_LEVEL_ARRAYS")) ctx->level_arrays = f[0] == '3' ? 3u : 2u;
-    GP_CUDA(ctx, ctx->d_V.ensure(gp::kCbfCounters * 4 * ctx->level_arrays));
-    ctx->surv_cap = uint32_t(size_t(ctx->alive_words) * 32 + size_t(8192) * 9 * 32);
-    GP_CUDA(ctx, ctx->d_alive.ensure(size_t(ctx->surv_cap) * gp::kLevelSurvWords * gp::kLevelListBufs * 4 + 64 + 8192));
+    GP_CUDA(ctx, ctx->d_V.ensure(gp::kCbfCounters * 4 * 2));
     GP_CUDA(ctx, cudaMemcpyAsync(ctx->d_step_pre.p, pre.data(), pre.size() * 4, cudaMemcpyHostToDevice, ctx->stream));
     GP_CUDA(ctx, cudaMemcpyAsync(ctx->d_batch_max_thr.p, maxthr.data(), maxthr.size() * 4, cudaMemcpyHostToDevice, ctx->stream));
     if (ok) {
@@ -617,17 +613,13 @@
     p.anchor = ctx->d_anchor.as<uint16_t>();
     p.anchor_stride = ctx->anchor_stride;
     p.V = ctx->d_V.as<uint32_t>();
-    p.surv = ctx->d_alive.as<uint32_t>();
-    p.bars = reinterpret_cast<unsigned long long*>(ctx->d_alive.as<uint32_t>() + size_t(gp::kLevelSurvWords) * gp::kLevelListBufs * ctx->surv_cap);
     p.overlap = ctx->level_slots > 1 ? 1u : 0u;
-    p.arrays = ctx->level_arrays;
     p.time_bits = ctx->level_time_bits;
     if (const char* f = std::getenv("GP_LEVEL_REPORT_CTA")) p.report_cta = uint32_t(std::atoi(f));
     p.cbf_pool = c.keep_counters ? ctx->d_cbf_pool.as<uint8_t>() : nullptr;
     p.bf_pool = ctx->d_bf_pool.as<uint32_t>();
     p.bf_slot = ctx->bf_all_resident ? nullptr : ctx->d_bf_slot.as<uint32_t>();
     p.counters = ctx->d_counters.as<unsigned long long>();
-    p.surv_cap = ctx->surv_cap;
     p.n_entries = ctx->n_entries;
     p.n_streams = ctx->wave_count[wv] * c.nk;
     p.first_batch = ctx->wave_first[wv];
@@ -635,7 +627,30 @@
     p.nk = c.nk;
     for (uint32_t i = 0; i < gp::kMaxK; i++) p.k[i] = i < c.nk ? c.k[i] : 0;
     if (c.keep_counters) GP_CUDA(ctx, cudaMemsetAsync(ctx->d_cbf_pool.p, 0, uint64_t(p.n_streams) * gp::kCbfCounters, s));
-    GP_CUDA(ctx, cudaMemsetAsync(ctx->d_V.p, 0xFF, gp::kCbfCounters * 4 * ctx->level_arrays, s));
+    {
+      const uint32_t ctas = uint32_t((ctx->sm_count - int(reserve_sms)) * gp::levels_ctas_per_sm(ctas_per_sm));
+      const uint32_t warps = ctas * gp::kLevelWarpsPerCta;
+      const uint64_t occ = uint64_t(ctx->alive_words) * 32;
+      const uint32_t per_cta = gp::buckets_per_cta(occ, ctas);
+      p.n_buckets = per_cta * ctas;
+      p.ovf_cap = uint32_t(occ);
+      p.list_stride = uint32_t(uint64_t(per_cta) * (gp::kBucketCap / gp::kLevelWarpsPerCta) + (occ + warps - 1) / warps + 32);
+      ctx->surv_cap = uint32_t(uint64_t(warps) * p.list_stride);
+      p.surv_cap = ctx->surv_cap;
+      const size_t list_b = size_t(ctx->surv_cap) * gp::kLevelSurvWords * gp::kLevelListBufs * 4;
+      GP_CUDA(ctx, ctx->d_alive.ensure(list_b + 64 + 8192));
+      p.surv = ctx->d_alive.as<uint32_t>();
+      p.bars = reinterpret_cast<unsigned long long*>(ctx->d_alive.as<char>() + list_b);
+      const size_t bkt_b = size_t(gp::kLevelListBufs) * p.n_buckets * gp::kBucketCap * 16, ovf_b = size_t(gp::kLevelListBufs) * p.ovf_cap * 16;
+      const size_t cnt_words = size_t(gp::kLevelListBufs) * p.n_buckets + p.n_streams;
+      GP_CUDA(ctx, ctx->d_groups.ensure(bkt_b + ovf_b + cnt_words * 4));
+      p.bkt = ctx->d_groups.as<uint4>();
+      p.ovf = reinterpret_cast<uint4*>(ctx->d_groups.as<char>() + bkt_b);
+      p.bkt_cnt = reinterpret_cast<uint32_t*>(ctx->d_groups.as<char>() + bkt_b + ovf_b);
+      p.ovf_cnt = p.bkt_cnt + size_t(gp::kLevelListBufs) * p.n_buckets;
+      GP_CUDA(ctx, cudaMemsetAsync(p.bkt_cnt, 0, cnt_words * 4, s));
+    }
+    GP_CUDA(ctx, cudaMemsetAsync(ctx->d_V.p, 0xFF, gp::kCbfCounters * 4 * 2, s));
     GP_CUDA(ctx, cudaMemsetAsync(p.bars, 0, 64 + 8192, s));
     p.speed = reinterpret_cast<uint32_t*>(p.bars + 8);
     {
@@ -648,18 +663,15 @@
     p.n_batches_total = ctx->n_batches;
     p.bf_host = ctx->bf_host_dev;
     {
-      const size_t vbytes = gp::kCbfCounters * 4 * p.arrays;
+      const size_t vbytes = gp::kCbfCounters * 4 * 2;
       const char* e = std::getenv("GP_L2_PERSIST");
       const bool want = !(e && e[0] == '0') && ctx->l2_persist_max > 0 && vbytes <= size_t(ctx->l2_window_max);
       cudaStreamAttrValue av;
       std::memset(&av, 0, sizeof av);
       if (want) {
-        const char* wsel = std::getenv("GP_L2_WINDOW");
-        const bool only_c = wsel && wsel[0] == 'c' && p.arrays == 3u;
-        const size_t wbytes = only_c ? gp::kCbfCounters * 4 : vbytes;
-        av.accessPolicyWindow.base_ptr = only_c ? static_cast<void*>(ctx->d_V.as<uint32_t>() + 2 * gp::kCbfCounters) : ctx->d_V.p;
-        av.accessPolicyWindow.num_bytes = wbytes;
-        av.accessPolicyWindow.hitRatio = std::min(1.0f, float(ctx->l2_persist_max) / float(wbytes));
+        av.accessPolicyWindow.base_ptr = ctx->d_V.p;
+        av.accessPolicyWindow.num_bytes = vbytes;
+        av.accessPolicyWindow.hitRatio = std::min(1.0f, float(ctx->l2_persist_max) / float(vbytes));
         av.accessPolicyWindow.hitProp = cudaAccessPropertyPersisting;
         av.accessPolicyWindow.missProp = cudaAccessPropertyStreaming;
       }
@@ -782,6 +794,7 @@
   GP_CUDA(ctx, cudaMemcpy(c, ctx->d_counters.p, sizeof c, cudaMemcpyDeviceToHost));
   std::memset(out, 0, 32 * 8);
   for (uint32_t i = 0; i < gp::kLevelDiag; i++) out[i] = c[gp::kLevelDiagAt + i];
+  for (uint32_t i = 0; i < gp::kLevelTouch; i++) out[gp::kLevelDiag + i] = c[gp::kLevelTouchAt + i];
   out[31] = c[17];
   return GP_OK;
 }
diff --git a/goldpolish_b200/csrc/gp_build_levels.cu b/goldpolish_b200/csrc/gp_build_levels.cu
--- a/goldpolish_b200/csrc/gp_build_levels.cu
+++ b/goldpolish_b200/csrc/gp_build_levels.cu
@@ -7,7 +7,9 @@
 
 constexpr uint32_t kTimeBits = 26;
 constexpr uint32_t kTimeMask = (1u << kTimeBits) - 1u;
-constexpr int kLevelWarps = 8;
+__device__ __forceinline__ uint32_t thr_of(uint32_t meta) { return meta >> kTimeBits; }
+constexpr int kLevelWarps = int(kLevelWarpsPerCta);
+constexpr uint32_t kGroupBins = 2048;
 
 constexpr uint32_t kRuns = 8;
 
@@ -17,10 +19,6 @@
   uint32_t lane, gwarp;
 };
 
-__device__ __forceinline__ uint64_t warp_list_base(uint32_t n_steps, const uint64_t* cum, uint32_t gwarp)
-{
-  return ((uint64_t(n_steps) * cum[0]) >> 32) + uint64_t(gwarp) * (kRuns + 1u);
-}
 __device__ __forceinline__ void run_of_row(uint32_t r, uint32_t n_steps, const uint64_t* cum, uint32_t& s0, uint32_t& len)
 {
   const uint32_t r0 = uint32_t(uint64_t(n_steps) * r / kRuns), r1 = uint32_t(uint64_t(n_steps) * (r + 1u) / kRuns);
@@ -134,10 +132,10 @@
 struct SurvList {
   uint32_t *lo, *hi, *meta;
 };
-__device__ __forceinline__ SurvList list_of(const LevelParams& p, uint32_t buf, uint32_t n_steps, const uint64_t* cum, uint32_t gwarp)
+__device__ __forceinline__ SurvList list_of(const LevelParams& p, uint32_t buf, uint32_t gwarp)
 {
   SurvList l;
-  l.lo = p.surv + uint64_t(buf) * kLevelSurvWords * p.surv_cap + warp_list_base(n_steps, cum, gwarp) * 32u;
+  l.lo = p.surv + uint64_t(buf) * kLevelSurvWords * p.surv_cap + uint64_t(gwarp) * p.list_stride;
   l.hi = l.lo + p.surv_cap;
   l.meta = l.hi + p.surv_cap;
   return l;
@@ -168,6 +166,10 @@
     }
   }
 }
+
+__device__ __forceinline__ bool leads(uint32_t sub, uint32_t lane) { return sub != 0u && uint32_t(__ffs(sub)) - 1u == lane; }
+__device__ __forceinline__ uint32_t earliest(uint32_t peers, bool race, uint32_t t) { return __reduce_min_sync(peers, race ? t : 0xFFFFFFFFu); }
+
 __device__ __forceinline__ void red_min(uint32_t* p, uint32_t v)
 {
   asm volatile("red.relaxed.gpu.global.min.u32 [%0], %1;" ::"l"(p), "r"(v) : "memory");
@@ -207,9 +209,10 @@
   uint8_t* cbf;
   uint32_t L, lread, tag, tag_next, vmask;
 };
+struct Touch { unsigned long long visits, reds; };
 
 __device__ __forceinline__ uint32_t list_round_all(const ListJob& J, const StreamConsts& sc, uint32_t lane, uint32_t (&nlo)[2],
-                                                   uint32_t (&nhi)[2], uint32_t (&nmeta)[2])
+                                                   uint32_t (&nhi)[2], uint32_t (&nmeta)[2], Touch& tc)
 {
   uint32_t kept = 0;
   for (uint32_t r = 0; r < J.cnt; r += 64u) {
@@ -221,7 +224,7 @@
       live[e] = r + 32u * e + lane < J.cnt;
       meta[e] = nmeta[e];
       h0[e] = uint64_t(nlo[e]) | (uint64_t(nhi[e]) << 32);
-      ins[e] = live[e] && (meta[e] >> kTimeBits) == J.L + 1u;
+      ins[e] = live[e] && thr_of(meta[e]) == J.L + 1u;
       pw[e][0] = pack_index(h0[e]);
       derive_rest(h0[e], sc, pw[e]);
 #pragma unroll
@@ -233,7 +236,7 @@
     if (r + 64u < J.cnt) fetch_entries<2>(J.lst, J.cnt, r + 64u, lane, nlo, nhi, nmeta);
 #pragma unroll
     for (int e = 0; e < 2; e++) {
-      const uint32_t t = meta[e] & kTimeMask, thr = meta[e] >> kTimeBits;
+      const uint32_t t = meta[e] & kTimeMask, thr = thr_of(meta[e]);
       bool reached = live[e];
       uint32_t mx = 0;
 #pragma unroll
@@ -243,11 +246,16 @@
         if (J.cbf && live[e] && v[e][j] == (J.tag | t)) J.cbf[pw[e][j] & 0xFFFFFFu] = (uint8_t)J.L;
       }
       q[e] = reached && t > mx && thr > J.L;
-      if (q[e] && ins[e]) bf_set(J.bf, pw[e], fw[e]);
-      if (q[e] && J.L < J.lread) {
-#pragma unroll
-        for (int j = 0; j < 4; j++) red_min(J.Vn + (pw[e][j] & 0xFFFFFFu), J.tag_next | t);
-      }
+      const bool race = q[e] && J.L < J.lread;
+      const uint32_t peers = __match_any_sync(0xffffffffu, h0[e]);
+      const uint32_t rm = __ballot_sync(0xffffffffu, race) & peers, tmin = earliest(peers, race, t);
+      if (leads(__ballot_sync(0xffffffffu, q[e] && ins[e]) & peers, lane)) bf_set(J.bf, pw[e], fw[e]);
+      if (leads(rm, lane)) {
+#pragma unroll
+        for (int j = 0; j < 4; j++) red_min(J.Vn + (pw[e][j] & 0xFFFFFFu), J.tag_next | tmin);
+      }
+      const bool vis = leads(__ballot_sync(0xffffffffu, live[e]) & peers, lane);
+      tc.visits += __popc(__ballot_sync(0xffffffffu, vis)); tc.reds += 4u * __popc(__ballot_sync(0xffffffffu, leads(rm, lane)));
     }
     surv_append(J.lst, kept, q[0], h0[0], meta[0], lane);
     surv_append(J.lst, kept, q[1], h0[1], meta[1], lane);
@@ -256,7 +264,7 @@
 }
 
 __device__ __forceinline__ uint32_t list_round_first(const ListJob& J, const StreamConsts& sc, uint32_t lane, uint32_t (&nlo)[2],
-                                                     uint32_t (&nhi)[2], uint32_t (&nmeta)[2])
+                                                     uint32_t (&nhi)[2], uint32_t (&nmeta)[2], Touch& tc)
 {
   uint32_t kept = 0;
   for (uint32_t r = 0; r < J.cnt; r += 64u) {
@@ -282,15 +290,20 @@
     }
 #pragma unroll
     for (int e = 0; e < 2; e++) {
-      const uint32_t t = meta[e] & kTimeMask, thr = meta[e] >> kTimeBits;
+      const uint32_t t = meta[e] & kTimeMask, thr = thr_of(meta[e]);
 #pragma unroll
       for (int j = 0; j < 3; j++) q[e] = q[e] && (v[e][j] & ~J.vmask) == J.tag && (v[e][j] & J.vmask) < t;
       q[e] = q[e] && thr > J.L;
-      if (q[e] && thr == J.L + 1u) bf_insert(J.bf, pw[e]);
-      if (q[e] && J.L < J.lread) {
-#pragma unroll
-        for (int j = 0; j < 4; j++) red_min(J.Vn + (pw[e][j] & 0xFFFFFFu), J.tag_next | t);
-      }
+      const bool ins = q[e] && thr == J.L + 1u, race = q[e] && J.L < J.lread;
+      const uint32_t peers = __match_any_sync(0xffffffffu, h0[e]);
+      const uint32_t rm = __ballot_sync(0xffffffffu, race) & peers, tmin = earliest(peers, race, t);
+      if (leads(__ballot_sync(0xffffffffu, ins) & peers, lane)) bf_insert(J.bf, pw[e]);
+      if (leads(rm, lane)) {
+#pragma unroll
+        for (int j = 0; j < 4; j++) red_min(J.Vn + (pw[e][j] & 0xFFFFFFu), J.tag_next | tmin);
+      }
+      const bool vis = leads(__ballot_sync(0xffffffffu, live[e]) & peers, lane);
+      tc.visits += __popc(__ballot_sync(0xffffffffu, vis)); tc.reds += 4u * __popc(__ballot_sync(0xffffffffu, leads(rm, lane)));
     }
     surv_append(J.lst, kept, q[0], h0[0], meta[0], lane);
     surv_append(J.lst, kept, q[1], h0[1], meta[1], lane);
@@ -337,7 +350,7 @@
   return t;
 }
 
-enum : uint32_t { MK_NONE = 0, MK_CLEAR = 1, MK_R0 = 2, MK_R1 = 3 };
+enum : uint32_t { MK_NONE = 0, MK_CLEAR = 1, MK_HASH = 2, MK_GROUP = 3, MK_R1 = 4 };
 
 struct StreamSt {
   uint32_t valid;
@@ -355,21 +368,22 @@
   StreamSt cur;
   StreamSt tail;
   uint32_t next_sid, epoch, ord;
-  uint32_t need_clear, parts, part, r0_done, publish, recal;
+  uint32_t need_clear, hashed, grouped, publish, recal;
   uint4 nx_info;
 };
 
 struct Plan {
   uint32_t finished, main_kind, tail_on;
-  uint32_t row0, row1, part, last_part, publish, recal;
+  uint32_t publish, recal;
   StreamSt cur, tail;
   uint32_t done_n, done_b[2], done_ki[2], done_slot[2];
 };
 
 __global__ void __launch_bounds__(kLevelWarps * 32, 3) build_filters_levels_kernel(LevelParams p)
 {
-  __shared__ uint64_t tf[8 * 256];
-  __shared__ uint64_t tr[8 * 256];
+  __shared__ uint64_t tabs[2][8 * 256];
+  uint64_t* const tf = tabs[0];
+  uint64_t* const tr = tabs[1];
   __shared__ Sched sch;
   __shared__ Plan plans[2];
   __shared__ uint32_t warp_cnt[2][kLevelWarps];
@@ -417,7 +431,8 @@
   const uint32_t wib = threadIdx.x >> 5;
   const uint32_t tb = p.time_bits, vmask = (1u << tb) - 1u, maxtag = (1u << (32u - tb)) - 1u;
   const bool planner = threadIdx.x == 32u;
-  unsigned long long ops = 0, list_seen = 0;
+  unsigned long long ops = 0, list_seen = 0, n_ovf = 0;
+  Touch tc = { 0ull, 0ull };
   if (threadIdx.x == 0) { cal_ns = 0; cal_steps = 0; }
   if (threadIdx.x < kLevelDiag) diag[threadIdx.x] = 0;
   if (threadIdx.x <= uint32_t(kLevelWarps))
@@ -448,16 +463,10 @@
       sch.publish = p.weighted && (sch.ord & 63u) == 4u;
       sch.recal = p.weighted && (sch.ord & 63u) == 5u;
       S.cum = sch.recal ? prev_cum ^ 1u : prev_cum;
-      sch.part = 0; sch.r0_done = 0;
+      sch.hashed = 0; sch.grouped = 0;
       const uint32_t pending = sch.tail.valid ? sch.tail.lread + 2u - sch.tail.L : 0u;
       sch.need_clear = sch.epoch + lmax + 2u + pending > maxtag - 1u;
-      const uint32_t z = (sch.tail.lread + sch.tail.pb) & 1u;
-      S.pb = sch.tail.valid ? (p.arrays == 3u ? z ^ 1u : z) : 0u;
-      sch.parts = 1;
-      if (p.overlap && p.arrays == 3u && sch.tail.valid && !sch.need_clear) {
-        const uint32_t left = sch.tail.lread + 1u - sch.tail.L;
-        sch.parts = left > 2u ? min(left - 1u, kRuns) : 1u;
-      }
+      S.pb = sch.tail.valid ? (sch.tail.lread + sch.tail.pb) & 1u : 0u;
       return;
     }
   };
@@ -473,11 +482,12 @@
       case MK_CLEAR:
         sch.epoch = 0; sch.need_clear = 0;
         break;
-      case MK_R0:
-        if (++sch.part == sch.parts) {
-          sch.r0_done = 1;
-          if (sch.cur.lread == 0u) { push_done(sch.cur); sch.cur.valid = 0; }
-        }
+      case MK_HASH:
+        sch.hashed = 1;
+        break;
+      case MK_GROUP:
+        sch.grouped = 1;
+        if (sch.cur.lread == 0u) { push_done(sch.cur); sch.cur.valid = 0; }
         break;
       case MK_R1:
         if (sch.cur.lread <= 1u) push_done(sch.cur);
@@ -491,24 +501,22 @@
     P.tail_on = sch.tail.valid;
     P.main_kind = MK_NONE;
     if (sch.cur.valid) {
-      if (sch.need_clear) {
-        if (!sch.tail.valid) P.main_kind = MK_CLEAR;
-      } else if (!sch.r0_done) {
-        if (!sch.tail.valid || (p.overlap && (p.arrays == 3u || sch.tail.L == sch.tail.lread))) {
-          P.main_kind = MK_R0;
-          if (sch.part == 0u) sch.cur.tag = new_tag();
-          P.part = sch.part;
-          P.last_part = sch.part + 1u == sch.parts;
-          P.row0 = kRuns * sch.part / sch.parts;
-          P.row1 = kRuns * (sch.part + 1u) / sch.parts;
+      if (!sch.hashed) {
+        if (!sch.tail.valid || p.overlap) {
+          P.main_kind = MK_HASH;
           P.publish = sch.publish; P.recal = sch.recal;
         }
-      } else {
-        if (!sch.tail.valid || (p.overlap && p.arrays == 3u && sch.tail.L == sch.tail.lread)) {
-          P.main_kind = MK_R1;
-          sch.cur.L = 1;
-          sch.cur.tag_next = new_tag();
+      } else if (sch.need_clear) {
+        if (!sch.tail.valid) P.main_kind = MK_CLEAR;
+      } else if (!sch.grouped) {
+        if (!sch.tail.valid || (p.overlap && sch.tail.L == sch.tail.lread)) {
+          P.main_kind = MK_GROUP;
+          sch.cur.tag = new_tag();
         }
+      } else if (!sch.tail.valid) {
+        P.main_kind = MK_R1;
+        sch.cur.L = 1;
+        sch.cur.tag_next = new_tag();
       }
     }
     if (P.tail_on) sch.tail.tag_next = new_tag();
@@ -518,23 +526,23 @@
   if (planner) {
     sch.next_sid = 0; sch.epoch = 0; sch.ord = 0;
     sch.cur.valid = 0; sch.cur.cum = 0; sch.tail.valid = 0;
-    sch.need_clear = 0; sch.parts = 1; sch.part = 0; sch.r0_done = 0; sch.publish = 0; sch.recal = 0;
+    sch.need_clear = 0; sch.hashed = 0; sch.grouped = 0; sch.publish = 0; sch.recal = 0;
     sch.nx_info = p.n_streams ? __ldg(p.stream_tab) : make_uint4(0u, 0u, 0u, 0u);
     make_plan(nullptr, plans[0]);
   }
   __syncthreads();
 
-  auto t1_array = [&](const StreamSt& S) { return p.V + (p.arrays == 3u ? 2u : ((1u + S.pb) & 1u)) * kCbfCounters; };
+  auto t1_array = [&](const StreamSt& S) { return p.V + ((1u + S.pb) & 1u) * kCbfCounters; };
   unsigned long long target = 0;
   for (uint32_t it = 0;; it++) {
     const Plan& P = plans[it & 1u];
     const uint32_t main_kind = P.main_kind, tail_on = P.tail_on;
-    const bool tail_first = tail_on && ((wib & 1u) == 0u || main_kind == MK_NONE);
+    const bool tail_first = tail_on && ((wib & 1u) == 0u || main_kind == MK_NONE || main_kind == MK_GROUP);
     uint32_t nx_lo[2], nx_hi[2], nx_meta[2];
     uint32_t pre_for = 0;
     if (!P.finished && (tail_first || main_kind == MK_R1)) {
       const StreamSt* S = tail_first ? &P.tail : &P.cur;
-      const SurvList l = list_of(p, S->buf, S->n_steps, cum_sh[S->cum] + wib, gwarp_now);
+      const SurvList l = list_of(p, S->buf, gwarp_now);
       fetch_entries<2>(l, warp_cnt[S->buf][wib], 0, c.lane, nx_lo, nx_hi, nx_meta);
       pre_for = tail_first ? 1u : 2u;
     }
@@ -552,7 +560,7 @@
     for (uint32_t i = 0; i < P.done_n; i++) filter_final(p, P.done_b[i], P.done_ki[i], P.done_slot[i], gtid, gthreads);
     if (P.finished) break;
     if (planner) make_plan(&P, plans[(it + 1u) & 1u]);
-    if (main_kind == MK_R0 && P.part == 0u && P.recal) {
+    if (main_kind == MK_HASH && P.recal) {
       unsigned long long tot = 0;
       for (uint32_t i = threadIdx.x; i < gridDim.x; i += blockDim.x) tot += __ldcg(p.speed + i);
       tot = block_sum(tot, red_sh[0]);
@@ -573,39 +581,38 @@
     for (uint32_t ph = 0; ph < 2u; ph++) {
       const bool tail_now = tail_on ? (tail_first ? ph == 0u : ph == 1u) : false;
       const bool main_now = tail_on ? !tail_now : ph == 0u;
-      if (!tail_now && !(main_now && main_kind != MK_NONE)) continue;
+      if (!tail_now && !(main_now && main_kind != MK_NONE && main_kind != MK_GROUP)) continue;
       if (main_now && main_kind == MK_CLEAR) {
-        for (uint64_t i = gtid; i < kCbfCounters * p.arrays; i += gthreads) p.V[i] = 0xFFFFFFFFu;
+        for (uint64_t i = gtid; i < kCbfCounters * 2u; i += gthreads) p.V[i] = 0xFFFFFFFFu;
         continue;
       }
-      if (main_now && main_kind == MK_R0) {
-        const uint32_t ki = P.cur.ki, batch = P.cur.batch, cb = P.cur.buf, n_steps = P.cur.n_steps;
+      if (main_now && main_kind == MK_HASH) {
+        const uint32_t ki = P.cur.ki, batch = P.cur.batch, n_steps = P.cur.n_steps;
         const uint64_t* cum = cum_sh[P.cur.cum] + wib;
         const StreamConsts sc = stream_consts(p.k[ki]);
-        uint32_t* __restrict__ bf = p.bf_pool + (uint64_t(P.cur.slot) * p.nk + ki) * kBfWords;
-        const SurvList lst = list_of(p, cb, n_steps, cum, gwarp_now);
-        uint32_t cnt = P.part ? warp_cnt[cb][wib] : 0u;
-        const uint32_t tag = P.cur.tag;
-        uint32_t* __restrict__ VC = t1_array(P.cur);
+        const uint32_t n_bkt = nb * buckets_per_cta(uint64_t(n_steps) * 32u, nb);
+        uint4* __restrict__ bkt = p.bkt + uint64_t(P.cur.buf) * p.n_buckets * kBucketCap;
+        uint32_t* __restrict__ bcnt = p.bkt_cnt + P.cur.buf * p.n_buckets;
+        uint4* __restrict__ ovf = p.ovf + uint64_t(P.cur.buf) * p.ovf_cap;
+        uint32_t* __restrict__ ocnt = p.ovf_cnt + P.cur.sid;
         unsigned long long w_t0 = 0;
         uint32_t w_steps = 0;
         if (threadIdx.x == 0) w_t0 = globaltimer_ns();
         with_kmer_shape(sc, [&](auto shape) {
-          for_runs<decltype(shape)::value>(p, c, cum, batch, ki, sc, n_steps, P.row0, P.row1,
+          for_runs<decltype(shape)::value>(p, c, cum, batch, ki, sc, n_steps, 0u, kRuns,
                    [&](uint32_t s, uint32_t thr, bool valid, uint64_t h0, const uint32_t (&pw)[4]) {
                      const uint32_t t = s * 32u + c.lane;
-                     const bool q = valid && thr > 0u;
-                     if (q) {
-#pragma unroll
-                       for (int j = 0; j < 4; j++) red_min(VC + (pw[j] & 0xFFFFFFu), tag | t);
-                       if (thr == 1u) bf_insert(bf, pw);
+                     if (valid && thr > 0u) {
+                       const uint32_t b = uint32_t(((h0 >> 32) * n_bkt) >> 32);
+                       const uint4 ent = make_uint4(uint32_t(h0), uint32_t(h0 >> 32), t | (thr << kTimeBits), 0u);
+                       const uint32_t i = atomicAdd(bcnt + b, 1u);
+                       if (i < kBucketCap) bkt[uint64_t(b) * kBucketCap + i] = ent;
+                       else { ovf[atomicAdd(ocnt, 1u)] = ent; n_ovf++; }
                      }
                      if (valid) ops++;
                      w_steps++;
-                     surv_append(lst, cnt, q && thr > 1u, h0, t | (thr << kTimeBits), c.lane);
                    });
         });
-        if (c.lane == 0) warp_cnt[cb][wib] = cnt;
         if (threadIdx.x == 0 && p.weighted) { cal_ns += globaltimer_ns() - w_t0; cal_steps += w_steps; }
         continue;
       }
@@ -614,8 +621,8 @@
       const StreamConsts sc = stream_consts(p.k[S->ki]);
       ListJob J;
       J.L = S->L; J.lread = S->lread; J.tag = S->tag; J.tag_next = S->tag_next; J.vmask = vmask;
-      J.lst = list_of(p, sbuf, S->n_steps, cum_sh[S->cum] + wib, gwarp_now);
-      J.V = J.L == 1u ? t1_array(*S) : p.V + ((J.L + S->pb) & 1u) * kCbfCounters;
+      J.lst = list_of(p, sbuf, gwarp_now);
+      J.V = p.V + ((J.L + S->pb) & 1u) * kCbfCounters;
       J.Vn = p.V + ((J.L + 1u + S->pb) & 1u) * kCbfCounters;
       J.bf = p.bf_pool + (uint64_t(S->slot) * p.nk + S->ki) * kBfWords;
       J.cbf = p.cbf_pool ? p.cbf_pool + uint64_t(S->sid) * kCbfCounters : nullptr;
@@ -623,22 +630,110 @@
       if (c.lane == 0) list_seen += J.cnt;
       if (pre_for != (tail_now ? 1u : 2u)) fetch_entries<2>(J.lst, J.cnt, 0, c.lane, nx_lo, nx_hi, nx_meta);
       pre_for = 0;
-      const uint32_t kept = (J.cbf || J.L > 1u) ? list_round_all(J, sc, c.lane, nx_lo, nx_hi, nx_meta)
-                                                 : list_round_first(J, sc, c.lane, nx_lo, nx_hi, nx_meta);
+      const uint32_t kept = (J.cbf || J.L > 1u) ? list_round_all(J, sc, c.lane, nx_lo, nx_hi, nx_meta, tc)
+                                                 : list_round_first(J, sc, c.lane, nx_lo, nx_hi, nx_meta, tc);
       __syncwarp();
       if (c.lane == 0) warp_cnt[sbuf][wib] = kept;
+    }
+
+    if (main_kind == MK_GROUP) {
+      const StreamSt& S = P.cur;
+      const uint32_t m = buckets_per_cta(uint64_t(S.n_steps) * 32u, nb);
+      const uint4* __restrict__ bkt = p.bkt + uint64_t(S.buf) * p.n_buckets * kBucketCap;
+      uint32_t* __restrict__ bcnt = p.bkt_cnt + S.buf * p.n_buckets;
+      const StreamConsts sc = stream_consts(p.k[S.ki]);
+      uint32_t* __restrict__ VC = t1_array(S);
+      uint32_t* __restrict__ bf = p.bf_pool + (uint64_t(S.slot) * p.nk + S.ki) * kBfWords;
+      const SurvList lst = list_of(p, S.buf, gwarp_now);
+      const uint32_t tag = S.tag;
+      uint32_t* const bin_at = reinterpret_cast<uint32_t*>(&tabs[0][0]);
+      uint16_t* const order = reinterpret_cast<uint16_t*>(bin_at + kGroupBins);
+      uint16_t* const bin_of = order + kBucketCap;
+      uint32_t cnt = 0;
+      auto visit = [&](bool live, uint4 ent) {
+        const uint64_t h0 = uint64_t(ent.x) | (uint64_t(ent.y) << 32);
+        const uint32_t t = ent.z & kTimeMask, thr = thr_of(ent.z);
+        const uint32_t peers = __match_any_sync(0xffffffffu, h0);
+        const uint32_t lm = __ballot_sync(0xffffffffu, live) & peers, tmin = earliest(peers, live, t);
+        const bool ins = leads(__ballot_sync(0xffffffffu, live && thr == 1u) & peers, c.lane);
+        if (leads(lm, c.lane) || ins) {
+          uint32_t pw[4];
+          pw[0] = pack_index(h0);
+          derive_rest(h0, sc, pw);
+          if (leads(lm, c.lane)) {
+#pragma unroll
+            for (int j = 0; j < 4; j++) red_min(VC + (pw[j] & 0xFFFFFFu), tag | tmin);
+          }
+          if (ins) bf_insert(bf, pw);
+        }
+        const uint32_t vis = __popc(__ballot_sync(0xffffffffu, leads(lm, c.lane)));
+        tc.visits += vis; tc.reds += 4u * vis;
+        surv_append(lst, cnt, live && thr > 1u, h0, ent.z, c.lane);
+      };
+      for (uint32_t bi = 0; bi < m; bi++) {
+        const uint32_t b = bid * m + bi;
+        const uint4* __restrict__ src = bkt + uint64_t(b) * kBucketCap;
+        const uint32_t n = min(__ldcg(bcnt + b), kBucketCap);
+        __syncthreads();
+        if (threadIdx.x == 0) bcnt[b] = 0u;
+        for (uint32_t i = threadIdx.x; i < kGroupBins; i += blockDim.x) bin_at[i] = 0u;
+        __syncthreads();
+        for (uint32_t i = threadIdx.x; i < n; i += blockDim.x) {
+          const uint32_t bin = __ldcg(&src[i].x) & (kGroupBins - 1u);
+          bin_of[i] = uint16_t(bin);
+          atomicAdd(bin_at + bin, 1u);
+        }
+        __syncthreads();
+        {
+          constexpr uint32_t per = kGroupBins / (kLevelWarps * 32);
+          uint32_t v[per], run = 0;
+#pragma unroll
+          for (uint32_t i = 0; i < per; i++) { v[i] = bin_at[threadIdx.x * per + i]; run += v[i]; }
+          uint32_t incl = run;
+#pragma unroll
+          for (int o = 1; o < 32; o <<= 1) { const uint32_t y = __shfl_up_sync(0xffffffffu, incl, o); if (c.lane >= uint32_t(o)) incl += y; }
+          if (c.lane == 31u) reinterpret_cast<uint32_t*>(red_sh)[wib] = incl;
+          __syncthreads();
+          uint32_t base = incl - run;
+          for (uint32_t w = 0; w < wib; w++) base += reinterpret_cast<const uint32_t*>(red_sh)[w];
+#pragma unroll
+          for (uint32_t i = 0; i < per; i++) { bin_at[threadIdx.x * per + i] = base; base += v[i]; }
+        }
+        __syncthreads();
+        for (uint32_t i = threadIdx.x; i < n; i += blockDim.x) order[atomicAdd(bin_at + bin_of[i], 1u)] = uint16_t(i);
+        __syncthreads();
+        const uint32_t s0 = n * wib / kLevelWarps, s1 = n * (wib + 1u) / kLevelWarps;
+        for (uint32_t j = s0; j < s1; j += 32u) {
+          const bool live = j + c.lane < s1;
+          uint4 e = make_uint4(0u, 0u, 0u, 0u);
+          if (live) e = __ldcg(src + order[j + c.lane]);
+          visit(live, e);
+        }
+      }
+      const uint32_t nov = __ldcg(p.ovf_cnt + S.sid);
+      const uint4* __restrict__ ovf = p.ovf + uint64_t(S.buf) * p.ovf_cap;
+      for (uint32_t j = gwarp_now * 32u; j < nov; j += nwarps * 32u) {
+        const bool live = j + c.lane < nov;
+        uint4 e = make_uint4(0u, 0u, 0u, 0u);
+        if (live) e = __ldcg(ovf + j + c.lane);
+        visit(live, e);
+      }
+      if (c.lane == 0) warp_cnt[S.buf][wib] = cnt;
+      __syncthreads();
+      fill_hash_tables(tf, tr);
     }
 
     __syncthreads();
     if (threadIdx.x == 0) {
       const unsigned long long t_c = globaltimer_ns();
-      if (main_kind == MK_R0 && P.publish && P.last_part && p.weighted) {
+      if (main_kind == MK_HASH && P.publish && p.weighted) {
         p.speed[bid] = uint32_t(min(max(cal_steps * 4000000ull / max(cal_ns, 1ull), 1ull), 262143ull));
         cal_ns = 0; cal_steps = 0;
       }
       __threadfence();
       atomicAdd(p.bars, 1ull);
-      const uint32_t kind = main_kind == MK_CLEAR ? 0u : main_kind == MK_R0 ? (tail_on ? 4u : 1u) : main_kind == MK_R1 ? (tail_on ? 5u : 2u) : 3u;
+      const uint32_t kind = main_kind == MK_CLEAR ? 0u : main_kind == MK_HASH ? (tail_on ? 4u : 1u) : main_kind == MK_GROUP ? 5u
+                            : main_kind == MK_R1 ? 2u : 3u;
       diag[kind * 3 + 0] += t_b - t_a;
       diag[kind * 3 + 1] += t_c - t_b;
       diag[kind * 3 + 2] += 1;
@@ -646,8 +741,13 @@
   }
 #pragma unroll
   for (int o = 16; o > 0; o >>= 1) ops += __shfl_xor_sync(0xffffffffu, ops, o);
+#pragma unroll
+  for (int o = 16; o > 0; o >>= 1) n_ovf += __shfl_xor_sync(0xffffffffu, n_ovf, o);
   if (c.lane == 0 && ops) atomicAdd(p.counters + 0, ops);
   if (c.lane == 0 && list_seen) atomicAdd(p.counters + 17, list_seen);
+  if (c.lane == 0 && tc.visits) atomicAdd(p.counters + kLevelTouchAt + 0, tc.visits);
+  if (c.lane == 0 && tc.reds) atomicAdd(p.counters + kLevelTouchAt + 1, tc.reds);
+  if (c.lane == 0 && n_ovf) atomicAdd(p.counters + kLevelTouchAt + 2, n_ovf);
   if (bid == 0 && threadIdx.x == 0) atomicMax(p.counters + 21, globaltimer_ns());
   if (bid == p.report_cta && threadIdx.x == 0)
     for (uint32_t i = 0; i < kLevelDiag; i++) p.counters[kLevelDiagAt + i] += diag[i];
diff --git a/goldpolish_b200/csrc/gp_kernels.cuh b/goldpolish_b200/csrc/gp_kernels.cuh
--- a/goldpolish_b200/csrc/gp_kernels.cuh
+++ b/goldpolish_b200/csrc/gp_kernels.cuh
@@ -6,6 +6,7 @@
 namespace gp {
 
 constexpr int kBuildCounters = 64;
+constexpr uint32_t kLevelTouchAt = 2, kLevelTouch = 3;
 constexpr uint32_t kLevelDiag = 18, kLevelDiagAt = 32;
 
 struct BuildParams {
@@ -28,7 +29,15 @@
 };
 
 constexpr uint32_t kLevelSurvWords = 3;
+constexpr uint32_t kLevelWarpsPerCta = 8;
 constexpr uint32_t kLevelListBufs = 2;
+constexpr uint32_t kBucketCap = 4096;
+constexpr uint32_t kBucketFill = 2048;
+__host__ __device__ __forceinline__ uint32_t buckets_per_cta(uint64_t occ, uint32_t ctas)
+{
+  const uint64_t per = uint64_t(ctas) * kBucketFill;
+  return occ > per ? uint32_t((occ + per - 1) / per) : 1u;
+}
 
 struct LevelParams {
   const uint64_t* pk;
@@ -46,6 +55,13 @@
   uint64_t anchor_stride;
   uint32_t* V;
   uint32_t* surv;
+  uint4* bkt;
+  uint32_t* bkt_cnt;
+  uint4* ovf;
+  uint32_t* ovf_cnt;
+  uint32_t n_buckets;
+  uint32_t ovf_cap;
+  uint32_t list_stride;
   unsigned long long* bars;
   uint32_t* speed;
   uint32_t weighted;
@@ -54,7 +70,6 @@
   uint32_t keep_sms;
   uint32_t* sm_table;
   uint32_t overlap;
-  uint32_t arrays;
   uint8_t* cbf_pool;
   uint32_t* bf_pool;
   const uint32_t* bf_slot;
diff --git a/profiles/grouped/ab_bench.py b/profiles/grouped/ab_bench.py
--- /dev/null
+++ b/profiles/grouped/ab_bench.py
@@ -0,0 +1,104 @@
+from __future__ import annotations
+
+import argparse
+import json
+import os
+import subprocess
+import sys
+import time
+
+import numpy as np
+
+ROOT = os.path.dirname(os.path.dirname(os.path.dirname(os.path.abspath(__file__))))
+if ROOT not in sys.path:
+    sys.path.insert(0, ROOT)
+
+TOUCH_WORKLOADS = {
+    "config2_5mbp_30x_bsize1": dict(genome_len=5_000_000, coverage=30.0, bsize=1),
+    "cut_10mbp_40x_bsize8": dict(genome_len=10_000_000, coverage=40.0, bsize=8),
+}
+SEED = 20250607
+
+
+def gpu_info():
+    try:
+        return subprocess.run(["nvidia-smi", "--query-gpu=name,power.limit,clocks.max.sm", "--format=csv,noheader"],
+                              capture_output=True, text=True, timeout=60).stdout.strip()
+    except (OSError, subprocess.SubprocessError):
+        return "unknown"
+
+
+def run_bench(lib, args):
+    env = dict(os.environ)
+    if lib:
+        env["GP_LIB_PATH"] = lib
+    t0 = time.time()
+    p = subprocess.run([sys.executable, os.path.join(ROOT, "bench.py"), "--gpus", "1"] + args, capture_output=True,
+                       text=True, env=env, cwd=ROOT)
+    lines = [l for l in p.stdout.splitlines() if l.startswith("{")]
+    return {"rc": p.returncode, "wall_s": time.time() - t0, "result": json.loads(lines[-1]) if lines else None,
+            "stderr_tail": p.stderr[-2000:] if p.returncode else ""}
+
+
+def ab(a):
+    out = {"gpu": gpu_info(), "bench_args": a.bench_args, "base_lib": a.base_lib, "rounds": []}
+    for r in range(a.rounds):
+        order = [("parent", a.base_lib), ("this", None)] if r % 2 == 0 else [("this", None), ("parent", a.base_lib)]
+        rec = {}
+        for name, lib in order:
+            rec[name] = run_bench(lib, a.bench_args)
+            res = rec[name]["result"] or {}
+            print(f"round {r} {name}: ms_per_step {res.get('ms_per_step')} build ops/s "
+                  f"{(res.get('roofline') or {}).get('kmer_ops_per_s')}", flush=True)
+        out["rounds"].append(rec)
+    return out
+
+
+def touch(a):
+    import goldpolish_b200 as gp
+    import sim
+    out = {"gpu": gpu_info(), "workloads": {}}
+    for name, w in TOUCH_WORKLOADS.items():
+        d = sim.simulate(genome_len=w["genome_len"], coverage=w["coverage"], seed=SEED)
+        pl = gp.plan_batches(np.diff(d.contig_off), [d.contig_name(i) for i in range(d.n_contigs)],
+                             [d.read_name(i) for i in range(d.n_reads)], d.read_phred, np.diff(d.read_off),
+                             d.map_read, d.map_contig, bsize=w["bsize"], subsample_max_per_10kbp=40.0)
+        with gp.Context() as ctx:
+            ctx.upload_reads(d.read_seq, d.read_off)
+            ctx.build_stage(pl.batch_entry_off, pl.entries)
+            ctx.build_run()
+            ctx.build_run()
+            st = ctx.stats()
+            rt = ctx.build_round_times()
+            tc = ctx.build_touch_counts()
+        ops = st["kmer_ops"]
+        streams = (len(pl.batch_entry_off) - 1) * 4
+        rec = {"kmer_ops": ops, "streams": streams, "build_kernel_ms": st["build_kernel_ms"],
+               "kmer_ops_per_s": ops / st["build_kernel_ms"] * 1e3, **tc,
+               "touches_per_op_upper": (4 * tc["group_visits"] + tc["red_min"]) / ops,
+               "group_visits_per_op": tc["group_visits"] / ops, "red_min_per_op": tc["red_min"] / ops,
+               "list_entries_per_op": rt.pop("list_entries") / ops,
+               "intervals_cta0": {k: {"n": n, "wait_us": 1e3 * wt / max(n, 1), "work_us": 1e3 * wk / max(n, 1),
+                                      "work_ms_total": wk, "wait_ms_total": wt} for k, (wt, wk, n) in rt.items()}}
+        rec["intervals_per_stream"] = sum(v["n"] for v in rec["intervals_cta0"].values()) / streams
+        out["workloads"][name] = rec
+        print(name, json.dumps(rec, indent=1), flush=True)
+    return out
+
+
+def main():
+    ap = argparse.ArgumentParser()
+    ap.add_argument("mode", choices=["ab", "touch"])
+    ap.add_argument("--base-lib")
+    ap.add_argument("--rounds", type=int, default=3)
+    ap.add_argument("--out", required=True)
+    ap.add_argument("bench_args", nargs="*")
+    a = ap.parse_args()
+    res = ab(a) if a.mode == "ab" else touch(a)
+    os.makedirs(os.path.dirname(os.path.abspath(a.out)), exist_ok=True)
+    with open(a.out, "w") as f:
+        json.dump(res, f, indent=1)
+
+
+if __name__ == "__main__":
+    main()
```

Result: slower. 25.53, median of 6 (-19.5%).
